# dluvizon/deephar

Measured on AMD Instinct MI355X. Metric: frames/sec whole-node, 256x256 MPII pose fwd, higher is better.
Workload: dtype f32; 1 GPU; MPII single-person 256x256, ReceptionNet 8 blocks J=16 ctx=2 k=5, pose-only forward, batch=64 per GPU (BASELINE.json configs[1]); global_batch=64, parallelism=frame-shard x1 (replicas, no collective), hipgraph=True, streams=1, input=f32, gemm=f32, outputs_finite_in_range=True

## Files before the change

### deephar_amd/_lib.py

```python
import ctypes as C
import os

_HERE = os.path.dirname(os.path.abspath(__file__))
LIB_PATH = os.path.join(_HERE, 'csrc', 'libdeephar_hip.so')

c_f = C.POINTER(C.c_float)
i32, i64, vp = C.c_int32, C.c_int64, C.c_void_p


class ConvArgs(C.Structure):
    _fields_ = [(n, vp) for n in ('x', 'w', 'y', 'pre_scale', 'pre_shift', 'post_scale', 'post_shift',
                                   'res1', 'res2', 'in_lut')] + \
               [(n, i32) for n in ('N', 'H', 'W', 'Cin', 'ldx', 'OH', 'OW', 'Cout', 'ldy', 'KH', 'KW', 'SH',
                                   'SW', 'PT', 'PL', 'K', 'Kp', 'Np', 'ldr1', 'ldr2', 'pre_relu', 'post_relu',
                                   'up2', 'x_u8', 'w_split', 'res2_down', 'ldyp', 'x_resample')] + [('y_pool', vp)]


class ConvSeg(C.Structure):
    _fields_ = [('x2', vp)] + [(n, i32) for n in ('ldx2', 'c_split', 'pool_sh', 'reserved')]


class DwArgs(C.Structure):
    _fields_ = [(n, vp) for n in ('x', 'w', 'y', 'pre_scale', 'pre_shift')] + \
               [(n, i32) for n in ('N', 'H', 'W', 'C', 'ldx', 'ldy', 'KH', 'KW', 'PT', 'PL', 'pre_relu', 'up_in')]


class DwsArgs(C.Structure):
    _fields_ = [(n, vp) for n in ('x', 'w', 'y', 'pre_scale', 'pre_shift')] + \
               [(n, i32) for n in ('N', 'H', 'W', 'C', 'ldx', 'ldy', 'OH', 'OW', 'KH', 'KW', 'SH', 'SW', 'PT', 'PL',
                                   'pre_relu', 'reserved')]


class ConvtArgs(C.Structure):
    _fields_ = [(n, vp) for n in ('x', 'w', 'y', 'pre_scale', 'pre_shift', 'res')] + \
               [(n, i32) for n in ('N', 'H', 'W', 'Cin', 'ldx', 'Cout', 'ldy', 'ldr', 'Kp', 'Np', 'pre_relu', 'post_relu')]


class PoolArgs(C.Structure):
    _fields_ = [(n, vp) for n in ('x', 'y')] + \
               [(n, i32) for n in ('N', 'H', 'W', 'C', 'ldx', 'OH', 'OW', 'ldy', 'KH', 'KW', 'SH', 'SW', 'PT',
                                   'PL', 'mode')]


class EltArgs(C.Structure):
    _fields_ = [(n, vp) for n in ('a', 'b', 'c', 'y', 'scale', 'shift')] + \
               [(n, i32) for n in ('lda', 'ldb', 'ldc', 'ldy')] + [('npix', i64)] + \
               [(n, i32) for n in ('C', 'relu', 'op', 'bcast_b')]


class SamArgs(C.Structure):
    _fields_ = [(n, vp) for n in ('h', 'gx', 'gy', 'xy', 'conf_raw', 'conf_prob', 'prob', 'gmax')] + \
               [(n, i32) for n in ('F', 'H', 'W', 'C', 'ldh', 'ldxy', 'ldcr', 'ldcp', 'ldp')] + \
               [('alpha', C.c_float), ('conf_scale', C.c_float), ('xy_times_conf', i32)]


SIGNATURES = {
    'dh_version': (C.c_int, []),
    'dh_error_string': (C.c_char_p, [C.c_int]),
    'dh_device_info': (C.c_int, [C.c_int, C.c_char_p, C.c_int, C.POINTER(C.c_int)]),
    'dh_conv2d_packed_dims': (C.c_int, [C.c_int] * 4 + [C.POINTER(C.c_int)] * 2),
    'dh_conv2d_pack_weights_host': (C.c_int, [vp, vp] + [C.c_int] * 4),
    'dh_conv2d_pack_weights_split_host': (C.c_int, [vp, vp] + [C.c_int] * 4),
    'dh_conv2d_pack_weights_parts_host': (C.c_int, [vp, vp] + [C.c_int] * 5),
    'dh_conv2d_num_tile_cfgs': (C.c_int, []),
    'dh_conv2d_num_split_tile_cfgs': (C.c_int, []),
    'dh_conv2d_pick_tile_cfg': (C.c_int, [C.c_int, C.c_int]),
    'dh_conv2d_uses_split_k': (C.c_int, [C.POINTER(ConvArgs)]),
    'dh_conv2d_uses_first_layer_kernel': (C.c_int, [C.POINTER(ConvArgs)]),
    'dh_conv2d_split_eligible': (C.c_int, [C.POINTER(ConvArgs)]),
    'dh_conv2d_split_wide_eligible': (C.c_int, [C.POINTER(ConvArgs)]),
    'dh_conv2d_halo_eligible': (C.c_int, [C.POINTER(ConvArgs)]),
    'dh_conv2d_num_halo_tile_cfgs': (C.c_int, []),
    'dh_conv2d_f32': (C.c_int, [C.POINTER(ConvArgs), C.c_int, vp]),
    'dh_normalize_u8_f32': (C.c_int, [vp, vp, vp, C.c_int64, C.c_int, vp]),
    'dh_dwconv2d_f32': (C.c_int, [C.POINTER(DwArgs), vp]),
    'dh_dwconv2d_strided_f32': (C.c_int, [C.POINTER(DwsArgs), vp]),
    'dh_conv2d_transpose2x2_num_tile_cfgs': (C.c_int, []),
    'dh_conv2d_transpose2x2_f32': (C.c_int, [C.POINTER(ConvtArgs), C.c_int, vp]),
    'dh_conv2d_transpose2x2_num_split_tile_cfgs': (C.c_int, []),
    'dh_conv2d_transpose2x2_split_eligible': (C.c_int, [C.POINTER(ConvtArgs)]),
    'dh_conv2d_transpose2x2_split_f32': (C.c_int, [C.POINTER(ConvtArgs), C.c_int, C.c_int, vp]),
    'dh_conv2d_dw_group_f32': (C.c_int, [C.POINTER(ConvArgs), C.POINTER(DwArgs), vp]),
    'dh_conv2d_pair_f32': (C.c_int, [C.POINTER(ConvArgs), C.POINTER(ConvArgs), vp]),
    'dh_conv2d_seg_f32': (C.c_int, [C.POINTER(ConvArgs), C.POINTER(ConvSeg), vp]),
    'dh_pool2d_f32': (C.c_int, [C.POINTER(PoolArgs), vp]),
    'dh_upsample2x_add_f32': (C.c_int, [vp, C.c_int, vp, C.c_int, vp, C.c_int] + [C.c_int] * 4 + [vp]),
    'dh_eltwise_f32': (C.c_int, [C.POINTER(EltArgs), vp]),
    'dh_softargmax2d_f32': (C.c_int, [C.POINTER(SamArgs), vp]),
    'dh_softargmax2d_context_f32': (C.c_int, [C.POINTER(SamArgs), C.c_int, C.c_int, C.c_float, vp, C.c_int, vp]),
    'dh_context_aggregation_f32': (C.c_int, [vp, vp, vp, vp, C.c_int, C.c_int, C.c_int, C.c_float, C.c_int, vp]),
    'dh_depth_means_f32': (C.c_int, [vp, C.c_int, vp, vp] + [C.c_int] * 4 + [vp]),
    'dh_softargmax1d_f32': (C.c_int, [vp, vp, vp, C.c_int, vp] + [C.c_int] * 3 + [vp]),
    'dh_kronecker_f32': (C.c_int, [vp, C.c_int, vp, C.c_int, vp, C.c_int] + [C.c_int] * 4 + [vp]),
    'dh_global_maxmin_softmax_f32': (C.c_int, [vp, C.c_int, vp] + [C.c_int] * 4 + [vp]),
    'dh_copy_channels_f32': (C.c_int, [vp, C.c_int, vp, C.c_int, i64, C.c_int, vp]),
    'dh_zeropad2d_f32': (C.c_int, [vp, vp] + [C.c_int] * 8 + [vp]),
    'dh_depth_from_maps_f32': (C.c_int, [vp, C.c_int, vp, C.c_int, vp, C.c_int] + [C.c_int] * 3 + [vp]),
    'dh_plan_create': (C.c_int, [vp, C.c_size_t, C.POINTER(vp)]),
    'dh_plan_destroy': (C.c_int, [vp]),
    'dh_plan_batch': (C.c_int, [vp]),
    'dh_plan_num_inputs': (C.c_int, [vp]),
    'dh_plan_num_outputs': (C.c_int, [vp]),
    'dh_plan_input_items': (C.c_int64, [vp, C.c_int]),
    'dh_plan_input_is_u8': (C.c_int, [vp, C.c_int]),
    'dh_plan_output_items': (C.c_int64, [vp, C.c_int]),
    'dh_forward': (C.c_int, [vp, C.POINTER(vp), C.c_int, C.POINTER(vp), vp]),
    'dh_forward_host': (C.c_int, [vp, C.POINTER(vp), C.c_int, C.POINTER(vp)]),
    'dh_graph_begin_capture': (C.c_int, [vp]),
    'dh_graph_end_capture': (C.c_int, [vp, C.POINTER(vp)]),
    'dh_graph_launch': (C.c_int, [vp, vp]),
    'dh_graph_destroy': (C.c_int, [vp]),
    'dh_event_create': (C.c_int, [C.POINTER(vp)]),
    'dh_event_record': (C.c_int, [vp, vp]),
    'dh_event_synchronize': (C.c_int, [vp]),
    'dh_event_elapsed_ms': (C.c_int, [vp, vp, C.POINTER(C.c_float)]),
    'dh_event_destroy': (C.c_int, [vp]),
    'dh_stream_synchronize': (C.c_int, [vp]),
    'dh_stream_create': (C.c_int, [C.POINTER(vp)]),
    'dh_stream_destroy': (C.c_int, [vp]),
    'dh_event_create_sync': (C.c_int, [C.POINTER(vp)]),
    'dh_stream_wait_event': (C.c_int, [vp, vp]),
    'dh_stream_spin_us': (C.c_int, [vp, C.c_int]),
}

_lib = None


class DeepharHipError(RuntimeError):
    pass


def load():
    global _lib
    if _lib is not None:
        return _lib
    try:
        import torch
    except ImportError:
        pass
    path = os.environ.get('DEEPHAR_HIP_LIB', LIB_PATH)
    if not os.path.exists(path):
        raise DeepharHipError(
            'libdeephar_hip.so not found at %s -- the HIP back-end is mandatory (no CPU fallback). '
            'Build it with `python -m deephar_amd.csrc.build`.' % path)
    lib = C.CDLL(path)
    for name, (res, args) in SIGNATURES.items():
        fn = getattr(lib, name)
        fn.restype = res
        fn.argtypes = args
    _lib = lib
    return lib


def check(rc, what=''):
    if rc != 0:
        msg = load().dh_error_string(rc).decode()
        raise DeepharHipError('%s failed: %s (rc=%d)' % (what or 'deephar_hip call', msg, rc))
```

### deephar_amd/csrc/build.py

```python
import os
import subprocess
import sys
from concurrent.futures import ThreadPoolExecutor

HERE = os.path.dirname(os.path.abspath(__file__))
ROOT = os.path.dirname(os.path.dirname(HERE))
INCLUDE = os.path.join(ROOT, "include")
SOURCES = ["conv_igemm.hip", "gemm1x1.hip", "convt2x2.hip", "convt2x2s.hip", "gemm1x1s.hip", "gemm1x1s_p2.hip", "gemm1x1s_p1.hip",
           "gemm1x1s_ext.hip", "gemm1x1s_ext_p2.hip", "gemm1x1s_ext_p1.hip", "conv_splitk.hip", "conv_halo.hip", "conv_stem.hip", "spatial.hip", "decoder.hip",
           "capi.hip", "plan.hip"]
HEADERS = sorted(os.path.join(HERE, f) for f in os.listdir(HERE) if f.endswith(".h")) + [os.path.join(INCLUDE, "deephar_hip.h")]
LIB = os.path.join(HERE, "libdeephar_hip.so")
OBJDIR = os.path.join(HERE, "build")
ARCH = "gfx950"
HIPCC = os.environ.get("HIPCC", "/opt/rocm/bin/hipcc")
FLAGS = ["--offload-arch=" + ARCH, "-O3", "-std=c++17", "-fPIC", "-I" + INCLUDE, "-I" + HERE,
         "-Wno-unused-result"]


def _stale(target, deps):
    if not os.path.exists(target):
        return True
    t = os.path.getmtime(target)
    return any(os.path.getmtime(d) > t for d in deps)


def _compile(src):
    obj = os.path.join(OBJDIR, src.replace(".hip", ".o"))
    path = os.path.join(HERE, src)
    deps = [path] + HEADERS
    if _stale(obj, deps):
        cmd = [HIPCC] + FLAGS + ["-c", path, "-o", obj]
        r = subprocess.run(cmd, capture_output=True, text=True)
        if r.returncode != 0:
            raise RuntimeError("hipcc failed for %s:\n%s\n%s" % (src, r.stdout, r.stderr))
    return obj


def build(force=False, verbose=True):
    os.makedirs(OBJDIR, exist_ok=True)
    if force:
        for f in os.listdir(OBJDIR):
            os.remove(os.path.join(OBJDIR, f))
        if os.path.exists(LIB):
            os.remove(LIB)
    with ThreadPoolExecutor(max_workers=len(SOURCES)) as ex:
        objs = list(ex.map(_compile, SOURCES))
    if _stale(LIB, objs):
        cmd = [HIPCC, "--offload-arch=" + ARCH, "-shared", "-fPIC", "-o", LIB] + objs
        r = subprocess.run(cmd, capture_output=True, text=True)
        if r.returncode != 0:
            raise RuntimeError("link failed:\n%s\n%s" % (r.stdout, r.stderr))
        if verbose:
            print("built", LIB)
    elif verbose:
        print("up to date:", LIB)
    return LIB


if __name__ == "__main__":
    build(force="--force" in sys.argv)
```

### deephar_amd/csrc/capi.hip

```cpp
#include <stddef.h>
#include <string.h>
#include <vector>
#include "dh_kernels.h"

using namespace dh;

static inline hipStream_t S(void* s) { return reinterpret_cast<hipStream_t>(s); }
static_assert(sizeof(dh_conv_seg) == 24, "dh_conv_seg layout");
static_assert(sizeof(dh_conv_args) == 200 && offsetof(dh_conv_args, y_pool) == 192 && offsetof(dh_conv_args, x_resample) == 188,
              "dh_conv_args layout");
static_assert(sizeof(dh_dw_args) == 88 && offsetof(dh_dw_args, up_in) == 84, "dh_dw_args layout");
static_assert(sizeof(dh_dw_strided) == 104 && sizeof(dh_conv_transpose) == 96, "dh_dw_strided / dh_conv_transpose layout");
static_assert(sizeof(dh_sam_args) == 112 && offsetof(dh_sam_args, xy_times_conf) == 108, "dh_sam_args layout");
static inline int rc_of(hipError_t e) { return e == hipSuccess ? DH_OK : DH_ELAUNCH; }

extern "C" {

int dh_version(void) { return 100; }

const char* dh_error_string(int rc) {
  switch (rc) {
    case DH_OK: return "ok";
    case DH_EINVAL: return "invalid argument or shape";
    case DH_EUNSUPPORTED: return "configuration not supported by the gfx950 kernels";
    case DH_ELAUNCH: return "HIP launch/runtime error";
    default: return "unknown error";
  }
}

int dh_device_info(int dev, char* arch_name, int arch_name_len, int* cu_count) {
  int n = 0;
  if (hipGetDeviceCount(&n) != hipSuccess || dev < 0 || dev >= n) return DH_ELAUNCH;
  hipDeviceProp_t p;
  if (hipGetDeviceProperties(&p, dev) != hipSuccess) return DH_ELAUNCH;
  if (arch_name != nullptr && arch_name_len > 0) {
    strncpy(arch_name, p.gcnArchName, (size_t)arch_name_len - 1);
    arch_name[arch_name_len - 1] = 0;
  }
  if (cu_count != nullptr) *cu_count = p.multiProcessorCount;
  return DH_OK;
}

int dh_conv2d_packed_dims(int KH, int KW, int Cin, int Cout, int* Kp, int* Np) {
  if (KH <= 0 || KW <= 0 || Cin <= 0 || Cout <= 0) return DH_EINVAL;
  const int K = KH * KW * Cin;
  if (Kp != nullptr) *Kp = (K + 31) / 32 * 32;
  if (Np != nullptr) *Np = (Cout + 31) / 32 * 32;
  return DH_OK;
}

int dh_conv2d_pack_weights_host(const float* w, float* packed, int KH, int KW, int Cin, int Cout) {
  int Kp, Np;
  if (w == nullptr || packed == nullptr || dh_conv2d_packed_dims(KH, KW, Cin, Cout, &Kp, &Np) != DH_OK)
    return DH_EINVAL;
  const int K = KH * KW * Cin;
  memset(packed, 0, sizeof(float) * (size_t)Kp * Np);
  for (int k = 0; k < K; ++k)
    for (int n = 0; n < Cout; ++n)
      packed[((size_t)(k >> 2) * Np + n) * 4 + (k & 3)] = w[(size_t)k * Cout + n];
  return DH_OK;
}

static inline uint16_t bf16_rne(float f) {
  uint32_t u;
  memcpy(&u, &f, 4);
  u += 0x7fffu + ((u >> 16) & 1u);
  return (uint16_t)(u >> 16);
}
static inline float bf16_to_f(uint16_t h) {
  const uint32_t u = (uint32_t)h << 16;
  float f;
  memcpy(&f, &u, 4);
  return f;
}

int dh_conv2d_pack_weights_parts_host(const float* w, uint16_t* packed, int KH, int KW, int Cin, int Cout, int parts) {
  int Kp, Np;
  if (w == nullptr || packed == nullptr || parts < 1 || parts > 3 || dh_conv2d_packed_dims(KH, KW, Cin, Cout, &Kp, &Np) != DH_OK)
    return DH_EINVAL;
  const int K = KH * KW * Cin;
  memset(packed, 0, sizeof(uint16_t) * (size_t)parts * Kp * Np);
  for (int k = 0; k < K; ++k)
    for (int n = 0; n < Cout; ++n) {
      float r = w[(size_t)k * Cout + n];
      const size_t base = ((size_t)(k >> 3) * parts * Np + n) * 8 + (k & 7);
      for (int q = 0; q < parts; ++q) {
        const uint16_t h = bf16_rne(r);
        packed[base + (size_t)q * Np * 8] = h;
        r -= bf16_to_f(h);
      }
    }
  return DH_OK;
}

int dh_conv2d_pack_weights_split_host(const float* w, uint16_t* packed, int KH, int KW, int Cin, int Cout) {
  return dh_conv2d_pack_weights_parts_host(w, packed, KH, KW, Cin, Cout, 3);
}

int dh_conv2d_num_tile_cfgs(void) { return conv_igemm_num_cfgs(); }
int dh_conv2d_num_split_tile_cfgs(void) { return gemm1x1_split_num_cfgs(); }
int dh_conv2d_uses_split_k(const dh_conv_args* a) { return a != nullptr && conv_is_skinny(*a) ? 1 : 0; }
int dh_conv2d_uses_first_layer_kernel(const dh_conv_args* a) {
  return a != nullptr && !conv_is_skinny(*a) && conv_stem_eligible(*a) ? 1 : 0;
}
int dh_conv2d_pick_tile_cfg(int M, int Cout) { return conv_igemm_pick_cfg(M, Cout); }
int dh_conv2d_split_eligible(const dh_conv_args* a) { return a != nullptr && gemm1x1_split_eligible(*a) ? 1 : 0; }
int dh_conv2d_split_wide_eligible(const dh_conv_args* a) { return a != nullptr && gemm1x1_split_wide_eligible(*a) ? 1 : 0; }
int dh_conv2d_halo_eligible(const dh_conv_args* a) { return a != nullptr && conv_halo_eligible(*a) ? 1 : 0; }
int dh_conv2d_num_halo_tile_cfgs(void) { return conv_halo_num_cfgs(); }

int dh_conv2d_f32(const dh_conv_args* a, int tile_cfg, void* stream) {
  if (a == nullptr || a->x == nullptr || a->w == nullptr || a->y == nullptr) return DH_EINVAL;
  if ((a->pre_scale == nullptr) != (a->pre_shift == nullptr)) return DH_EINVAL;
  if ((a->post_scale == nullptr) != (a->post_shift == nullptr)) return DH_EINVAL;
  if (a->SH <= 0 || a->SW <= 0 || a->KH <= 0 || a->KW <= 0) return DH_EINVAL;
  if (a->res2_down && (a->res2 == nullptr || a->up2 || (a->OH & 1) || (a->OW & 1))) return DH_EINVAL;
  return launch_conv_igemm(*a, tile_cfg, S(stream));
}

int dh_conv2d_dw_group_f32(const dh_conv_args* a, const dh_dw_args* d, void* stream) {
  if (a == nullptr || d == nullptr || a->x == nullptr || a->w == nullptr || a->y == nullptr || d->x == nullptr ||
      d->w == nullptr || d->y == nullptr)
    return DH_EINVAL;
  if ((a->pre_scale == nullptr) != (a->pre_shift == nullptr) || (a->post_scale == nullptr) != (a->post_shift == nullptr) ||
      (d->pre_scale == nullptr) != (d->pre_shift == nullptr))
    return DH_EINVAL;
  return launch_conv_dw_group(*a, *d, S(stream));
}

static int check_skinny_args(const dh_conv_args* c) {
  if (c == nullptr || c->x == nullptr || c->w == nullptr || c->y == nullptr) return DH_EINVAL;
  if ((c->pre_scale == nullptr) != (c->pre_shift == nullptr) || (c->post_scale == nullptr) != (c->post_shift == nullptr)) return DH_EINVAL;
  if (c->SH <= 0 || c->SW <= 0 || c->KH <= 0 || c->KW <= 0 || c->N <= 0 || c->Cin <= 0 || c->Cout <= 0 || c->OH <= 0 || c->OW <= 0)
    return DH_EINVAL;
  if (c->Kp % 32 != 0 || c->Np % 32 != 0 || c->Kp < c->K || c->Np < c->Cout || c->K != c->KH * c->KW * c->Cin) return DH_EINVAL;
  if ((long long)c->N * c->H * c->W > 0x7fffffffLL || (long long)c->N * c->OH * c->OW * (c->up2 ? 4 : 1) > 0x7fffffffLL) return DH_EINVAL;
  return DH_OK;
}

int dh_conv2d_pair_f32(const dh_conv_args* a, const dh_conv_args* b, void* stream) {
  if (check_skinny_args(a) != DH_OK || check_skinny_args(b) != DH_OK) return DH_EINVAL;
  return launch_conv_skinny_pair(*a, *b, S(stream));
}

int dh_conv2d_seg_f32(const dh_conv_args* a, const dh_conv_seg* seg, void* stream) {
  if (seg == nullptr || check_skinny_args(a) != DH_OK) return DH_EINVAL;
  return launch_conv_splitk_seg(*a, *seg, S(stream));
}

int dh_normalize_u8_f32(const uint8_t* x, const float* lut, float* y, int64_t n_pixels, int C, void* stream) {
  if (x == nullptr || lut == nullptr || y == nullptr) return DH_EINVAL;
  return launch_normalize_u8(x, lut, y, n_pixels, C, S(stream));
}

int dh_dwconv2d_f32(const dh_dw_args* a, void* stream) {
  if (a == nullptr || a->x == nullptr || a->w == nullptr || a->y == nullptr) return DH_EINVAL;
  if ((a->pre_scale == nullptr) != (a->pre_shift == nullptr)) return DH_EINVAL;
  return launch_dwconv(*a, S(stream));
}

int dh_dwconv2d_strided_f32(const dh_dw_strided* a, void* stream) {
  if (a == nullptr || a->x == nullptr || a->w == nullptr || a->y == nullptr) return DH_EINVAL;
  if ((a->pre_scale == nullptr) != (a->pre_shift == nullptr)) return DH_EINVAL;
  if (a->SH <= 0 || a->SW <= 0 || a->KH <= 0 || a->KW <= 0) return DH_EINVAL;
  return launch_dwconv_strided(*a, S(stream));
}

int dh_conv2d_transpose2x2_num_tile_cfgs(void) { return convt2x2_num_cfgs(); }

static dh_conv_args convt_gemm(const dh_conv_transpose* a) {
  dh_conv_args g;
  memset(&g, 0, sizeof(g));
  g.x = a->x; g.w = a->w; g.y = a->y;
  g.pre_scale = a->pre_scale; g.pre_shift = a->pre_shift;
  g.res1 = a->res; g.ldr1 = a->ldr;
  g.N = a->N; g.H = g.OH = a->H; g.W = g.OW = a->W; g.Cin = g.K = a->Cin; g.ldx = a->ldx;
  g.Cout = 4 * a->Cout; g.ldy = a->ldy;
  g.KH = g.KW = g.SH = g.SW = 1;
  g.Kp = a->Kp; g.Np = a->Np;
  g.pre_relu = a->pre_relu; g.post_relu = a->post_relu;
  return g;
}

int dh_conv2d_transpose2x2_f32(const dh_conv_transpose* a, int tile_cfg, void* stream) {
  if (a == nullptr || a->x == nullptr || a->w == nullptr || a->y == nullptr) return DH_EINVAL;
  if ((a->pre_scale == nullptr) != (a->pre_shift == nullptr)) return DH_EINVAL;
  if (a->N <= 0 || a->H <= 0 || a->W <= 0 || a->Cin <= 0 || a->Cout <= 0 || a->Cout > 0x7fffffff / 4) return DH_EINVAL;
  if (tile_cfg >= convt2x2_num_cfgs()) return DH_EINVAL;
  return launch_convt2x2(convt_gemm(a), a->Cout, tile_cfg, S(stream));
}

int dh_conv2d_transpose2x2_num_split_tile_cfgs(void) { return convt2x2_split_num_cfgs(); }

int dh_conv2d_transpose2x2_split_eligible(const dh_conv_transpose* a) {
  if (a == nullptr || (a->pre_scale == nullptr) != (a->pre_shift == nullptr)) return 0;
  if (a->N <= 0 || a->H <= 0 || a->W <= 0 || a->Cin <= 0 || a->Cout <= 0 || a->Cout > 0x7fffffff / 4) return 0;
  return convt2x2_split_eligible(convt_gemm(a), a->Cout) ? 1 : 0;
}

int dh_conv2d_transpose2x2_split_f32(const dh_conv_transpose* a, int parts, int tile_cfg, void* stream) {
  if (parts < 1 || parts > 3) return DH_EINVAL;
  if (a == nullptr || a->x == nullptr || a->w == nullptr || a->y == nullptr) return DH_EINVAL;
  if ((a->pre_scale == nullptr) != (a->pre_shift == nullptr)) return DH_EINVAL;
  if (a->N <= 0 || a->H <= 0 || a->W <= 0 || a->Cin <= 0 || a->Cout <= 0 || a->Cout > 0x7fffffff / 4) return DH_EINVAL;
  if (tile_cfg >= convt2x2_split_num_cfgs()) return DH_EINVAL;
  return launch_convt2x2_split(convt_gemm(a), a->Cout, parts, tile_cfg, S(stream));
}

int dh_pool2d_f32(const dh_pool_args* a, void* stream) {
  if (a == nullptr || a->x == nullptr || a->y == nullptr || a->SH <= 0 || a->SW <= 0) return DH_EINVAL;
  return launch_pool(*a, S(stream));
}

int dh_upsample2x_add_f32(const float* a, int lda, const float* b, int ldb, float* y, int ldy, int N, int H,
                          int W, int C, void* stream) {
  if (b == nullptr || y == nullptr) return DH_EINVAL;
  return launch_upsample2x_add(a, lda, b, ldb, y, ldy, N, H, W, C, S(stream));
}

int dh_eltwise_f32(const dh_elt_args* a, void* stream) {
  if (a == nullptr) return DH_EINVAL;
  if ((a->scale == nullptr) != (a->shift == nullptr)) return DH_EINVAL;
  return launch_eltwise(*a, S(stream));
}

int dh_softargmax2d_f32(const dh_sam_args* a, void* stream) {
  if (a == nullptr) return DH_EINVAL;
  return launch_softargmax2d(*a, S(stream));
}

int dh_softargmax2d_context_f32(const dh_sam_args* a, int J, int nctx, float agg_alpha, float* y, int ldy,
                                void* stream) {
  if (a == nullptr) return DH_EINVAL;
  return launch_softargmax2d_context(*a, J, nctx, agg_alpha, y, ldy, S(stream));
}

int dh_context_aggregation_f32(const float* ys, const float* yc, const float* pc, float* y, int F, int J,
                               int nctx, float alpha, int ldy, void* stream) {
  if (ys == nullptr || yc == nullptr || pc == nullptr || y == nullptr || ldy < 2) return DH_EINVAL;
  return launch_context_agg(ys, yc, pc, y, F, J, nctx, alpha, ldy, S(stream));
}

int dh_depth_means_f32(const float* h, int ldh, float* hxy, float* hz, int F, int HW, int D, int J,
                       void* stream) {
  if (h == nullptr || (hxy == nullptr && hz == nullptr)) return DH_EINVAL;
  return launch_depth_means(h, ldh, hxy, hz, F, HW, D, J, S(stream));
}

int dh_softargmax1d_f32(const float* hz, const float* grid, float* z, int ldz, float* vz, int F, int D, int J,
                        void* stream) {
  if (hz == nullptr || grid == nullptr) return DH_EINVAL;
  return launch_softargmax1d(hz, grid, z, ldz, vz, F, D, J, S(stream));
}

int dh_kronecker_f32(const float* hm, int ldh, const float* x, int ldx, float* f, int ldf, int B, int P, int J,
                     int C, void* stream) {
  if (hm == nullptr || x == nullptr || f == nullptr) return DH_EINVAL;
  return launch_kronecker(hm, ldh, x, ldx, f, ldf, B, P, J, C, S(stream));
}

int dh_global_maxmin_softmax_f32(const float* x, int ldx, float* y, int B, int P, int C, int softmax,
                                 void* stream) {
  if (x == nullptr || y == nullptr) return DH_EINVAL;
  return launch_global_maxmin_softmax(x, ldx, y, B, P, C, softmax, S(stream));
}

int dh_copy_channels_f32(const float* x, int ldx, float* y, int ldy, int64_t npix, int C, void* stream) {
  if (x == nullptr || y == nullptr) return DH_EINVAL;
  return launch_copy_channels(x, ldx, y, ldy, (long long)npix, C, S(stream));
}

int dh_zeropad2d_f32(const float* x, float* y, int B, int H, int W, int C, int OH, int OW, int PT, int PL,
                     void* stream) {
  if (x == nullptr || y == nullptr) return DH_EINVAL;
  return launch_zeropad(x, y, B, H, W, C, OH, OW, PT, PL, S(stream));
}

int dh_depth_from_maps_f32(const float* d, int ldd, const float* h, int ldh, float* z, int ldz, int F, int HW,
                           int J, void* stream) {
  if (d == nullptr || h == nullptr || z == nullptr) return DH_EINVAL;
  return launch_depth_from_maps(d, ldd, h, ldh, z, ldz, F, HW, J, S(stream));
}

int dh_graph_begin_capture(void* stream) {
  return rc_of(hipStreamBeginCapture(S(stream), hipStreamCaptureModeThreadLocal));
}

int dh_graph_end_capture(void* stream, void** graph_exec_out) {
  if (graph_exec_out == nullptr) return DH_EINVAL;
  hipGraph_t g = nullptr;
  if (hipStreamEndCapture(S(stream), &g) != hipSuccess || g == nullptr) return DH_ELAUNCH;
  hipGraphExec_t ge = nullptr;
  hipError_t e = hipGraphInstantiate(&ge, g, nullptr, nullptr, 0);
  hipGraphDestroy(g);
  if (e != hipSuccess) return DH_ELAUNCH;
  *graph_exec_out = ge;
  return DH_OK;
}

int dh_graph_launch(void* graph_exec, void* stream) {
  if (graph_exec == nullptr) return DH_EINVAL;
  return rc_of(hipGraphLaunch(reinterpret_cast<hipGraphExec_t>(graph_exec), S(stream)));
}

int dh_graph_destroy(void* graph_exec) {
  if (graph_exec == nullptr) return DH_OK;
  return rc_of(hipGraphExecDestroy(reinterpret_cast<hipGraphExec_t>(graph_exec)));
}

int dh_event_create(void** event_out) {
  if (event_out == nullptr) return DH_EINVAL;
  hipEvent_t e;
  if (hipEventCreate(&e) != hipSuccess) return DH_ELAUNCH;
  *event_out = e;
  return DH_OK;
}
int dh_event_record(void* event, void* stream) {
  return rc_of(hipEventRecord(reinterpret_cast<hipEvent_t>(event), S(stream)));
}
int dh_event_synchronize(void* event) { return rc_of(hipEventSynchronize(reinterpret_cast<hipEvent_t>(event))); }
int dh_event_elapsed_ms(void* start, void* stop, float* ms_out) {
  if (ms_out == nullptr) return DH_EINVAL;
  return rc_of(hipEventElapsedTime(ms_out, reinterpret_cast<hipEvent_t>(start), reinterpret_cast<hipEvent_t>(stop)));
}
int dh_event_destroy(void* event) { return rc_of(hipEventDestroy(reinterpret_cast<hipEvent_t>(event))); }
int dh_stream_synchronize(void* stream) { return rc_of(hipStreamSynchronize(S(stream))); }

int dh_stream_create(void** stream_out) {
  if (stream_out == nullptr) return DH_EINVAL;
  hipStream_t st;
  if (hipStreamCreateWithFlags(&st, hipStreamNonBlocking) != hipSuccess) return DH_ELAUNCH;
  *stream_out = st;
  return DH_OK;
}
int dh_stream_destroy(void* stream) { return rc_of(hipStreamDestroy(S(stream))); }
int dh_event_create_sync(void** event_out) {
  if (event_out == nullptr) return DH_EINVAL;
  hipEvent_t e;
  if (hipEventCreateWithFlags(&e, hipEventDisableTiming) != hipSuccess) return DH_ELAUNCH;
  *event_out = e;
  return DH_OK;
}
int dh_stream_wait_event(void* stream, void* event) {
  return rc_of(hipStreamWaitEvent(S(stream), reinterpret_cast<hipEvent_t>(event), 0));
}

__global__ void spin_kernel(long long ticks) {
  const long long t0 = wall_clock64();
  for (int i = 0; i < (1 << 22) && wall_clock64() - t0 < ticks; ++i) __builtin_amdgcn_s_sleep(8);
}
int dh_stream_spin_us(void* stream, int us) {
  if (us < 0 || us > 20000) return DH_EINVAL;
  hipLaunchKernelGGL(spin_kernel, dim3(1), dim3(64), 0, S(stream), (long long)us * 100);
  return check_launch();
}

}
```

### deephar_amd/csrc/dh_kernels.h

```cpp
#pragma once
#include <hip/hip_runtime.h>
#include <stdint.h>
#include "deephar_hip.h"

namespace dh {

using ConvArgs = dh_conv_args;
using ConvSeg = dh_conv_seg;
using DwArgs = dh_dw_args;
using DwsArgs = dh_dw_strided;
using PoolArgs = dh_pool_args;
using EltArgs = dh_elt_args;
using SamArgs = dh_sam_args;

__device__ __forceinline__ int xcd_order(int b, int nwg) {
  const int xcd = b & 7, q = nwg >> 3, r = nwg & 7;
  return (xcd < r ? xcd * (q + 1) : r * (q + 1) + (xcd - r) * q) + (b >> 3);
}

int launch_conv_igemm(const ConvArgs& a, int cfg, hipStream_t s);
int launch_normalize_u8(const unsigned char* x, const float* lut, float* y, long long n_pixels, int C, hipStream_t s);
int conv_igemm_pick_cfg(int M, int Cout);
int conv_igemm_num_cfgs();
bool conv_is_skinny(const ConvArgs& a);
bool conv_stem_eligible(const ConvArgs& a);
int gemm1x1_split_num_cfgs();
bool gemm1x1_split_eligible(const ConvArgs& a);
int conv_split_parts(int w_split);
bool gemm1x1_split_wide_eligible(const ConvArgs& a);
int conv_split_wide_base(int w_split);
bool conv_halo_eligible(const ConvArgs& a);
int conv_halo_num_cfgs();
int launch_dwconv(const DwArgs& a, hipStream_t s);
int launch_dwconv_strided(const DwsArgs& a, hipStream_t s);
int launch_convt2x2(const ConvArgs& gemm, int cb, int cfg, hipStream_t s);
int convt2x2_num_cfgs();
int launch_convt2x2_split(const ConvArgs& gemm, int cb, int parts, int cfg, hipStream_t s);
bool convt2x2_split_eligible(const ConvArgs& gemm, int cb);
int convt2x2_split_num_cfgs();
int launch_conv_dw_group(const ConvArgs& a, const DwArgs& d, hipStream_t s);
int launch_conv_skinny_pair(const ConvArgs& a, const ConvArgs& b, hipStream_t s);
int launch_conv_splitk_seg(const ConvArgs& a, const ConvSeg& seg, hipStream_t s);
int launch_pool(const PoolArgs& a, hipStream_t s);
int launch_upsample2x_add(const float* a, int lda, const float* b, int ldb, float* y, int ldy, int N, int H,
                          int W, int C, hipStream_t s);
int launch_eltwise(const EltArgs& a, hipStream_t s);
int launch_softargmax2d(const SamArgs& a, hipStream_t s);
int launch_softargmax2d_context(const SamArgs& a, int J, int nctx, float agg_alpha, float* y, int ldy, hipStream_t s);
int launch_context_agg(const float* ys, const float* yc, const float* pc, float* y, int F, int J, int nctx,
                       float alpha, int ldy, hipStream_t s);
int launch_depth_means(const float* h, int ldh, float* hxy, float* hz, int F, int HW, int D, int J,
                       hipStream_t s);
int launch_softargmax1d(const float* hz, const float* grid, float* z, int ldz, float* vz, int F, int D, int J,
                        hipStream_t s);
int launch_kronecker(const float* hm, int ldh, const float* x, int ldx, float* f, int ldf, int B, int P, int J,
                     int C, hipStream_t s);
int launch_global_maxmin_softmax(const float* x, int ldx, float* y, int B, int P, int C, int softmax,
                                 hipStream_t s);
int launch_copy_channels(const float* x, int ldx, float* y, int ldy, long long npix, int C, hipStream_t s);
int launch_zeropad(const float* x, float* y, int B, int H, int W, int C, int OH, int OW, int PT, int PL,
                   hipStream_t s);
int launch_depth_from_maps(const float* d, int ldd, const float* h, int ldh, float* z, int ldz, int F, int HW,
                           int J, hipStream_t s);

struct LdsLimit {
  unsigned long long done = 0;
  void raise(const void* kern, int bytes) {
    int dev = 0;
    if (hipGetDevice(&dev) != hipSuccess) return;
    const unsigned long long bit = 1ull << (dev & 63);
    if (done & bit) return;
    hipFuncSetAttribute(kern, hipFuncAttributeMaxDynamicSharedMemorySize, bytes);
    done |= bit;
  }
};

inline bool al16(const void* q) { return (reinterpret_cast<uintptr_t>(q) & 15) == 0; }
constexpr long long kMaxBufferBytes = 0xf0000000LL;
inline bool conv_is_1x1(const ConvArgs& a) { return a.KH == 1 && a.KW == 1 && a.SH == 1 && a.SW == 1 && a.PT == 0 && a.PL == 0; }
inline bool conv_is_pointwise(const ConvArgs& a) { return conv_is_1x1(a) && a.H == a.OH && a.W == a.OW && a.Cin % 4 == 0; }

inline int check_launch() {
  hipError_t e = hipGetLastError();
  return e == hipSuccess ? DH_OK : DH_ELAUNCH;
}

}
```

### deephar_amd/csrc/dw_lds.h

```cpp
#pragma once
#include "dh_kernels.h"
#include "lds_dma.h"

namespace dh {
namespace dwl {

__device__ __forceinline__ float4 ld4(const float* p) { return *reinterpret_cast<const float4*>(p); }
__device__ __forceinline__ void st4(float* p, float4 v) { *reinterpret_cast<float4*>(p) = v; }
__device__ __forceinline__ float4 fma4(float4 a, float4 b, float4 c) {
  return make_float4(fmaf(a.x, b.x, c.x), fmaf(a.y, b.y, c.y), fmaf(a.z, b.z, c.z), fmaf(a.w, b.w, c.w));
}
__device__ __forceinline__ float4 max4(float4 a, float4 b) {
  return make_float4(fmaxf(a.x, b.x), fmaxf(a.y, b.y), fmaxf(a.z, b.z), fmaxf(a.w, b.w));
}
__device__ __forceinline__ float4 min4(float4 a, float4 b) {
  return make_float4(fminf(a.x, b.x), fminf(a.y, b.y), fminf(a.z, b.z), fminf(a.w, b.w));
}


constexpr int DW_CQ = 8;
#ifndef DW_LDS_MIN_W
#define DW_LDS_MIN_W 8
#endif
constexpr int DW_PITCH = 9;
constexpr int DW_OOB = (int)0x80000000u;

typedef unsigned int dw_u4 __attribute__((ext_vector_type(4)));
template <typename RSRC>
__device__ __forceinline__ float4 buf_ld4(RSRC rs, int voff) {
  float4 r = make_float4(0.f, 0.f, 0.f, 0.f);
#if defined(__HIP_DEVICE_COMPILE__)
  const dw_u4 v = __builtin_amdgcn_raw_buffer_load_b128(rs, voff, 0, 0);
  r = make_float4(__uint_as_float(v.x), __uint_as_float(v.y), __uint_as_float(v.z), __uint_as_float(v.w));
#endif
  return r;
}
template <typename RSRC>
__device__ __forceinline__ void buf_st4(RSRC rs, int voff, int soff, float4 r) {
#if defined(__HIP_DEVICE_COMPILE__)
  dw_u4 v;
  v.x = __float_as_uint(r.x); v.y = __float_as_uint(r.y); v.z = __float_as_uint(r.z); v.w = __float_as_uint(r.w);
  __builtin_amdgcn_raw_buffer_store_b128(v, rs, voff, soff, 0);
#endif
}

template <int KS, int NT, int MAXT, int MAXN, bool AFF, bool RELU>
__device__ __forceinline__ void dwconv_lds_body(const DwArgs& p, const int tw, const int rows, const int twh_magic,
                                                const int block, float4* dsm) {
  constexpr int SP = NT / DW_CQ;
  const int tid = threadIdx.x;
  const int chunks = p.C / 32;
  const int bands = (p.H + rows - 1) / rows;
  const int ctiles = (p.W + tw - 1) / tw;
  int b = block;
  const int cchunk = b % chunks; b /= chunks;
  const int ct = b % ctiles;
  const int n = b / ctiles;
  const int c0 = cchunk * 32, w0 = ct * tw;
  const int th = rows + KS - 1, twh = tw + KS - 1;
  float4* wts = dsm;
  float4* tile = dsm + KS * KS * DW_CQ;
  const float4 zero = make_float4(0.f, 0.f, 0.f, 0.f);

  constexpr int WPT = (KS * KS * DW_CQ + NT - 1) / NT;
  float4 wreg[WPT];
#pragma unroll
  for (int k = 0; k < WPT; ++k) {
    const int i = tid + k * NT;
    const int ic = i < KS * KS * DW_CQ ? i : 0;
    wreg[k] = ld4(p.w + (size_t)(ic / DW_CQ) * p.C + c0 + (ic % DW_CQ) * 4);
  }
  const int q = tid & (DW_CQ - 1);
  float4 sc = make_float4(1.f, 1.f, 1.f, 1.f), sh = zero;
  if constexpr (AFF) { sc = ld4(p.pre_scale + c0 + q * 4); sh = ld4(p.pre_shift + c0 + q * 4); }

  const int ush = p.up_in ? 1 : 0;
  const int hw_in = (p.H >> ush) * (p.W >> ush), w_in = p.W >> ush;
  const auto rs_x = __builtin_amdgcn_make_buffer_rsrc(
      const_cast<float*>(p.x) + (size_t)n * hw_in * p.ldx, 0,
      (int)(((unsigned)(hw_in - 1) * p.ldx + (unsigned)p.C) * 4u), 0x00020000);
  const auto rs_y = __builtin_amdgcn_make_buffer_rsrc(
      p.y + (size_t)n * p.H * p.W * p.ldy, 0, (int)(((unsigned)(p.H * p.W - 1) * p.ldy + (unsigned)p.C) * 4u), 0x00020000);
  const int row_bytes = twh * DW_PITCH * 16, ring_bytes = th * row_bytes;
  const int dump = ring_bytes;
  auto row_of = [&](int px) { return (px * twh_magic) >> 16; };
  auto px_offset = [&](int px, int first_row) {
    const int tr = row_of(px), tc = px - tr * twh;
    const int iw = w0 - p.PL + tc;
    return (unsigned)iw < (unsigned)p.W ? ((((first_row + tr) >> ush) * w_in + (iw >> ush)) * p.ldx + c0 + q * 4) * 4 : DW_OOB;
  };

  float4 top[MAXT];
#pragma unroll
  for (int j = 0; j < MAXT; ++j) {
    const int px = (tid >> 3) + j * SP;
    top[j] = buf_ld4(rs_x, px < (KS - 1) * twh ? px_offset(px, -p.PT) : DW_OOB);
  }
  int voff[MAXN], loff[MAXN];
  int trow[AFF ? MAXN : 1];
#pragma unroll
  for (int j = 0; j < MAXN; ++j) {
    const int px = (tid >> 3) + j * SP;
    const bool in = px < rows * twh;
    voff[j] = in ? px_offset(px, KS - 1 - p.PT) : DW_OOB;
    loff[j] = in ? (KS - 1) * row_bytes + (px * DW_PITCH + q) * 16 : -1;
    if constexpr (AFF) trow[j] = (in && voff[j] != DW_OOB) ? row_of(px) : -1;
  }
  float4 stage[MAXN];
  auto fetch = [&](int band) {
    const int boff = band * (rows >> ush) * w_in * p.ldx * 4;
#pragma unroll
    for (int j = 0; j < MAXN; ++j) stage[j] = buf_ld4(rs_x, voff[j] + boff);
  };
  fetch(0);
#pragma unroll
  for (int k = 0; k < WPT; ++k) {
    const int i = tid + k * NT;
    if (i < KS * KS * DW_CQ) wts[i] = wreg[k];
  }
#pragma unroll
  for (int j = 0; j < MAXT; ++j) {
    const int px = (tid >> 3) + j * SP;
    float4 v = top[j];
    if constexpr (AFF) {
      const int tr = row_of(px), iw = w0 - p.PL + px - tr * twh;
      v = fma4(v, sc, sh);
      if (!((unsigned)(tr - p.PT) < (unsigned)p.H && (unsigned)iw < (unsigned)p.W)) v = zero;
    }
    if constexpr (RELU) v = relu4(v);
    if (px < (KS - 1) * twh) tile[px * DW_PITCH + q] = v;
  }
  const int strips = tw >> 3;
  const int strip = (tid >> 3) % strips;
  const int row = (tid >> 3) / strips;
  const int y_off = ((row * p.W + w0 + strip * 8) * p.ldy + c0 + q * 4) * 4;
  const int y_col = p.ldy * 4;
  char* const tile_b = reinterpret_cast<char*>(tile);

  int ring0 = 0;
  for (int band = 0; band < bands; ++band) {
    const int r0 = band * rows;
    const int shift = ring0 * row_bytes;
    if (band > 0) fetch(band);
#pragma unroll
    for (int j = 0; j < MAXN; ++j) {
      float4 v = stage[j];
      if constexpr (AFF) {
        v = fma4(v, sc, sh);
        if (!(trow[j] >= 0 && (unsigned)(r0 + KS - 1 - p.PT + trow[j]) < (unsigned)p.H)) v = zero;
      }
      if constexpr (RELU) v = relu4(v);
      int o = loff[j] + shift;
      o = o >= ring_bytes ? o - ring_bytes : o;
      o = loff[j] < 0 ? dump : o;
      *reinterpret_cast<float4*>(tile_b + o) = v;
    }
    __syncthreads();

    if (row < rows && r0 + row < p.H && w0 + strip * 8 < p.W) {
      float4 acc[8];
#pragma unroll
      for (int i = 0; i < 8; ++i) acc[i] = zero;
      int rr = ring0 + row;
      rr = rr >= th ? rr - th : rr;
#pragma unroll 1
      for (int kh = 0; kh < KS; ++kh) {
        float4 wv[KS];
#pragma unroll
        for (int kw = 0; kw < KS; ++kw) wv[kw] = wts[(kh * KS + kw) * DW_CQ + q];
        const float4* src = tile + (rr * twh + strip * 8) * DW_PITCH + q;
#pragma unroll
        for (int j = 0; j < 8 + KS - 1; ++j) {
          const float4 v = src[j * DW_PITCH];
#pragma unroll
          for (int kw = 0; kw < KS; ++kw) {
            const int o = j - kw;
            if (o >= 0 && o < 8) acc[o] = fma4(v, wv[kw], acc[o]);
          }
        }
        rr = rr + 1 == th ? 0 : rr + 1;
      }
      const int yo = y_off + r0 * p.W * p.ldy * 4;
#pragma unroll
      for (int i = 0; i < 8; ++i) buf_st4(rs_y, yo, i * y_col, acc[i]);
    }
    __syncthreads();
    ring0 += rows;
    ring0 = ring0 >= th ? ring0 - th : ring0;
  }
}

struct DwLdsGeom {
  int tw, rows, nt;
  unsigned blocks;
  size_t lds;
};
inline bool dw_lds_geometry(const DwArgs& a, DwLdsGeom& g) {
  const bool vec = (a.C % 4 == 0) && (a.ldx % 4 == 0) && (a.ldy % 4 == 0) && al16(a.x) && al16(a.y) && al16(a.w) &&
                   (a.pre_scale == nullptr || (al16(a.pre_scale) && al16(a.pre_shift)));
  if (!(vec && a.KH == a.KW && (a.KW == 5 || a.KW == 3) && a.C % 32 == 0 && a.W >= DW_LDS_MIN_W && a.W % 8 == 0)) return false;
  g.tw = a.W >= 32 ? 32 : a.W;
  g.nt = g.tw == 8 ? 64 : 256;
  g.rows = g.nt / (8 * (g.tw / 8));
  if (g.rows > a.H) g.rows = a.H;
  const long long blocks = (long long)a.N * ((a.W + g.tw - 1) / g.tw) * (a.C / 32);
  g.lds = ((size_t)(g.rows + a.KW - 1) * (g.tw + a.KW - 1) * DW_PITCH + (size_t)a.KW * a.KW * DW_CQ + 1) * 16;
  const bool fits31 = (long long)a.H * a.W * a.ldx * 4 < 0x7fffffffLL && (long long)a.H * a.W * a.ldy * 4 < 0x7fffffffLL;
  if (blocks > 0x7fffffffLL || !fits31) return false;
  g.blocks = (unsigned)blocks;
  const int twh = g.tw + a.KW - 1, maxt = a.KW == 5 ? (g.nt == 256 ? 5 : 6) : 3, maxn = a.KW == 5 ? (g.nt == 256 ? 10 : 12) : 10;
  return (a.KW - 1) * twh <= maxt * (g.nt / DW_CQ) && g.rows * twh <= maxn * (g.nt / DW_CQ);
}

}
}
```

### deephar_amd/csrc/gemm1x1_body.h

```cpp
#pragma once
#include "conv_common.h"
#include "gemm_family.h"
#include "lds_dma.h"

namespace dh {

template <bool PRE, int S>
__device__ __forceinline__ void fetch_affine(unsigned t_sc, unsigned t_sh, float4& sc, float4& sh) {
  if constexpr (PRE) {
    sc = lds_rd<S * 32>(t_sc);
    sh = lds_rd<S * 32>(t_sh);
  }
}

template <int TM, int TN, int BN, int BOFF, int S>
__device__ __forceinline__ void fetch_frags(const unsigned (&a_addr)[TM][4], unsigned b_addr, float4 (&fa)[TM],
                                            float4 (&fb)[TN]) {
  fa[0] = lds_rd<0>(a_addr[0][S]);
  if constexpr (TM > 1) fa[1] = lds_rd<0>(a_addr[1][S]);
  constexpr int BO = BOFF + S * 2 * BN * 16;
  fb[0] = lds_rd<BO>(b_addr);
  if constexpr (TN > 1) fb[1] = lds_rd<BO + 512>(b_addr);
  if constexpr (TN > 2) fb[2] = lds_rd<BO + 1024>(b_addr);
}

template <int WM, int WN, int TM, int TN, bool UP2, bool RELU, bool KXK = false, bool PRE = false, bool D2S = false>
__device__ __forceinline__ void gemm1x1_body(const ConvArgs& p, const int epi_vec, const int block, const int nblocks,
                                             float* const smem, const int cb = 0) {
  static_assert(!(PRE && (KXK || UP2)), "the BN prologue is built for the plain pointwise form");
  static_assert(!(D2S && (KXK || UP2)), "the depth-to-space epilogue follows the plain pointwise main loop");
  constexpr int NT = WM * WN * 64;
  constexpr int BM = WM * TM * 32;
  constexpr int BN = WN * TN * 32;
  constexpr int APASS = BM * 8 / NT;
  constexpr int BPASS = 8 * BN / NT;
  constexpr int STAGE = BM * BK + BK * BN;
  static_assert(BM * 8 % NT == 0 && (8 * BN) % NT == 0, "tile/thread mismatch");

  const int tid = threadIdx.x;
  const int lane = tid & 63;
  const int wave = tid >> 6;
  const int wm = wave / WN, wn = wave % WN;
  const int li = lane & 31, lh = lane >> 5;

  const int M = p.N * p.OH * p.OW;
  const int tiles_n = (p.Cout + BN - 1) / BN;
  const int tile = xcd_tile(block, nblocks);
  const int m0 = (tile / tiles_n) * BM;
  const int n0 = (tile % tiles_n) * BN;

  const int wave_u = __builtin_amdgcn_readfirstlane(wave);
  const auto rs_x = __builtin_amdgcn_make_buffer_rsrc(
      const_cast<float*>(p.x), 0, (int)(((unsigned)(p.N * p.H * p.W - 1) * p.ldx + (unsigned)p.Cin) * 4u), 0x00020000);
  const auto rs_w = __builtin_amdgcn_make_buffer_rsrc(const_cast<float*>(p.w), 0, (int)((unsigned)p.Kp * p.Np * 4u),
                                                      0x00020000);
  unsigned a_off[APASS];
  int a_slot[APASS];
  int a_pix[KXK ? APASS : 1], a_ih0[KXK ? APASS : 1], a_iw0[KXK ? APASS : 1];
#pragma unroll
  for (int ps = 0; ps < APASS; ++ps) {
    const int r = (tid >> 3) + ps * (NT / 8);
    int m = m0 + r;
    m = m < M ? m : M - 1;
    a_slot[ps] = ((tid & 7) ^ (r & 7)) * 4;
    if constexpr (KXK) {
      const int n = m / (p.OH * p.OW);
      const int rem = m - n * (p.OH * p.OW);
      const int oh = rem / p.OW, ow = rem - oh * p.OW;
      a_pix[ps] = n * p.H * p.W;
      a_ih0[ps] = oh * p.SH - p.PT;
      a_iw0[ps] = ow * p.SW - p.PL;
      a_off[ps] = 0;
    } else {
      a_off[ps] = ((unsigned)m * p.ldx + a_slot[ps]) * 4u;
    }
  }
  const int chunks_per_tap = KXK ? p.Cin / BK : 1;
  unsigned b_off[BPASS];
#pragma unroll
  for (int q = 0; q < BPASS; ++q) {
    const int idx = tid + q * NT;
    const int kq = idx / BN, j = idx - kq * BN;
    const int col = n0 + j < p.Np ? n0 + j : 0;
    b_off[q] = ((unsigned)kq * p.Np + col) * 16u;
  }
  const int b_step = 8 * p.Np * 16;

  auto issue = [&](int kt, int stage) {
    float* sA = smem + stage * STAGE;
    float* sB = sA + BM * BK;
    int kh = 0, kw = 0, c0 = 0;
    if constexpr (KXK) {
      const int tap = kt / chunks_per_tap;
      c0 = (kt - tap * chunks_per_tap) * BK;
      kh = tap / p.KW;
      kw = tap - kh * p.KW;
    }
#pragma unroll
    for (int ps = 0; ps < APASS; ++ps) {
      if constexpr (KXK) {
        const int ih = a_ih0[ps] + kh, iw = a_iw0[ps] + kw;
        const bool ok = (unsigned)ih < (unsigned)p.H && (unsigned)iw < (unsigned)p.W && kt * BK < p.K;
        const unsigned off = ok ? ((unsigned)(a_pix[ps] + ih * p.W + iw) * p.ldx + c0 + a_slot[ps]) * 4u : OOB;
        dma16(rs_x, sA + (ps * NT + wave_u * 64) * 4, off, 0);
      } else {
        dma16(rs_x, sA + (ps * NT + wave_u * 64) * 4, a_off[ps], kt * BK * 4);
      }
    }
#pragma unroll
    for (int q = 0; q < BPASS; ++q) dma16(rs_w, sB + (q * NT + wave_u * 64) * 4, b_off[q], kt * b_step);
  };

  f32x16 acc[TM][TN];
#pragma unroll
  for (int i = 0; i < TM; ++i)
#pragma unroll
    for (int j = 0; j < TN; ++j)
#pragma unroll
      for (int r = 0; r < 16; ++r) acc[i][j][r] = 0.f;

  const int nk = p.Kp / BK;
  issue(0, 0);
  if constexpr (PRE) {
    float* tab = smem + 2 * STAGE;
    for (int i = tid; i < p.Kp; i += NT) {
      tab[i] = i < p.K ? p.pre_scale[i] : 0.f;
      tab[p.Kp + i] = i < p.K ? p.pre_shift[i] : 0.f;
    }
  }
  asm volatile("s_waitcnt vmcnt(0)" ::: "memory");
  __syncthreads();

  const unsigned lds0 = (unsigned)(uintptr_t)(lptr_t)smem;
  unsigned a_base[TM][4];
#pragma unroll
  for (int i = 0; i < TM; ++i)
#pragma unroll
    for (int q = 0; q < 4; ++q)
      a_base[i][q] = lds0 + (unsigned)(((wm * TM + i) * 32 + li) * BK * 4 + (((q * 2 + lh) ^ (li & 7)) << 4));
  const unsigned b_base = lds0 + (unsigned)((lh * BN + wn * TN * 32 + li) * 16);
  constexpr int BOFF = BM * BK * 4;

  auto mfma_block = [&](const float4 (&a)[TM], const float4 (&b)[TN]) {
#pragma unroll
    for (int i = 0; i < TM; ++i)
#pragma unroll
      for (int j = 0; j < TN; ++j) {
        acc[i][j] = __builtin_amdgcn_mfma_f32_32x32x2f32(a[i].x, b[j].x, acc[i][j], 0, 0, 0);
        acc[i][j] = __builtin_amdgcn_mfma_f32_32x32x2f32(a[i].y, b[j].y, acc[i][j], 0, 0, 0);
        acc[i][j] = __builtin_amdgcn_mfma_f32_32x32x2f32(a[i].z, b[j].z, acc[i][j], 0, 0, 0);
        acc[i][j] = __builtin_amdgcn_mfma_f32_32x32x2f32(a[i].w, b[j].w, acc[i][j], 0, 0, 0);
      }
  };
  auto relu_frags = [&](float4 (&a)[TM], const float4& sc, const float4& sh) {
    if constexpr (PRE) {
#pragma unroll
      for (int i = 0; i < TM; ++i)
        a[i] = make_float4(fmaf(a[i].x, sc.x, sh.x), fmaf(a[i].y, sc.y, sh.y), fmaf(a[i].z, sc.z, sh.z), fmaf(a[i].w, sc.w, sh.w));
    }
    if constexpr (RELU) {
#pragma unroll
      for (int i = 0; i < TM; ++i) a[i] = relu4(a[i]);
    }
  };
  const unsigned t_sc0 = lds0 + (unsigned)(2 * STAGE * 4 + lh * 16);

  EpiPrefetch<TM, TN> pre;
  for (int kt = 0; kt < nk; ++kt) {
    const int cur = kt & 1;
    if constexpr (!D2S) {
      if (kt == nk - 1) pre.template issue<WM, WN>(p, m0, n0, M, epi_vec);
    }
    const unsigned so = (unsigned)(cur * STAGE * 4);
    unsigned a_addr[TM][4];
#pragma unroll
    for (int i = 0; i < TM; ++i)
#pragma unroll
      for (int q = 0; q < 4; ++q) a_addr[i][q] = a_base[i][q] + so;
    const unsigned b_addr = b_base + so;

    float4 fa0[TM], fb0[TN], fa1[TM], fb1[TN];
    float4 sc0, sh0, sc1, sh1;
    const unsigned t_sc = t_sc0 + (unsigned)(kt * BK * 4), t_sh = t_sc + (unsigned)(p.Kp * 4);
    fetch_frags<TM, TN, BN, BOFF, 0>(a_addr, b_addr, fa0, fb0);
    fetch_affine<PRE, 0>(t_sc, t_sh, sc0, sh0);
    __builtin_amdgcn_sched_barrier(0);
    if (kt + 1 < nk) issue(kt + 1, cur ^ 1);
    lgkm_wait();
    fetch_frags<TM, TN, BN, BOFF, 1>(a_addr, b_addr, fa1, fb1);
    fetch_affine<PRE, 1>(t_sc, t_sh, sc1, sh1);
    __builtin_amdgcn_sched_barrier(0);
    relu_frags(fa0, sc0, sh0);
    mfma_block(fa0, fb0);
    lgkm_wait();
    fetch_frags<TM, TN, BN, BOFF, 2>(a_addr, b_addr, fa0, fb0);
    fetch_affine<PRE, 2>(t_sc, t_sh, sc0, sh0);
    __builtin_amdgcn_sched_barrier(0);
    relu_frags(fa1, sc1, sh1);
    mfma_block(fa1, fb1);
    lgkm_wait();
    fetch_frags<TM, TN, BN, BOFF, 3>(a_addr, b_addr, fa1, fb1);
    fetch_affine<PRE, 3>(t_sc, t_sh, sc1, sh1);
    __builtin_amdgcn_sched_barrier(0);
    relu_frags(fa0, sc0, sh0);
    mfma_block(fa0, fb0);
    lgkm_wait();
    relu_frags(fa1, sc1, sh1);
    mfma_block(fa1, fb1);

    asm volatile("s_waitcnt vmcnt(0)" ::: "memory");
    __syncthreads();
  }

  if constexpr (D2S) d2s_epilogue<WM, WN, TM, TN>(p, acc, smem, m0, n0, M, epi_vec, cb);
  else conv_epilogue<WM, WN, TM, TN, UP2, true>(p, acc, smem, m0, n0, M, epi_vec, pre);
}

}
```

### deephar_amd/csrc/plan.hip

```cpp
#include <cstring>
#include <vector>
#include "dh_kernels.h"

namespace {

using dh::check_launch;

enum Fn { F_CONV, F_DW, F_POOL, F_UPADD, F_ELT, F_SAM, F_CTX, F_DMEANS, F_SAM1D, F_KRON, F_GMM, F_COPY, F_ZPAD, F_DFM, F_SAMCTX, F_NORM, F_GROUP, F_PAIR, F_SEG, F_DWS, F_CONVT, F_CONVTS, F_COUNT };

struct Step { int fn; std::vector<unsigned char> payload; };
struct In { uint64_t tag; size_t items; int u8; char* dst; };
struct Out { size_t off, npix; int C, ld; };

}

struct dh_plan {
  int n = 0;
  size_t arena_bytes = 0, weight_bytes = 0, byte_bytes = 0;
  char* arena = nullptr;
  char* weights = nullptr;
  char* bytes = nullptr;
  std::vector<In> ins;
  std::vector<Out> outs;
  std::vector<Step> steps;
  std::vector<float*> in_dev, out_dev;
  hipStream_t stream = nullptr;
};

namespace {

struct Reader {
  const unsigned char* p;
  const unsigned char* end;
  bool ok = true;
  template <typename T>
  T get() {
    T v{};
    if (p + sizeof(T) > end) { ok = false; return v; }
    std::memcpy(&v, p, sizeof(T));
    p += sizeof(T);
    return v;
  }
};

bool fix(const dh_plan& pl, uint64_t v, void** out) {
  const uint64_t region = v >> 60, off = v & ((1ull << 60) - 1);
  if (v == 0) { *out = nullptr; return true; }
  if (region == 1 && off < pl.arena_bytes) { *out = pl.arena + off; return true; }
  if (region == 2 && off < pl.weight_bytes) { *out = pl.weights + off; return true; }
  if (region == 3 && off < pl.byte_bytes) { *out = pl.bytes + off; return true; }
  return false;
}

int struct_pointers(int fn) {
  switch (fn) {
    case F_CONV: return 10;
    case F_DW: return 5;
    case F_POOL: return 2;
    case F_ELT: return 6;
    case F_SAM: return 8;
    case F_SAMCTX: return 8;
    case F_DWS: return 5;
    case F_CONVT: return 6;
    case F_CONVTS: return 6;
  }
  return -1;
}
void struct_extra(int fn, int* nargs, unsigned* ptr_mask) {
  *nargs = 0;
  *ptr_mask = 0;
  if (fn == F_CONV || fn == F_CONVT) *nargs = 1;
  if (fn == F_CONVTS) *nargs = 2;
  if (fn == F_SAMCTX) { *nargs = 5; *ptr_mask = 0x08; }
}
size_t struct_size(int fn) {
  switch (fn) {
    case F_CONV: return sizeof(dh_conv_args);
    case F_DW: return sizeof(dh_dw_args);
    case F_POOL: return sizeof(dh_pool_args);
    case F_ELT: return sizeof(dh_elt_args);
    case F_SAM: return sizeof(dh_sam_args);
    case F_SAMCTX: return sizeof(dh_sam_args);
    case F_DWS: return sizeof(dh_dw_strided);
    case F_CONVT: return sizeof(dh_conv_transpose);
    case F_CONVTS: return sizeof(dh_conv_transpose);
  }
  return 0;
}
bool scalar_sig(int fn, int* nargs, unsigned* ptr_mask) {
  switch (fn) {
    case F_UPADD: *nargs = 10; *ptr_mask = 0x15; return true;
    case F_CTX: *nargs = 9; *ptr_mask = 0x0f; return true;
    case F_DMEANS: *nargs = 8; *ptr_mask = 0x0d; return true;
    case F_SAM1D: *nargs = 8; *ptr_mask = 0x17; return true;
    case F_KRON: *nargs = 10; *ptr_mask = 0x15; return true;
    case F_GMM: *nargs = 7; *ptr_mask = 0x05; return true;
    case F_COPY: *nargs = 6; *ptr_mask = 0x05; return true;
    case F_ZPAD: *nargs = 10; *ptr_mask = 0x03; return true;
    case F_DFM: *nargs = 9; *ptr_mask = 0x15; return true;
    case F_NORM: *nargs = 5; *ptr_mask = 0x07; return true;
  }
  return false;
}

int run_step(const Step& st, void* stream) {
  const unsigned char* p = st.payload.data();
  auto u = [&](int i) { uint64_t v; std::memcpy(&v, p + 8 * i, 8); return v; };
  auto P = [&](int i) { return reinterpret_cast<float*>(static_cast<uintptr_t>(u(i))); };
  auto I = [&](int i) { return static_cast<int>(static_cast<int64_t>(u(i))); };
  auto Fl = [&](int i) { float f; std::memcpy(&f, p + 8 * i, 4); return f; };
  switch (st.fn) {
    case F_CONV: {
      int64_t cfg;
      std::memcpy(&cfg, p + sizeof(dh_conv_args), 8);
      return dh_conv2d_f32(reinterpret_cast<const dh_conv_args*>(p), (int)cfg, stream);
    }
    case F_SAMCTX: {
      const unsigned char* e = p + sizeof(dh_sam_args);
      int64_t J, nctx, ldy;
      float alpha;
      void* y;
      std::memcpy(&J, e, 8); std::memcpy(&nctx, e + 8, 8); std::memcpy(&alpha, e + 16, 4);
      std::memcpy(&y, e + 24, 8); std::memcpy(&ldy, e + 32, 8);
      return dh_softargmax2d_context_f32(reinterpret_cast<const dh_sam_args*>(p), (int)J, (int)nctx, alpha,
                                         static_cast<float*>(y), (int)ldy, stream);
    }
    case F_DW: return dh_dwconv2d_f32(reinterpret_cast<const dh_dw_args*>(p), stream);
    case F_DWS: return dh_dwconv2d_strided_f32(reinterpret_cast<const dh_dw_strided*>(p), stream);
    case F_CONVT: {
      int64_t cfg;
      std::memcpy(&cfg, p + sizeof(dh_conv_transpose), 8);
      return dh_conv2d_transpose2x2_f32(reinterpret_cast<const dh_conv_transpose*>(p), (int)cfg, stream);
    }
    case F_CONVTS: {
      int64_t parts, cfg;
      std::memcpy(&parts, p + sizeof(dh_conv_transpose), 8);
      std::memcpy(&cfg, p + sizeof(dh_conv_transpose) + 8, 8);
      return dh_conv2d_transpose2x2_split_f32(reinterpret_cast<const dh_conv_transpose*>(p), (int)parts, (int)cfg, stream);
    }
    case F_GROUP:
      return dh_conv2d_dw_group_f32(reinterpret_cast<const dh_conv_args*>(p),
                                    reinterpret_cast<const dh_dw_args*>(p + sizeof(dh_conv_args)), stream);
    case F_PAIR:
      return dh_conv2d_pair_f32(reinterpret_cast<const dh_conv_args*>(p), reinterpret_cast<const dh_conv_args*>(p + sizeof(dh_conv_args)),
                                stream);
    case F_SEG:
      return dh_conv2d_seg_f32(reinterpret_cast<const dh_conv_args*>(p), reinterpret_cast<const dh_conv_seg*>(p + sizeof(dh_conv_args)),
                               stream);
    case F_POOL: return dh_pool2d_f32(reinterpret_cast<const dh_pool_args*>(p), stream);
    case F_ELT: return dh_eltwise_f32(reinterpret_cast<const dh_elt_args*>(p), stream);
    case F_SAM: return dh_softargmax2d_f32(reinterpret_cast<const dh_sam_args*>(p), stream);
    case F_UPADD: return dh_upsample2x_add_f32(P(0), I(1), P(2), I(3), P(4), I(5), I(6), I(7), I(8), I(9), stream);
    case F_CTX: return dh_context_aggregation_f32(P(0), P(1), P(2), P(3), I(4), I(5), I(6), Fl(7), I(8), stream);
    case F_DMEANS: return dh_depth_means_f32(P(0), I(1), P(2), P(3), I(4), I(5), I(6), I(7), stream);
    case F_SAM1D: return dh_softargmax1d_f32(P(0), P(1), P(2), I(3), P(4), I(5), I(6), I(7), stream);
    case F_KRON: return dh_kronecker_f32(P(0), I(1), P(2), I(3), P(4), I(5), I(6), I(7), I(8), I(9), stream);
    case F_GMM: return dh_global_maxmin_softmax_f32(P(0), I(1), P(2), I(3), I(4), I(5), I(6), stream);
    case F_COPY: return dh_copy_channels_f32(P(0), I(1), P(2), I(3), static_cast<int64_t>(u(4)), I(5), stream);
    case F_ZPAD: return dh_zeropad2d_f32(P(0), P(1), I(2), I(3), I(4), I(5), I(6), I(7), I(8), I(9), stream);
    case F_DFM: return dh_depth_from_maps_f32(P(0), I(1), P(2), I(3), P(4), I(5), I(6), I(7), I(8), stream);
    case F_NORM: return dh_normalize_u8_f32(reinterpret_cast<const uint8_t*>(P(0)), P(1), P(2), static_cast<int64_t>(u(3)),
                                            I(4), stream);
  }
  return DH_EINVAL;
}

}

extern "C" {

int dh_plan_create(const void* blob, size_t blob_bytes, dh_plan** out) {
  if (blob == nullptr || out == nullptr || blob_bytes < 44) return DH_EINVAL;
  Reader r{static_cast<const unsigned char*>(blob), static_cast<const unsigned char*>(blob) + blob_bytes};
  if (std::memcmp(r.p, "DHPL", 4) != 0) return DH_EINVAL;
  r.p += 4;
  const uint32_t version = r.get<uint32_t>();
  if (version < 1 || version > 4) return DH_EINVAL;
  dh_plan* pl = new dh_plan();
  pl->n = r.get<int32_t>();
  pl->arena_bytes = r.get<uint64_t>();
  pl->weight_bytes = r.get<uint64_t>();
  const uint32_t nin = r.get<uint32_t>(), nout = r.get<uint32_t>(), nsteps = r.get<uint32_t>();
  if (version >= 2) pl->byte_bytes = r.get<uint64_t>();
  auto fail = [&](int rc) { dh_plan_destroy(pl); return rc; };
  if (!r.ok || pl->n <= 0 || nin == 0 || nout == 0 || nin > 64 || nout > 4096 || nsteps > (1u << 20) ||
      pl->byte_bytes > (1ull << 40))
    return fail(DH_EINVAL);
  for (uint32_t i = 0; i < nin; ++i) {
    In in{};
    in.tag = r.get<uint64_t>();
    in.items = (size_t)r.get<uint64_t>();
    if (version >= 2) {
      in.u8 = (int)r.get<uint32_t>();
      (void)r.get<uint32_t>();
    } else {
      in.tag |= 1ull << 60;
    }
    pl->ins.push_back(in);
  }
  for (uint32_t i = 0; i < nout; ++i) {
    Out o;
    o.off = r.get<uint64_t>(); o.npix = r.get<uint64_t>(); o.C = (int)r.get<uint32_t>(); o.ld = (int)r.get<uint32_t>();
    pl->outs.push_back(o);
  }
  for (uint32_t i = 0; i < nsteps && r.ok; ++i) {
    Step st;
    st.fn = (int)r.get<uint32_t>();
    const uint32_t nb = r.get<uint32_t>();
    if (!r.ok || st.fn < 0 || st.fn >= (version >= 4 ? (int)F_COUNT : (version == 3 ? (int)F_CONVTS : (int)F_DWS)) || r.p + nb > r.end) return fail(DH_EINVAL);
    st.payload.assign(r.p, r.p + nb);
    r.p += nb;
    pl->steps.push_back(std::move(st));
  }
  if (!r.ok || (size_t)(r.end - r.p) != pl->weight_bytes) return fail(DH_EINVAL);
  if (hipMalloc(&pl->arena, pl->arena_bytes ? pl->arena_bytes : 16) != hipSuccess) return fail(DH_ELAUNCH);
  if (hipMalloc(&pl->weights, pl->weight_bytes ? pl->weight_bytes : 16) != hipSuccess) return fail(DH_ELAUNCH);
  if (pl->weight_bytes && hipMemcpy(pl->weights, r.p, pl->weight_bytes, hipMemcpyHostToDevice) != hipSuccess)
    return fail(DH_ELAUNCH);
  if (pl->byte_bytes && hipMalloc(&pl->bytes, pl->byte_bytes) != hipSuccess) return fail(DH_ELAUNCH);
  const uint64_t arena_f = pl->arena_bytes / 4, nn = (uint64_t)pl->n;
  auto fits = [&](uint64_t off_bytes, uint64_t rows, uint64_t pitch, uint64_t last) {
    if (off_bytes % 4 || off_bytes / 4 > arena_f || rows == 0 || pitch > arena_f || last > arena_f || rows > arena_f) return false;
    const uint64_t room = arena_f - off_bytes / 4;
    if (pitch != 0 && rows - 1 > room / pitch) return false;
    return (rows - 1) * pitch + last <= room;
  };
  for (In& in : pl->ins) {
    const uint64_t region = in.tag >> 60, off = in.tag & ((1ull << 60) - 1);
    if (in.u8 == 0) {
      if (region != 1 || in.items == 0 || in.items > arena_f || !fits(off, nn, in.items, in.items)) return fail(DH_EINVAL);
      in.dst = pl->arena + off;
    } else {
      if (in.u8 != 1 || region != 3 || in.items == 0 || in.items > pl->byte_bytes || nn > pl->byte_bytes / in.items ||
          off > pl->byte_bytes - in.items * nn)
        return fail(DH_EINVAL);
      in.dst = pl->bytes + off;
    }
  }
  for (const Out& o : pl->outs)
    if (o.C <= 0 || o.ld < o.C || o.npix == 0 || o.npix > arena_f || !fits(o.off, o.npix * nn, (uint64_t)o.ld, (uint64_t)o.C))
      return fail(DH_EINVAL);
  for (Step& st : pl->steps) {
    const int np = struct_pointers(st.fn);
    if (st.fn == F_GROUP || st.fn == F_PAIR || st.fn == F_SEG) {
      const size_t second = st.fn == F_GROUP ? sizeof(dh_dw_args) : (st.fn == F_PAIR ? sizeof(dh_conv_args) : sizeof(dh_conv_seg));
      if (st.payload.size() != sizeof(dh_conv_args) + second) return fail(DH_EINVAL);
      size_t at_off[10 + 1 + 10 + 1];
      int k = 0;
      for (int i = 0; i < 10; ++i) at_off[k++] = (size_t)8 * i;
      at_off[k++] = offsetof(dh_conv_args, y_pool);
      for (int i = 0; i < (st.fn == F_GROUP ? 5 : (st.fn == F_PAIR ? 10 : 1)); ++i) at_off[k++] = sizeof(dh_conv_args) + (size_t)8 * i;
      if (st.fn == F_PAIR) at_off[k++] = sizeof(dh_conv_args) + offsetof(dh_conv_args, y_pool);
      for (int i = 0; i < k; ++i) {
        unsigned char* at = st.payload.data() + at_off[i];
        uint64_t v;
        void* ptr;
        std::memcpy(&v, at, 8);
        if (!fix(*pl, v, &ptr)) return fail(DH_EINVAL);
        std::memcpy(at, &ptr, 8);
      }
    } else if (np >= 0) {
      int nextra;
      unsigned emask;
      struct_extra(st.fn, &nextra, &emask);
      if (st.payload.size() != struct_size(st.fn) + (size_t)nextra * 8) return fail(DH_EINVAL);
      if (st.fn == F_CONV) {
        unsigned char* at = st.payload.data() + offsetof(dh_conv_args, y_pool);
        uint64_t v;
        void* ptr;
        std::memcpy(&v, at, 8);
        if (!fix(*pl, v, &ptr)) return fail(DH_EINVAL);
        std::memcpy(at, &ptr, 8);
      }
      for (int i = 0; i < np + nextra; ++i) {
        if (i >= np && !(emask & (1u << (i - np)))) continue;
        unsigned char* at = st.payload.data() + (i < np ? (size_t)8 * i : struct_size(st.fn) + (size_t)8 * (i - np));
        uint64_t v;
        void* ptr;
        std::memcpy(&v, at, 8);
        if (!fix(*pl, v, &ptr)) return fail(DH_EINVAL);
        std::memcpy(at, &ptr, 8);
      }
    } else {
      int nargs;
      unsigned mask;
      if (!scalar_sig(st.fn, &nargs, &mask) || st.payload.size() != (size_t)nargs * 8) return fail(DH_EINVAL);
      for (int i = 0; i < nargs; ++i)
        if (mask & (1u << i)) {
          uint64_t v;
          void* ptr;
          std::memcpy(&v, st.payload.data() + 8 * i, 8);
          if (!fix(*pl, v, &ptr)) return fail(DH_EINVAL);
          std::memcpy(st.payload.data() + 8 * i, &ptr, 8);
        }
    }
  }
  *out = pl;
  return DH_OK;
}

int dh_plan_destroy(dh_plan* pl) {
  if (pl == nullptr) return DH_OK;
  if (pl->stream) hipStreamSynchronize(pl->stream);
  for (float* q : pl->in_dev) hipFree(q);
  for (float* q : pl->out_dev) hipFree(q);
  if (pl->stream) hipStreamDestroy(pl->stream);
  if (pl->arena) hipFree(pl->arena);
  if (pl->weights) hipFree(pl->weights);
  if (pl->bytes) hipFree(pl->bytes);
  delete pl;
  return DH_OK;
}

int dh_plan_batch(const dh_plan* pl) { return pl ? pl->n : 0; }
int dh_plan_num_inputs(const dh_plan* pl) { return pl ? (int)pl->ins.size() : 0; }
int dh_plan_num_outputs(const dh_plan* pl) { return pl ? (int)pl->outs.size() : 0; }
int64_t dh_plan_input_items(const dh_plan* pl, int i) {
  return (pl && i >= 0 && i < (int)pl->ins.size()) ? (int64_t)pl->ins[i].items : -1;
}
int dh_plan_input_is_u8(const dh_plan* pl, int i) {
  return (pl && i >= 0 && i < (int)pl->ins.size()) ? pl->ins[i].u8 : -1;
}
int64_t dh_plan_output_items(const dh_plan* pl, int i) {
  return (pl && i >= 0 && i < (int)pl->outs.size()) ? (int64_t)(pl->outs[i].npix * pl->outs[i].C) : -1;
}

int dh_forward(dh_plan* pl, const float* const* inputs, int m, float* const* outputs, void* stream) {
  if (pl == nullptr || inputs == nullptr || outputs == nullptr || m <= 0 || m > pl->n) return DH_EINVAL;
  hipStream_t s = reinterpret_cast<hipStream_t>(stream);
  for (size_t i = 0; i < pl->ins.size(); ++i) {
    if (inputs[i] == nullptr) return DH_EINVAL;
    const In& in = pl->ins[i];
    if (hipMemcpyAsync(in.dst, inputs[i], in.items * (in.u8 ? 1 : 4) * (size_t)m, hipMemcpyDeviceToDevice, s) != hipSuccess)
      return DH_ELAUNCH;
  }
  for (const Step& st : pl->steps) {
    const int rc = run_step(st, stream);
    if (rc != DH_OK) return rc;
  }
  for (size_t i = 0; i < pl->outs.size(); ++i) {
    const Out& o = pl->outs[i];
    if (outputs[i] == nullptr) continue;
    const int rc = dh_copy_channels_f32(reinterpret_cast<const float*>(pl->arena + o.off), o.ld, outputs[i], o.C,
                                        (int64_t)o.npix * m, o.C, stream);
    if (rc != DH_OK) return rc;
  }
  return DH_OK;
}

int dh_forward_host(dh_plan* pl, const float* const* inputs_host, int m, float* const* outputs_host) {
  if (pl == nullptr || inputs_host == nullptr || outputs_host == nullptr || m <= 0 || m > pl->n) return DH_EINVAL;
  if (pl->stream == nullptr) {
    hipStream_t st = nullptr;
    std::vector<float*> in_dev, out_dev;
    bool ok = hipStreamCreateWithFlags(&st, hipStreamNonBlocking) == hipSuccess;
    for (size_t i = 0; ok && i < pl->ins.size(); ++i) {
      float* q = nullptr;
      ok = hipMalloc(&q, pl->ins[i].items * (pl->ins[i].u8 ? 1 : 4) * (size_t)pl->n) == hipSuccess;
      if (ok) in_dev.push_back(q);
    }
    for (size_t i = 0; ok && i < pl->outs.size(); ++i) {
      float* q = nullptr;
      ok = hipMalloc(&q, pl->outs[i].npix * pl->outs[i].C * 4 * (size_t)pl->n) == hipSuccess;
      if (ok) out_dev.push_back(q);
    }
    if (!ok) {
      for (float* q : in_dev) hipFree(q);
      for (float* q : out_dev) hipFree(q);
      if (st) hipStreamDestroy(st);
      return DH_ELAUNCH;
    }
    pl->in_dev.swap(in_dev);
    pl->out_dev.swap(out_dev);
    pl->stream = st;
  }
  for (size_t i = 0; i < pl->ins.size(); ++i)
    if (hipMemcpyAsync(pl->in_dev[i], inputs_host[i], pl->ins[i].items * (pl->ins[i].u8 ? 1 : 4) * (size_t)m,
                       hipMemcpyHostToDevice, pl->stream) != hipSuccess)
      return DH_ELAUNCH;
  const int rc = dh_forward(pl, pl->in_dev.data(), m, pl->out_dev.data(), pl->stream);
  if (rc != DH_OK) return rc;
  for (size_t i = 0; i < pl->outs.size(); ++i)
    if (outputs_host[i] != nullptr &&
        hipMemcpyAsync(outputs_host[i], pl->out_dev[i], pl->outs[i].npix * pl->outs[i].C * 4 * (size_t)m,
                       hipMemcpyDeviceToHost, pl->stream) != hipSuccess)
      return DH_ELAUNCH;
  return hipStreamSynchronize(pl->stream) == hipSuccess ? DH_OK : DH_ELAUNCH;
}

}
```

### deephar_amd/engine/executor.py

```python
import ctypes as C
import functools
import os

import numpy as np

from .. import _lib
from . import packing

SPLIT_CODES = {'bf16x3': 1, 'bf16x2': 3, 'bf16': 4}
WIDE_SPLIT_CODES = {'bf16x3': 5, 'bf16x2': 6, 'bf16': 7}

BN_EPS = 1e-3


def _torch():
    import torch
    return torch


class WeightStore:

    def __init__(self, device):
        self.device = device
        self.conv = {}
        self.dw = {}
        self.bn = {}
        self.const = {}

    def _dev(self, arr):
        torch = _torch()
        return torch.from_numpy(np.ascontiguousarray(arr, dtype=np.float32)).to(self.device)

    @staticmethod
    def _require(p):
        if p.value is None:
            raise RuntimeError('weight %s is not set: call model.load_weights(...) or '
                               'deephar_amd.weights.init_synthetic(model) before predict' % p.key)
        return p.value

    def conv_weight(self, p, split=0):
        split = packing.WIDE_SPLIT_BASE.get(int(split), int(split))
        key = (id(p), int(split))
        ent = self.conv.get(key)
        if ent is None or ent[3] != p.version:
            packer = {0: packing.pack_conv, 2: packing.pack_conv_halo}.get(int(split)) or \
                functools.partial(packing.pack_conv_split, parts=packing.SPLIT_PARTS[int(split)])
            packed, kp, np_ = packer(self._require(p))
            if ent is None:
                ent = (self._dev(packed), kp, np_, p.version)
            else:
                ent[0].copy_(self._dev(packed))
                ent = (ent[0], kp, np_, p.version)
            self.conv[key] = ent
        return ent[0], ent[1], ent[2]

    CONVT = 'convt'

    def convt_weight(self, p, split=0):
        key = (id(p), self.CONVT if not split else (self.CONVT, int(split)))
        ent = self.conv.get(key)
        if ent is None or ent[3] != p.version:
            packed, kp, np_ = packing.pack_convt(self._require(p), parts=packing.SPLIT_PARTS[int(split)] if split else None)
            if ent is None:
                ent = (self._dev(packed), kp, np_, p.version)
            else:
                ent[0].copy_(self._dev(packed))
                ent = (ent[0], kp, np_, p.version)
            self.conv[key] = ent
        return ent[0], ent[1], ent[2]

    def dw_weight(self, p):
        ent = self.dw.get(id(p))
        if ent is None or ent[1] != p.version:
            w = self._require(p)
            flat = np.ascontiguousarray(w.reshape(w.shape[0] * w.shape[1], w.shape[2]))
            if ent is None:
                ent = (self._dev(flat), p.version)
            else:
                ent[0].copy_(self._dev(flat))
                ent = (ent[0], p.version)
            self.dw[id(p)] = ent
        return ent[0]

    def _bn_host(self, layer):
        byrole = {p.role: self._require(p) for p in layer.params}
        inv = (np.float32(1.0) / np.sqrt(byrole['var'].astype(np.float32) + np.float32(BN_EPS))).astype(np.float32)
        if 'gamma' in byrole:
            inv = (inv * byrole['gamma']).astype(np.float32)
        return inv, (byrole['beta'] - byrole['mean'] * inv).astype(np.float32)

    def bn_affine(self, layer):
        vers = tuple(p.version for p in layer.params)
        ent = self.bn.get(id(layer))
        if ent is None or ent[2] != vers:
            if hasattr(layer, 'parts'):
                pieces = [self._bn_host(l) if l is not None else (np.ones(c, np.float32), np.zeros(c, np.float32))
                          for c, l in layer.parts]
                inv = np.concatenate([a for a, _ in pieces]).astype(np.float32)
                shift = np.concatenate([b for _, b in pieces]).astype(np.float32)
            else:
                inv, shift = self._bn_host(layer)
            if ent is None:
                ent = (self._dev(inv), self._dev(shift), vers)
            else:
                ent[0].copy_(self._dev(inv))
                ent[1].copy_(self._dev(shift))
                ent = (ent[0], ent[1], vers)
            self.bn[id(layer)] = ent
        return ent[0], ent[1]

    def constant(self, key, make):
        t = self.const.get(key)
        if t is None:
            t = self._dev(make())
            self.const[key] = t
        return t


def grid_x(w):
    return np.linspace(0.0, 1.0, num=w).astype(np.float32)


def normalization_lut(channels, channel_power=1):
    powers = [channel_power] * channels if isinstance(channel_power, int) else list(channel_power)
    if len(powers) != channels:
        raise ValueError('channel_power expected to be int or a list with one entry per channel')
    lut = np.empty((channels, 256), np.float32)
    for c, pw in enumerate(powers):
        v = np.arange(256, dtype=np.float32)
        v /= 255.
        if pw != 1:
            v = np.power(v, pw)
        v -= .5
        v *= 2.
        lut[c] = v
    return lut


def grid_depth(d):
    s = 1 / (2 * d)
    return np.linspace(s, 1 - s, num=d).astype(np.float32)


class _InputStep:
    kind, name, stream, wait, record, deps, params = 'normalize_u8', 'input', 0, (), False, (), {}

    def __init__(self, v):
        self.outs = {'y': v}
        self.ins = {}
        self.attrs = {}

    def flops(self, n):
        return 0

    def bytes(self, n):
        v = self.outs['y']
        return 5 * n * int(np.prod(v.shape))


from .planner import split_k_rule


class BoundPlan:

    def __init__(self, plan, n, store, device, u8_norm=None):
        torch = _torch()
        self.plan, self.n, self.store, self.device = plan, n, store, device
        self.lib = _lib.load()
        self.arena = torch.empty(max(plan.arena_items * n, 4), dtype=torch.float32, device=device)
        self.base = self.arena.data_ptr()
        self.calls = []
        self._keep = []
        self.graph = None
        self.perturb = None
        self.u8 = None
        self.npre = 0
        if u8_norm is not None:
            self.u8 = {}
            for v in plan.inputs:
                lut = store.constant(('u8lut', v.C, repr(u8_norm)), lambda v=v: normalization_lut(v.C, u8_norm))
                buf = torch.zeros((n,) + v.shape, dtype=torch.uint8, device=device)
                users = [s for s in plan.steps for w in s.ins.values() if w is not None and w.buf is v.buf]
                fused = all(s.kind == 'conv' and s.ins['x'].buf is v.buf and s.ins['x'].C == v.C and
                            s.ins['x'].coff == v.coff and v.C % 4 != 0 and 'pre_bn' not in s.params and
                            s.ins.get('res1') is None and s.ins.get('res2') is None for s in users)
                self.u8[id(v.buf)] = (buf, lut, fused)
                if not fused:
                    self.calls.append((self.lib.dh_normalize_u8_f32,
                                       (buf.data_ptr(), lut.data_ptr(), self.ptr(v), n * int(np.prod(v.shape[:-1])),
                                        v.C), _InputStep(v)))
                    self.npre += 1
        for step in plan.steps:
            self._bind(step)
        self.grouped = 0
        self.noop_calls = set()
        self.paired = []
        self.absorbed = {}

    def weight_layout(self, args):
        mode = getattr(self.plan, 'gemm_precision', 'f32')
        if getattr(self.plan, 'gemm_scope', 'standard') == 'extended':
            code = WIDE_SPLIT_CODES.get(mode)
            if code and self.lib.dh_conv2d_split_wide_eligible(C.byref(args)):
                return code
        else:
            code = SPLIT_CODES.get(mode)
            if code and self.lib.dh_conv2d_split_eligible(C.byref(args)):
                return code
        if self.plan.rules.halo_conv and self.lib.dh_conv2d_halo_eligible(C.byref(args)):
            return 2
        return 0

    def ptr(self, v):
        return self.base + 4 * (v.buf.offset * self.n + v.coff)

    def tensor(self, v):
        torch = _torch()
        shape = (self.n,) + v.shape
        strides = [1] * len(shape)
        strides[-1] = 1
        if len(shape) >= 2:
            strides[-2] = v.ld
            for i in range(len(shape) - 3, -1, -1):
                strides[i] = strides[i + 1] * shape[i + 1]
        return torch.as_strided(self.arena, shape, strides, v.buf.offset * self.n + v.coff)

    def _bind(self, s):
        lib, n, k = self.lib, self.n, s.kind
        a = s.attrs
        P = self.ptr

        def opt(role, d=s.ins):
            v = d.get(role)
            return P(v) if v is not None else None

        if k == 'conv':
            x, y = s.ins['x'], s.outs['y']
            args = _lib.ConvArgs()
            args.x, args.y = P(x), P(y)
            if 'pre_bn' in s.params:
                sc, sh = self.store.bn_affine(s.params['pre_bn'])
                args.pre_scale, args.pre_shift = sc.data_ptr(), sh.data_ptr()
            if 'post_bn' in s.params or 'post_affine' in s.params:
                sc, sh = self.store.bn_affine(s.params.get('post_bn') or s.params['post_affine'])
                args.post_scale, args.post_shift = sc.data_ptr(), sh.data_ptr()
            up = 2 if a['up2'] else 1
            args.N = n * x.lead(3)
            args.H, args.W, args.Cin, args.ldx = x.shape[-3], x.shape[-2], x.C, x.ld
            sg = a.get('seg')
            if sg is not None:
                args.H, args.W, args.Cin = x.shape[-3] // sg['pool_sh'], x.shape[-2] // 2, a['Cin']
            rs = a.get('x_resample', 0)
            if rs:
                args.x_resample = rs
                args.H, args.W = (2 * x.shape[-3], 2 * x.shape[-2]) if rs == 1 else (x.shape[-3] // 2, x.shape[-2] // 2)
            args.OH, args.OW, args.Cout, args.ldy = y.shape[-3] // up, y.shape[-2] // up, a['Cout'], y.ld
            args.KH, args.KW, args.SH, args.SW, args.PT, args.PL = a['kh'], a['kw'], a['sh'], a['sw'], a['pt'], a['pl']
            kp_np = (C.c_int(), C.c_int())
            _lib.check(lib.dh_conv2d_packed_dims(a['kh'], a['kw'], args.Cin, a['Cout'], C.byref(kp_np[0]), C.byref(kp_np[1])))
            args.K, args.Kp, args.Np = a['K'], kp_np[0].value, kp_np[1].value
            r1, r2 = s.ins.get('res1'), s.ins.get('res2')
            if r1 is not None:
                args.res1, args.ldr1 = P(r1), r1.ld
            if r2 is not None:
                args.res2, args.ldr2 = P(r2), r2.ld
            args.pre_relu, args.post_relu, args.up2 = a['pre_relu'], a['post_relu'], a['up2']
            args.res2_down = a.get('res2_down', 0)
            yp = s.outs.get('ypool')
            if yp is not None:
                args.y_pool, args.ldyp = P(yp), yp.ld
            if self.u8 is not None and id(x.buf) in self.u8 and self.u8[id(x.buf)][2]:
                buf, lut, _ = self.u8[id(x.buf)]
                args.x, args.in_lut, args.x_u8 = buf.data_ptr(), lut.data_ptr(), 1
            a['x_u8'] = int(args.x_u8)
            split = self.weight_layout(args)
            wt, kp, np_ = self.store.conv_weight(s.params['w'], split=split)
            assert (kp, np_) == (args.Kp, args.Np)
            args.w, args.w_split = wt.data_ptr(), int(split)
            a['w_split'] = int(split)
            self._keep.append(args)
            if sg is not None:
                seg = _lib.ConvSeg()
                x2 = s.ins.get('x2')
                if x2 is not None:
                    seg.x2, seg.ldx2 = P(x2), x2.ld
                seg.c_split, seg.pool_sh = sg['c_split'], sg['pool_sh']
                self._keep.append(seg)
                self.calls.append((lib.dh_conv2d_seg_f32, (C.byref(args), C.byref(seg)), s))
                return
            self.calls.append((lib.dh_conv2d_f32, (C.byref(args), a.get('tile_cfg', -1)), s))
        elif k == 'dwconv' and (a.get('sh', 1), a.get('sw', 1)) != (1, 1):
            x, y = s.ins['x'], s.outs['y']
            args = _lib.DwsArgs()
            args.x, args.w, args.y = P(x), self.store.dw_weight(s.params['w']).data_ptr(), P(y)
            if 'pre_bn' in s.params:
                sc, sh = self.store.bn_affine(s.params['pre_bn'])
                args.pre_scale, args.pre_shift = sc.data_ptr(), sh.data_ptr()
            args.N, args.H, args.W, args.C = n * x.lead(3), x.shape[-3], x.shape[-2], x.C
            args.OH, args.OW, args.ldx, args.ldy = y.shape[-3], y.shape[-2], x.ld, y.ld
            args.KH, args.KW, args.SH, args.SW, args.PT, args.PL = a['kh'], a['kw'], a['sh'], a['sw'], a['pt'], a['pl']
            args.pre_relu = a['pre_relu']
            self._keep.append(args)
            self.calls.append((lib.dh_dwconv2d_strided_f32, (C.byref(args),), s))
        elif k == 'convtranspose':
            x, y = s.ins['x'], s.outs['y']
            args = _lib.ConvtArgs()
            args.x, args.y = P(x), P(y)
            if 'pre_bn' in s.params:
                sc, sh = self.store.bn_affine(s.params['pre_bn'])
                args.pre_scale, args.pre_shift = sc.data_ptr(), sh.data_ptr()
            r1 = s.ins.get('res1')
            if r1 is not None:
                args.res, args.ldr = P(r1), r1.ld
            args.N, args.H, args.W, args.Cin, args.ldx = n * x.lead(3), x.shape[-3], x.shape[-2], x.C, x.ld
            kp_np = (C.c_int(), C.c_int())
            _lib.check(lib.dh_conv2d_packed_dims(1, 1, x.C, 4 * a['Cout'], C.byref(kp_np[0]), C.byref(kp_np[1])))
            args.Cout, args.ldy, args.Kp, args.Np = a['Cout'], y.ld, kp_np[0].value, kp_np[1].value
            args.pre_relu, args.post_relu = a['pre_relu'], a['post_relu']
            split = SPLIT_CODES.get(getattr(self.plan, 'gemm_precision', 'f32'), 0)
            if split and not lib.dh_conv2d_transpose2x2_split_eligible(C.byref(args)):
                split = 0
            wt, kp, np_ = self.store.convt_weight(s.params['w'], split=split)
            assert (kp, np_) == (args.Kp, args.Np)
            args.w = wt.data_ptr()
            a['w_split'] = int(split)
            self._keep.append(args)
            if split:
                self.calls.append((lib.dh_conv2d_transpose2x2_split_f32,
                                   (C.byref(args), packing.SPLIT_PARTS[split], a.get('tile_cfg', -1)), s))
            else:
                self.calls.append((lib.dh_conv2d_transpose2x2_f32, (C.byref(args), a.get('tile_cfg', -1)), s))
        elif k == 'dwconv':
            x, y = s.ins['x'], s.outs['y']
            args = _lib.DwArgs()
            args.x, args.w, args.y = P(x), self.store.dw_weight(s.params['w']).data_ptr(), P(y)
            if 'pre_bn' in s.params:
                sc, sh = self.store.bn_affine(s.params['pre_bn'])
                args.pre_scale, args.pre_shift = sc.data_ptr(), sh.data_ptr()
            args.N, args.H, args.W, args.C = n * y.lead(3), y.shape[-3], y.shape[-2], x.C
            args.ldx, args.ldy = x.ld, y.ld
            args.KH, args.KW, args.PT, args.PL, args.pre_relu = a['kh'], a['kw'], a['pt'], a['pl'], a['pre_relu']
            args.up_in = a.get('up_in', 0)
            self._keep.append(args)
            self.calls.append((lib.dh_dwconv2d_f32, (C.byref(args),), s))
        elif k == 'pool':
            x, y = s.ins['x'], s.outs['y']
            args = _lib.PoolArgs()
            args.x, args.y = P(x), P(y)
            args.N, args.H, args.W, args.C, args.ldx = n * x.lead(3), x.shape[-3], x.shape[-2], x.C, x.ld
            args.OH, args.OW, args.ldy = y.shape[-3], y.shape[-2], y.ld
            args.KH, args.KW, args.SH, args.SW, args.PT, args.PL = a['kh'], a['kw'], a['sh'], a['sw'], a['pt'], a['pl']
            args.mode = a.get('mode', 0)
            self._keep.append(args)
            self.calls.append((lib.dh_pool2d_f32, (C.byref(args),), s))
        elif k == 'upsample_add':
            b, y = s.ins['b'], s.outs['y']
            av = s.ins.get('a')
            self.calls.append((lib.dh_upsample2x_add_f32,
                               (P(av) if av is not None else None, av.ld if av is not None else 0, P(b), b.ld,
                                P(y), y.ld, n * y.lead(3), y.shape[-3], y.shape[-2], y.C), s))
        elif k == 'eltwise':
            av, y = s.ins['a'], s.outs['y']
            args = _lib.EltArgs()
            args.a, args.y, args.lda, args.ldy = P(av), P(y), av.ld, y.ld
            bv, cv = s.ins.get('b'), s.ins.get('c')
            if bv is not None:
                args.b, args.ldb = P(bv), bv.ld
            if cv is not None:
                args.c, args.ldc = P(cv), cv.ld
            if 'bn' in s.params:
                sc, sh = self.store.bn_affine(s.params['bn'])
                args.scale, args.shift = sc.data_ptr(), sh.data_ptr()
            elif 'scale_const' in a:
                kc, cc = a['scale_const'], av.C
                args.scale = self.store.constant(('const', kc, cc), lambda: np.full(cc, kc, np.float32)).data_ptr()
                args.shift = self.store.constant(('const', 0.0, cc), lambda: np.zeros(cc, np.float32)).data_ptr()
            args.npix, args.C = n * av.npix, av.C
            args.relu, args.op, args.bcast_b = a.get('relu', 0), a.get('op', 0), a.get('bcast_b', 0)
            self._keep.append(args)
            self.calls.append((lib.dh_eltwise_f32, (C.byref(args),), s))
        elif k == 'sam':
            h = s.ins['h']
            H, W = h.shape[-3], h.shape[-2]
            args = _lib.SamArgs()
            args.h = P(h)
            args.gx = self.store.constant(('gx', W), lambda: grid_x(W)).data_ptr()
            args.gy = self.store.constant(('gx', H), lambda: grid_x(H)).data_ptr()
            o = s.outs
            if o.get('xy') is not None:
                args.xy, args.ldxy = P(o['xy']), o['xy'].ld
            if o.get('conf_raw') is not None:
                args.conf_raw, args.ldcr = P(o['conf_raw']), o['conf_raw'].ld
            if o.get('conf_prob') is not None:
                args.conf_prob, args.ldcp = P(o['conf_prob']), o['conf_prob'].ld
            if o.get('prob') is not None:
                args.prob, args.ldp = P(o['prob']), o['prob'].ld
            if o.get('gmax') is not None:
                assert o['gmax'].dense
                args.gmax = P(o['gmax'])
            args.F, args.H, args.W, args.C, args.ldh = n * h.lead(3), H, W, h.C, h.ld
            args.alpha, args.conf_scale = a['alpha'], a['conf_scale']
            args.xy_times_conf = a.get('xy_times_conf', 0)
            self._keep.append(args)
            self.calls.append((lib.dh_softargmax2d_f32, (C.byref(args),), s))
        elif k == 'sam_ctx':
            h, y = s.ins['h'], s.outs['y']
            H, W = h.shape[-3], h.shape[-2]
            args = _lib.SamArgs()
            args.h = P(h)
            args.gx = self.store.constant(('gx', W), lambda: grid_x(W)).data_ptr()
            args.gy = self.store.constant(('gx', H), lambda: grid_x(H)).data_ptr()
            cr = s.outs.get('conf_raw')
            if cr is not None:
                args.conf_raw, args.ldcr = P(cr), cr.ld
            args.F, args.H, args.W, args.C, args.ldh = n * h.lead(3), H, W, h.C, h.ld
            args.alpha, args.conf_scale = a['sam_alpha'], a['conf_scale']
            self._keep.append(args)
            self.calls.append((lib.dh_softargmax2d_context_f32,
                               (C.byref(args), a['J'], a['nctx'], a['alpha'], P(y), y.ld), s))
        elif k == 'context_agg':
            ys, y = s.ins['ys'], s.outs['y']
            self.calls.append((lib.dh_context_aggregation_f32,
                               (P(ys), P(s.ins['yc']), P(s.ins['pc']), P(y), n * ys.lead(2), ys.shape[-2],
                                a['nctx'], a['alpha'], y.ld), s))
        elif k == 'depth_means':
            h = s.ins['h']
            self.calls.append((lib.dh_depth_means_f32,
                               (P(h), h.ld, opt('hxy', s.outs), opt('hz', s.outs), n * h.lead(3),
                                h.shape[-3] * h.shape[-2], a['D'], a['J']), s))
        elif k == 'softargmax1d':
            hz = s.ins['hz']
            D, J = hz.shape[-2], hz.shape[-1]
            grid = self.store.constant(('gd', D), lambda: grid_depth(D))
            z = s.outs.get('z')
            self.calls.append((lib.dh_softargmax1d_f32,
                               (P(hz), grid.data_ptr(), P(z) if z is not None else None,
                                z.ld if z is not None else 1, opt('vz', s.outs), n * hz.lead(2), D, J), s))
        elif k == 'kronecker':
            hm, x, y = s.ins['hm'], s.ins['x'], s.outs['y']
            self.calls.append((lib.dh_kronecker_f32,
                               (P(hm), hm.ld, P(x), x.ld, P(y), y.ld, n * hm.lead(3),
                                hm.shape[-3] * hm.shape[-2], hm.C, x.C), s))
        elif k == 'globalmaxmin':
            x, y = s.ins['x'], s.outs['y']
            self.calls.append((lib.dh_global_maxmin_softmax_f32,
                               (P(x), x.ld, P(y), n * x.lead(3), x.shape[-3] * x.shape[-2], x.C, a['softmax']), s))
        elif k == 'copy':
            x, y = s.ins['x'], s.outs['y']
            self.calls.append((lib.dh_copy_channels_f32, (P(x), x.ld, P(y), y.ld, n * x.npix, x.C), s))
        elif k == 'zeropad':
            x, y = s.ins['x'], s.outs['y']
            self.calls.append((lib.dh_zeropad2d_f32,
                               (P(x), P(y), n * x.lead(3), x.shape[-3], x.shape[-2], x.C, y.shape[-3],
                                y.shape[-2], a.get('pt', 0), a.get('pl', 0)), s))
        elif k == 'depthsum':
            d, h, z = s.ins['d'], s.ins['h'], s.outs['z']
            self.calls.append((lib.dh_depth_from_maps_f32,
                               (P(d), d.ld, P(h), h.ld, P(z), z.ld, n * d.lead(3), d.shape[-3] * d.shape[-2], d.C), s))
        else:
            raise NotImplementedError('no binding for step kind %r' % k)

    def _side_streams(self, main_ptr=None):
        if getattr(self, '_streams', None) is None:
            lib = self.lib
            self._streams, self._events, self._join, self._fork, self._relay = [], {}, [], C.c_void_p(), {}
            roles = [shared_stream(self.device, r) for r in ('head', 'comm', 'copy')]
            spare = [st for st in roles if main_ptr is None or st.cuda_stream != main_ptr]
            for k in range(self.plan.nstreams - 1):
                st, ev = C.c_void_p(), C.c_void_p()
                if k < len(spare):
                    st = C.c_void_p(spare[k].cuda_stream)
                else:
                    _lib.check(lib.dh_stream_create(C.byref(st)), 'stream create')
                _lib.check(lib.dh_event_create_sync(C.byref(ev)), 'event create')
                self._streams.append(st)
                self._join.append(ev)
            _lib.check(lib.dh_event_create_sync(C.byref(self._fork)), 'event create')
            for i, (_, _, step) in enumerate(self.calls):
                if step.record:
                    ev = C.c_void_p()
                    _lib.check(lib.dh_event_create_sync(C.byref(ev)), 'event create')
                    self._events[i] = ev
        return self._streams

    def launch_all(self, stream_ptr):
        lib = self.lib
        if self.plan.nstreams <= 1:
            for i, (fn, args, step) in enumerate(self.calls):
                if self.perturb is not None:
                    self.perturb(i, step, stream_ptr, [stream_ptr])
                rc = fn(*args, stream_ptr)
                if rc != 0:
                    _lib.check(rc, 'step %s (%s)' % (step.kind, step.name))
            return
        side = self._side_streams(stream_ptr)
        ptrs = [stream_ptr] + [st for st in side]
        for fn, args, step in self.calls[:self.npre]:
            _lib.check(fn(*args, stream_ptr), step.kind)
        _lib.check(lib.dh_event_record(self._fork, stream_ptr), 'fork')
        for st in side:
            _lib.check(lib.dh_stream_wait_event(st, self._fork), 'fork wait')
        for i, (fn, args, step) in enumerate(self.calls):
            if i < self.npre:
                continue
            sp = ptrs[step.stream]
            for w in step.wait:
                ev = self._events[w + self.npre]
                src = self.calls[w + self.npre][2].stream
                if step.stream != 0 and src > step.stream:
                    key = (i, w)
                    if key not in self._relay:
                        r = C.c_void_p()
                        _lib.check(lib.dh_event_create_sync(C.byref(r)), 'event create')
                        self._relay[key] = r
                    _lib.check(lib.dh_stream_wait_event(stream_ptr, ev), 'relay wait')
                    _lib.check(lib.dh_event_record(self._relay[key], stream_ptr), 'relay record')
                    ev = self._relay[key]
                _lib.check(lib.dh_stream_wait_event(sp, ev), 'dependency wait')
            if self.perturb is not None:
                self.perturb(i, step, sp, ptrs)
            rc = fn(*args, sp)
            if rc != 0:
                _lib.check(rc, 'step %s (%s)' % (step.kind, step.name))
            if step.record:
                _lib.check(lib.dh_event_record(self._events[i], sp), 'event record')
        for st, ev in zip(side, self._join):
            _lib.check(lib.dh_event_record(ev, st), 'join record')
            _lib.check(lib.dh_stream_wait_event(stream_ptr, ev), 'join wait')

    GROUP_MAX_ROWS = 8192
    GROUP_MAX_DW_ELEMS = 1 << 23

    def group_launches(self, stream_ptr):
        if not self.plan.rules.group_launches or self.grouped or self.paired:
            return self.grouped
        lib = self.lib
        for i in range(self.npre, len(self.calls) - 1):
            fc, ac, sc = self.calls[i]
            j = next((k for k in range(i + 1, len(self.calls)) if self.calls[k][2].stream == sc.stream), None)
            if j is None:
                continue
            fd, ad, sd = self.calls[j]
            if sc.kind != 'conv' or sd.kind != 'dwconv' or sd.wait or i in self.noop_calls or fc is lib.dh_conv2d_dw_group_f32:
                continue
            if fd is not lib.dh_dwconv2d_f32:
                continue
            if sc.ins['x'].buf is not sd.ins['x'].buf or not self._independent(sc, sd):
                continue
            ca, da = ac[0]._obj, ad[0]._obj
            if ca.N * ca.OH * ca.OW > self.GROUP_MAX_ROWS or da.N * da.H * da.W * da.C > self.GROUP_MAX_DW_ELEMS:
                continue
            if lib.dh_conv2d_dw_group_f32(ac[0], ad[0], stream_ptr) != 0:
                continue
            sc.attrs['grouped'] = True
            self._absorb(i, j, lib.dh_conv2d_dw_group_f32)
            self.grouped += 1
        self._pair_skinny_convs(stream_ptr)
        if self.grouped or self.paired:
            self._drop_graph()
        return self.grouped

    def _absorb(self, i, k, fn):
        (_, ai, si), (_, ak, sk) = self.calls[i], self.calls[k]
        self.calls[i] = (fn, (ai[0], ak[0]), si)
        self.calls[k] = (_noop_launch, (), sk)
        self.noop_calls.add(k)
        self.absorbed[i] = sk

    PAIR_LOOKAHEAD = 3

    @staticmethod
    def _values_overlap(v, w):
        if v is None or w is None:
            return False
        if v.buf is w.buf:
            return not (v.ld == w.ld and (v.coff + v.C <= w.coff or w.coff + w.C <= v.coff))
        a, b = v.buf, w.buf
        return not (a.offset + a.items <= b.offset or b.offset + b.items <= a.offset)

    @classmethod
    def _independent(cls, s, t):
        for o in s.outs.values():
            if any(cls._values_overlap(o, v) for v in list(t.ins.values()) + list(t.outs.values())):
                return False
        for o in t.outs.values():
            if any(cls._values_overlap(o, v) for v in s.ins.values()):
                return False
        return True

    def _pair_skinny_convs(self, stream_ptr):
        if not self.plan.rules.pair_convs:
            return
        lib = self.lib

        def skinny(k):
            fn, args, st = self.calls[k]
            if fn is not lib.dh_conv2d_f32 or k in self.noop_calls or st.kind != 'conv':
                return False
            ca = args[0]._obj
            return not ca.x_resample and ca.N * ca.OH * ca.OW <= self.GROUP_MAX_ROWS and lib.dh_conv2d_uses_split_k(args[0]) == 1

        i = self.npre
        while i < len(self.calls) - 1:
            if not skinny(i):
                i += 1
                continue
            fa, aa, sa = self.calls[i]
            passed, npassed = [], 0
            for k in range(i + 1, len(self.calls)):
                fk, ak, sk = self.calls[k]
                if sk.stream != sa.stream or k in self.noop_calls:
                    continue
                if sk.wait or npassed > self.PAIR_LOOKAHEAD:
                    break
                if skinny(k) and self._independent(sa, sk) and all(self._independent(q, sk) for q in passed) and \
                        lib.dh_conv2d_pair_f32(aa[0], ak[0], stream_ptr) == 0:
                    self._absorb(i, k, lib.dh_conv2d_pair_f32)
                    self.paired.append((i, k))
                    break
                passed.append(sk)
                npassed += 1
                if k in self.absorbed:
                    passed.append(self.absorbed[k])
            i += 1

    def capture(self, stream_ptr):
        global _MULTISTREAM_GRAPHS
        lib = self.lib
        if self.plan.nstreams > 1:
            if _MULTISTREAM_GRAPHS >= MAX_MULTISTREAM_GRAPHS:
                return False
        _lib.check(lib.dh_graph_begin_capture(stream_ptr), 'graph capture begin')
        try:
            self.launch_all(stream_ptr)
        finally:
            g = C.c_void_p()
            rc = lib.dh_graph_end_capture(stream_ptr, C.byref(g))
        _lib.check(rc, 'graph capture end')
        self.graph = g
        if self.plan.nstreams > 1:
            _MULTISTREAM_GRAPHS += 1
        return True

    def replay(self, stream_ptr):
        _lib.check(self.lib.dh_graph_launch(self.graph, stream_ptr), 'graph launch')

    @staticmethod
    def _conv_signature(step):
        a, x, y = step.attrs, step.ins['x'], step.outs['y']
        r1, r2 = step.ins.get('res1'), step.ins.get('res2')
        align = (x.coff % 4, y.coff % 4, r1.coff % 4 if r1 is not None else 0, r2.coff % 4 if r2 is not None else 0,
                 r1.ld % 4 if r1 is not None else 0, r2.ld % 4 if r2 is not None else 0)
        return (x.lead(3), x.shape[-3], x.shape[-2], x.C, x.ld, y.ld, a['Cout'], a['kh'], a['kw'], a['sh'],
                a['sw'], a['pre_relu'], a['post_relu'], a['up2'], 'res1' in step.ins, 'res2' in step.ins,
                'pre_bn' in step.params, 'post_bn' in step.params or 'post_affine' in step.params, a['pt'], a['pl'], y.shape[-3], y.shape[-2], a.get('res2_down', 0), 'ypool' in step.outs) + align

    def autotune(self, stream_ptr, table=None, reps=3):
        lib = self.lib
        table = {} if table is None else table
        ncfgs = {'conv': lib.dh_conv2d_num_tile_cfgs()}
        e0, e1 = C.c_void_p(), C.c_void_p()
        _lib.check(lib.dh_event_create(C.byref(e0)))
        _lib.check(lib.dh_event_create(C.byref(e1)))
        for i, (fn, args, step) in enumerate(self.calls):
            if step.kind not in ncfgs:
                continue
            if fn is lib.dh_conv2d_seg_f32:
                step.attrs['tile_cfg'] = -1
                step.attrs['split_k'] = True
                continue
            ncfg = ncfgs[step.kind]
            cargs = args[0]._obj
            sig = (self.n, step.kind) + self._conv_signature(step) + ((('u8',) if cargs.x_u8 else ())) + \
                ((({1: 'bf16x3', 2: 'halo', 3: 'bf16x2', 4: 'bf16', 5: 'bf16x3', 6: 'bf16x2', 7: 'bf16'}[cargs.w_split],) if cargs.w_split else ()))
            if cargs.w_split:
                ncfg = lib.dh_conv2d_num_halo_tile_cfgs() if cargs.w_split == 2 else lib.dh_conv2d_num_split_tile_cfgs()
            if step.kind == 'conv' and lib.dh_conv2d_uses_split_k(args[0]):
                step.attrs['tile_cfg'] = -1
                step.attrs['split_k'] = True
                self.calls[i] = (fn, (args[0], -1), step)
                continue
            if step.kind == 'conv' and lib.dh_conv2d_uses_first_layer_kernel(args[0]):
                step.attrs['tile_cfg'] = -1
                step.attrs['first_layer'] = True
                self.calls[i] = (fn, (args[0], -1), step)
                continue
            shape_key = ('shape', int(cargs.w_split), self.n, cargs.N * cargs.OH * cargs.OW, cargs.K, cargs.Cout, cargs.KH,
                         cargs.KW, cargs.up2)
            if sig not in table:
                def time_cfg(cfg, nrep, trials):
                    t_cfg = float('inf')
                    for _trial in range(trials):
                        _lib.check(lib.dh_event_record(e0, stream_ptr))
                        for _ in range(nrep):
                            fn(args[0], cfg, stream_ptr)
                        _lib.check(lib.dh_event_record(e1, stream_ptr))
                        _lib.check(lib.dh_event_synchronize(e1))
                        ms = C.c_float()
                        _lib.check(lib.dh_event_elapsed_ms(e0, e1, C.byref(ms)))
                        t_cfg = min(t_cfg, ms.value / nrep)
                    return t_cfg
                timed = {}
                for cfg in range(ncfg):
                    if fn(args[0], cfg, stream_ptr) != 0:
                        continue
                    timed[cfg] = time_cfg(cfg, reps, 2)
                best = -1
                if timed:
                    lo = min(timed.values())
                    close = [c for c, t in timed.items() if t <= 1.08 * lo]
                    if len(close) > 1:
                        for c in close:
                            timed[c] = time_cfg(c, 4 * reps, 3)
                        best = min(close, key=lambda c: timed[c])
                        pref = table.get(shape_key)
                        if pref in close and timed[pref] <= 1.01 * timed[best]:
                            best = pref
                    else:
                        best = close[0]
                table[sig] = best
                table.setdefault(shape_key, best)
            step.attrs['tile_cfg'] = table[sig]
            self.calls[i] = (fn, (args[0], table[sig]), step)
        lib.dh_event_destroy(e0)
        lib.dh_event_destroy(e1)
        self._drop_graph()
        return table

    def profile(self, stream_ptr, reps=1):
        lib = self.lib
        evs = []
        for _ in range(len(self.calls) + 1):
            e = C.c_void_p()
            _lib.check(lib.dh_event_create(C.byref(e)))
            evs.append(e)
        times = np.zeros(len(self.calls))
        for _ in range(reps):
            _lib.check(lib.dh_event_record(evs[0], stream_ptr))
            for i, (fn, args, step) in enumerate(self.calls):
                _lib.check(fn(*args, stream_ptr), step.kind)
                _lib.check(lib.dh_event_record(evs[i + 1], stream_ptr))
            _lib.check(lib.dh_event_synchronize(evs[-1]))
            for i in range(len(self.calls)):
                ms = C.c_float()
                _lib.check(lib.dh_event_elapsed_ms(evs[i], evs[i + 1], C.byref(ms)))
                times[i] += ms.value
        for e in evs:
            lib.dh_event_destroy(e)
        return times / reps

    def _drop_graph(self):
        if self.graph is not None:
            if self.plan.nstreams > 1:
                _GRAPH_GRAVEYARD.append(self.graph)
            else:
                self.lib.dh_graph_destroy(self.graph)
            self.graph = None

    def __del__(self):
        try:
            self._drop_graph()
        except Exception:
            pass


def _noop_launch(*_args):
    return 0


_GRAPH_GRAVEYARD = []
_MULTISTREAM_GRAPHS = 0
MAX_MULTISTREAM_GRAPHS = max(0, int(os.environ.get('DEEPHAR_MAX_MULTISTREAM_GRAPHS', '64')))
_ROLE_STREAMS = {}
_ROLE_LOCKS = {}


def stream_lock(device, role):
    import threading
    torch = _torch()
    device = torch.device(device)
    key = (device.index if device.index is not None else torch.cuda.current_device(), role)
    lk = _ROLE_LOCKS.get(key)
    if lk is None:
        lk = _ROLE_LOCKS.setdefault(key, threading.RLock())
    return lk


def shared_stream(device, role):
    torch = _torch()
    device = torch.device(device)
    key = (device.index if device.index is not None else torch.cuda.current_device(), role)
    st = _ROLE_STREAMS.get(key)
    if st is None:
        with torch.cuda.device(device):
            for r in ('compute', 'copy', 'head', 'comm'):
                k = (key[0], r)
                if k not in _ROLE_STREAMS:
                    _ROLE_STREAMS[k] = torch.cuda.Stream(device=device)
        st = _ROLE_STREAMS.get(key)
        if st is None:
            with torch.cuda.device(device):
                st = _ROLE_STREAMS[key] = torch.cuda.Stream(device=device)
    return st


_STAGING_THREADS = max(1, min(8, (os.cpu_count() or 2) // 2, int(os.environ.get('DEEPHAR_STAGING_THREADS', '6'))))
_POOL = None


def _staging_pool():
    global _POOL
    if _POOL is None:
        from concurrent.futures import ThreadPoolExecutor
        _POOL = ThreadPoolExecutor(max_workers=_STAGING_THREADS, thread_name_prefix='deephar-staging')
    return _POOL


class Executor:
    def __init__(self, plan, device=None, use_graph=True, autotune=True, stream_role='compute'):
        torch = _torch()
        if not torch.cuda.is_available():
            raise _lib.DeepharHipError('no HIP device visible: deephar_amd runs only on an AMD GPU (gfx950); '
                                       'there is no CPU execution path')
        _lib.load()
        self.device = torch.device(device or 'cuda:%d' % torch.cuda.current_device())
        self.plan = plan
        self.use_graph = use_graph
        self.autotune = autotune
        self.tune_table = {}
        self.store = WeightStore(self.device)
        self.bound = {}
        self.max_bound = max(1, int(os.environ.get('DEEPHAR_MAX_BOUND_PLANS', '4')))
        self._wstamp = None
        self.stream = shared_stream(self.device, stream_role)
        self._lock = stream_lock(self.device, stream_role)

    @property
    def stream_ptr(self):
        return self.stream.cuda_stream

    def bind(self, n, u8_norm=None):
        with self._lock:
            return self._bind_locked(n, u8_norm)

    def _bind_locked(self, n, u8_norm=None):
        key = n if u8_norm is None else (n, repr(u8_norm))
        bp = self.bound.get(key)
        if bp is None:
            torch = _torch()
            with torch.cuda.device(self.device), torch.cuda.stream(self.stream):
                bp = BoundPlan(self.plan, n, self.store, self.device, u8_norm=u8_norm)
                if self.autotune:
                    bp.autotune(self.stream_ptr, self.tune_table)
                bp.group_launches(self.stream_ptr)
            self.bound[key] = bp
            while len(self.bound) > self.max_bound:
                old = next(iter(self.bound))
                if old == key:
                    break
                del self.bound[old]
        else:
            self.bound[key] = self.bound.pop(key)
        return bp

    def _weight_stamp(self):
        return sum(p.version for p in self.plan.params)

    def sync_weights(self):
        stamp = self._weight_stamp()
        if self._wstamp is None:
            self._wstamp = stamp
        elif stamp != self._wstamp:
            self.refresh_weights()

    def refresh_weights(self):
        torch = _torch()
        self._wstamp = self._weight_stamp()
        with torch.cuda.device(self.device), torch.cuda.stream(self.stream):
            for s in self.plan.steps:
                for role, p in s.params.items():
                    if role == 'w' and s.kind == 'convtranspose':
                        for (pid, key) in [k_ for k_ in self.store.conv if k_[0] == id(p)]:
                            self.store.convt_weight(p, split=key[1] if isinstance(key, tuple) else 0)
                    elif role == 'w' and s.kind != 'dwconv':
                        for (pid, split) in [k_ for k_ in self.store.conv if k_[0] == id(p)]:
                            self.store.conv_weight(p, split=split)
                    elif role == 'w':
                        self.store.dw_weight(p)
                    elif role == 'dw':
                        self.store.dw_weight(p)
                    else:
                        self.store.bn_affine(p)
        self.stream.synchronize()

    def set_inputs(self, bp, arrays):
        torch = _torch()
        for v, arr in zip(self.plan.inputs, arrays):
            if bp.u8 is not None:
                dst = bp.u8[id(v.buf)][0]
                src = torch.from_numpy(np.ascontiguousarray(arr)) if isinstance(arr, np.ndarray) else arr
                if src.dtype != torch.uint8 or tuple(src.shape[1:]) != tuple(dst.shape[1:]) or src.shape[0] > bp.n:
                    raise ValueError('uint8-bound plan expects uint8 input [<=%d, %s], got %s %s' %
                                     (bp.n, tuple(dst.shape[1:]), src.dtype, tuple(src.shape)))
                dst[:src.shape[0]].copy_(src.to(self.device, non_blocking=True))
                continue
            dst = bp.tensor(v)
            if isinstance(arr, np.ndarray):
                src = torch.from_numpy(np.ascontiguousarray(arr))
            else:
                src = arr
            m = src.shape[0]
            if tuple(src.shape[1:]) != tuple(dst.shape[1:]) or m > bp.n:
                raise ValueError('input has shape %s, model expects [<=%d, %s]' % (tuple(src.shape), bp.n,
                                                                                  tuple(dst.shape[1:])))
            dst[:m].copy_(src.to(self.device, non_blocking=True).to(torch.float32))

    def forward(self, bp):
        with self._lock:
            return self._forward_locked(bp)

    def _forward_locked(self, bp):
        if self.use_graph and (bp.graph is not None or bp.capture(self.stream_ptr)):
            bp.replay(self.stream_ptr)
        else:
            bp.launch_all(self.stream_ptr)

    def run(self, arrays, n=None, u8_norm=None):
        return self.run_pipelined(arrays, n or arrays[0].shape[0], u8_norm=u8_norm)

    def _io(self, bp, depth):
        io = getattr(bp, '_io', None)
        if io is None:
            io = bp._io = dict(host_in=[], dev_in=[], host_out=[], h2d=[], done=[], pending=[])
        torch = _torch()
        dt = torch.uint8 if bp.u8 is not None else torch.float32
        while len(io['host_in']) < depth:
            io['host_in'].append([torch.empty((bp.n,) + v.shape, dtype=dt, pin_memory=True) for v in self.plan.inputs])
            io['dev_in'].append([torch.empty((bp.n,) + v.shape, dtype=dt, device=self.device) for v in self.plan.inputs])
            io['host_out'].append(torch.empty(max(self.plan.out_items * bp.n, 4), dtype=torch.float32, pin_memory=True))
            io['h2d'].append(torch.cuda.Event())
            io['done'].append(torch.cuda.Event())
            io['pending'].append(None)
        return io

    def _host_outputs(self, bp, flat, m):
        torch = _torch()
        outs = []
        for v in self.plan.outputs:
            shape = (bp.n,) + v.shape
            strides = [1] * len(shape)
            if len(shape) >= 2:
                strides[-2] = v.ld
                for i in range(len(shape) - 3, -1, -1):
                    strides[i] = strides[i + 1] * shape[i + 1]
            view = torch.as_strided(flat, shape, strides, v.buf.offset * bp.n + v.coff)
            outs.append(np.array(view[:m].numpy(), dtype=np.float32, copy=True, order='C'))
        return outs

    def run_pipelined(self, arrays, bs, u8_norm=None, verbose=0):
        with self._lock:
            return self._run_pipelined_locked(arrays, bs, u8_norm, verbose)

    def _run_pipelined_locked(self, arrays, bs, u8_norm=None, verbose=0):
        torch = _torch()
        total = arrays[0].shape[0]
        bs = int(min(bs, total))
        nchunks = (total + bs - 1) // bs
        with torch.cuda.device(self.device):
            if self.bound:
                self.sync_weights()
            with torch.cuda.stream(self.stream):
                bp = self.bind(bs, u8_norm=u8_norm)
            if self._wstamp is None:
                self._wstamp = self._weight_stamp()
            if getattr(self, 'copy_stream', None) is None:
                self.copy_stream = shared_stream(self.device, 'copy')
            want = torch.uint8 if bp.u8 is not None else torch.float32
            slot_bytes = sum(bs * int(np.prod(v.shape)) for v in self.plan.inputs) * (1 if want == torch.uint8 else 4)
            depth = max(2, min(nchunks, int(os.environ.get('DEEPHAR_PREDICT_DEPTH', '8')),
                               max(2, (512 << 20) // max(slot_bytes, 1))))
            io = self._io(bp, depth)
            io['pending'] = [None] * len(io['pending'])
            results = []
            ahead = min(2, depth - 1)
            pool = _staging_pool()
            staged = {}

            def collect(slot):
                m = io['pending'][slot]
                if m is not None:
                    io['done'][slot].synchronize()
                    results.append(self._host_outputs(bp, io['host_out'][slot], m))
                    io['pending'][slot] = None

            def stage(ci):
                slot, start = ci % depth, ci * bs
                collect(slot)
                m = min(bs, total - start)
                on_dev, dev_src, futs = [], [], []
                for k, (v, arr) in enumerate(zip(self.plan.inputs, arrays)):
                    part = arr[start:start + m]
                    if tuple(part.shape[1:]) != tuple(v.shape):
                        raise ValueError('input has shape %s, model expects [N, %s]' % (tuple(arr.shape), tuple(v.shape)))
                    src = torch.from_numpy(np.ascontiguousarray(part)) if isinstance(part, np.ndarray) else part
                    if (src.dtype == torch.uint8) != (want == torch.uint8):
                        raise ValueError('plan bound for %s inputs, got %s' % (want, src.dtype))
                    on_dev.append(bool(src.is_cuda))
                    dev_src.append(src if src.is_cuda else None)
                    if not src.is_cuda:
                        dst = io['host_in'][slot][k]
                        nsl = max(1, min(_STAGING_THREADS, src.numel() * src.element_size() >> 22, m))
                        step = -(-m // nsl)
                        for a0 in range(0, m, step):
                            a1 = min(a0 + step, m)
                            futs.append(pool.submit(dst[a0:a1].copy_, src[a0:a1]))
                return m, on_dev, dev_src, futs

            try:
                for ci in range(min(ahead, nchunks)):
                    staged[ci] = stage(ci)
                for ci in range(nchunks):
                    if ci + ahead < nchunks:
                        staged[ci + ahead] = stage(ci + ahead)
                    slot = ci % depth
                    m, on_dev, dev_src, futs = staged.pop(ci)
                    for fu in futs:
                        fu.result()
                    with torch.cuda.stream(self.copy_stream):
                        if any(on_dev):
                            self.copy_stream.wait_stream(torch.cuda.current_stream())
                        for k in range(len(arrays)):
                            src = dev_src[k] if on_dev[k] else io['host_in'][slot][k][:m]
                            io['dev_in'][slot][k][:m].copy_(src, non_blocking=True)
                        io['h2d'][slot].record(self.copy_stream)
                    with torch.cuda.stream(self.stream):
                        self.stream.wait_event(io['h2d'][slot])
                        for k, v in enumerate(self.plan.inputs):
                            dst = bp.u8[id(v.buf)][0] if bp.u8 is not None else bp.tensor(v)
                            dst[:m].copy_(io['dev_in'][slot][k][:m], non_blocking=True)
                        self.forward(bp)
                        io['host_out'][slot].copy_(bp.arena[:io['host_out'][slot].numel()], non_blocking=True)
                        io['done'][slot].record(self.stream)
                    io['pending'][slot] = m
                    if verbose:
                        print('%d/%d' % (min((ci + 1) * bs, total), total))
                for k in range(depth):
                    collect((nchunks + k) % depth)
            finally:
                for _, _, _, futs in staged.values():
                    for fu in futs:
                        fu.cancel() or fu.exception()
                if any(p is not None for p in io['pending']):
                    self.stream.synchronize()
                    io['pending'] = [None] * len(io['pending'])
        nres = len(self.plan.outputs)
        return [np.concatenate([r[k] for r in results], axis=0) if len(results) > 1 else results[0][k]
                for k in range(nres)]

    def run_device(self, tensors, n=None, inputs_copied=None):
        with self._lock:
            return self._run_device_locked(tensors, n, inputs_copied)

    def _run_device_locked(self, tensors, n=None, inputs_copied=None):
        torch = _torch()
        m = tensors[0].shape[0]
        n = n or m
        with torch.cuda.device(self.device), torch.cuda.stream(self.stream):
            if self.bound:
                self.sync_weights()
            bp = self.bind(n)
            if self._wstamp is None:
                self._wstamp = self._weight_stamp()
            for v, t in zip(self.plan.inputs, tensors):
                dst = bp.tensor(v)[:m] if m <= bp.n else None
                if dst is None or t.shape[0] != m or t.numel() != dst.numel() or \
                        tuple(t.shape[-1:]) != tuple(v.shape[-1:]):
                    raise ValueError('input has shape %s, model expects [<=%d, %s]' % (tuple(t.shape), bp.n, v.shape))
                if tuple(t.shape) != tuple(dst.shape):
                    dst = dst.view(tuple(t.shape))
                dst.copy_(t, non_blocking=True)
            if inputs_copied is not None:
                inputs_copied.record(self.stream)
            self.forward(bp)
            return [bp.tensor(v)[:m] for v in self.plan.outputs]
```

### deephar_amd/engine/planner.py

```python
import os

import numpy as np

from .. import graph as G
from .rules import RuleSet


class Buf:
    def __init__(self, items, kind='act'):
        self.items = int(items)
        self.kind = kind
        self.start = None
        self.end = None
        self.offset = None
        self.pinned = False


class Value:

    def __init__(self, shape, buf, coff=0, ld=None):
        self.shape = tuple(shape)
        self.buf = buf
        self.coff = coff
        self.ld = self.shape[-1] if ld is None else ld
# ... 80 lines not shown
        self.params = params or {}
        self.name = name

    def flops(self, n=1):
        a = self.attrs
        if self.kind == 'conv':
            y = self.outs['y']
            m = y.npix // (4 if a.get('up2') else 1)
            return 2.0 * n * m * a['K'] * a['Cout']
        if self.kind == 'convtranspose':
            return 2.0 * n * self.outs['y'].npix * a['K'] * a['Cout']
        if self.kind == 'dwconv':
            y = self.outs['y']
            return 2.0 * n * y.npix * y.C * a['kh'] * a['kw']
        if self.kind == 'kronecker':
            return 2.0 * n * self.ins['x'].npix * self.ins['hm'].C * self.ins['x'].C
        return 0.0

    def bytes(self, n=1):
        tot = 0
        for v in list(self.ins.values()) + list(self.outs.values()):
            if v is not None:
                tot += v.npix * v.C
        return 4.0 * n * tot


class Plan:
    def __init__(self):
        self.steps = []
        self.inputs = []
        self.outputs = []
        self.bufs = []
        self.arena_items = 0
        self.out_items = 0
        self.params = []
        self.nstreams = 1
        self.gemm_precision = 'f32'
        self.gemm_scope = 'standard'
        self.rules = RuleSet()

    @property
    def split_adds(self):
        return self.rules.split_adds

    def total_flops(self, n=1):
        return sum(s.flops(n) for s in self.steps)



class _Lazy:

    def __init__(self, base, bn=None, relu=False):
        self.base = base
        self.bn = bn
        self.relu = relu


class _UpView:

    def __init__(self, low, shape):
        self.low, self.shape, self.full = low, tuple(shape), None


class _PoolView:

    def __init__(self, base, shape, attrs):
        self.base, self.shape, self.attrs, self.full = base, tuple(shape), dict(attrs), None


class Planner:
    def __init__(self, inputs, outputs, nstreams=1, stream_policy='list', rules=RuleSet()):
        self.rules = rules
        self.nstreams = nstreams
        self.stream_policy = stream_policy
        self.producer = {}
        self.g_inputs = inputs
        self.g_outputs = outputs
        self.nodes = G.topo_nodes(outputs)
        if self.rules.split_adds:
            self.nodes = self._split_wide_adds(self.nodes, outputs)
        self.plan = Plan()
        self.plan.rules = self.rules
        self.val = {}
        self.absorbed = set()
        self.consumers = {}
        for n in self.nodes:
            for i, t in enumerate(n.inputs):
                self.consumers.setdefault(t.uid, []).append((n, i))
        self.out_uids = {}
        for t in outputs:
            self.out_uids[t.uid] = self.out_uids.get(t.uid, 0) + 1
        self.concat_val = {}
        self.processed = set()
        self.deferred = {}

    @staticmethod
    def _split_wide_adds(nodes, outputs):
        index = {n.uid: i for i, n in enumerate(nodes)}
        readers = {}
        for n in nodes:
            for t in n.inputs:
                readers[t.uid] = readers.get(t.uid, 0) + 1
        for t in outputs:
            readers[t.uid] = readers.get(t.uid, 0) + 1
        insert_after, replace = {}, {}
        for n in nodes:
            if n.op != 'add' or len(n.inputs) < 4 or len({t.uid for t in n.inputs}) != len(n.inputs):
                continue
            prods = [t for t in n.inputs if t.node is not None and t.node.op in ('conv', 'sepconv') and
                     t.node.uid in index and readers.get(t.uid, 0) == 1]
            if not prods:
                continue
            prods.sort(key=lambda t: index[t.node.uid])
            others = [t for t in n.inputs if all(t.uid != q.uid for q in prods)]
            pos = lambda t: index[t.node.uid] if t.node is not None and t.node.uid in index else -1
            partial = None
            for k, p in enumerate(prods):
                last = k == len(prods) - 1
                take = [partial] if partial is not None else []
                ready = [t for t in others if pos(t) < index[p.node.uid]]
                while len(take) < 2 and ready:
                    take.append(ready.pop(0))
                others = [t for t in others if all(t.uid != q.uid for q in take)]
                ins = [p] + take + (others if last else [])
                if not last and len(ins) == 1:
                    others.append(p)
                    continue
                node = G.Node('add', ins, [n.outputs[0].shape], name=(n.name or 'add') + ('' if last else '/part%d' % k))
                if last:
                    node.outputs = [n.outputs[0]]
                    replace[n.uid] = node
                else:
                    insert_after.setdefault(p.node.uid, []).append(node)
                partial = node.outputs[0]
        if not replace:
            return nodes
        out = []
        for n in nodes:
            out.append(replace.get(n.uid, n))
            out.extend(insert_after.get(n.uid, []))
        return out

    def new_buf(self, shape, kind='act'):
        items = int(np.prod(shape))
        items = (items + 3) // 4 * 4
        b = Buf(items, kind)
        self.plan.bufs.append(b)
        return b

    def new_value(self, shape):
        return Value(shape, self.new_buf(shape))

    def n_consumers(self, t):
        return len(self.consumers.get(t.uid, [])) + self.out_uids.get(t.uid, 0)

    def sole_consumer(self, t, op=None):
        if self.out_uids.get(t.uid, 0):
            return None
        cs = self.consumers.get(t.uid, [])
        if len(cs) != 1:
            return None
        n = cs[0][0]
        if op is not None and n.op != op:
            return None
        return n

    def emit(self, kind, ins, outs, attrs=None, params=None, name=None):
        s = Step(kind, ins, outs, attrs, params, name)
        self.plan.steps.append(s)
        for v in outs.values():
            if v is not None:
                self.producer[id(v)] = s
        return s

    def available(self, t):
        return t.uid in self.val

    def materialize(self, t):
        v = self.val[t.uid]
        if isinstance(v, _UpView):
            v = self.val[t.uid] = self._realize_up(v)
        if isinstance(v, _PoolView):
            v = self.val[t.uid] = self._realize_pool(v)
        if isinstance(v, _Lazy) and isinstance(v.base, _UpView):
            v = _Lazy(self._realize_up(v.base), bn=v.bn, relu=v.relu)
        if isinstance(v, _Lazy) and isinstance(v.base, _PoolView):
            v = _Lazy(self._realize_pool(v.base), bn=v.bn, relu=v.relu)
        if isinstance(v, _Lazy):
            out = self.new_value(v.base.shape)
            self.emit('eltwise', dict(a=v.base), dict(y=out), dict(op=0, relu=int(v.relu)),
                      dict(bn=v.bn) if v.bn is not None else {}, name='materialize')
            self.val[t.uid] = out
            return out
        return v

    def lazy_or_value(self, t):
        return self.val[t.uid]

    def _realize_up(self, uv):
        if uv.full is None:
            uv.full = self.new_value(uv.shape)
            self.emit('upsample_add', dict(b=uv.low), dict(y=uv.full), name='upsample')
        return uv.full

    def _realize_pool(self, pv):
        if pv.full is None:
            pv.full = self.new_value(pv.shape)
            self.emit('pool', dict(x=pv.base), dict(y=pv.full), dict(pv.attrs), name='pool')
        return pv.full

    def _skinny_conv_node(self, n, cin):
        a, shape = n.attrs, n.outputs[0].shape
        return n.op == 'conv' and len(shape) >= 3 and (a.get('sh', 1), a.get('sw', 1)) == (1, 1) and \
            split_k_rule(shape[-3] * shape[-2], a['kh'] * a['kw'] * cin, a['filters'], cin, a['kh'], a['kw'])

    def _only_reader_through_bn_relu(self, t):
        while True:
            if self.out_uids.get(t.uid, 0):
                return None
            cs = self.consumers.get(t.uid, [])
            if len(cs) != 1:
                return None
            n = cs[0][0]
            if n.op not in ('bn', 'relu'):
                return n
            t = n.outputs[0]

    def _virtual_upsample_ok(self, node):
        t = node.outputs[0]
        if not self.rules.up_commute or len(t.shape) < 3 or node.attrs.get('size', (2, 2)) != (2, 2):
            return False
        seen, stack, ends = set(), [t], 0
        while stack:
            x = stack.pop()
            if self.out_uids.get(x.uid, 0):
                return False
            for n, _ in self.consumers.get(x.uid, []):
                if n.op in ('bn', 'relu'):
                    if n.uid not in seen:
                        seen.add(n.uid)
                        stack.append(n.outputs[0])
                elif n.op == 'conv' and (n.attrs['kh'], n.attrs['kw'], n.attrs.get('sh', 1), n.attrs.get('sw', 1)) == (1, 1, 1, 1):
                    ends += 1
                elif self._skinny_conv_node(n, t.shape[-1]) and self.rules.resample_on_load:
                    ends += 1
                elif n.op == 'sepconv' and (n.attrs.get('sh', 1), n.attrs.get('sw', 1)) == (1, 1):
                    ends += 1
                else:
                    return False
        return ends > 0

    _VIEW_READERS = ('softmax2d', 'jointprob', 'globalmax2d')

    def _concat_home(self, t):
        cat = self.sole_consumer(t, 'concat')
        if cat is not None or self.out_uids.get(t.uid, 0) or not self.rules.concat_shared:
            return cat
        cs = [n for n, _ in self.consumers.get(t.uid, [])]
        cats = [n for n in cs if n.op == 'concat']
        if len(cats) != 1 or any(n.op not in self._VIEW_READERS for n in cs if n.op != 'concat'):
            return None
        return cats[0]

    def out_value_for(self, t, shape=None):
        shape = shape or t.shape
        cat = self._concat_home(t)
        if cat is not None and all(len(x.shape) == len(shape) for x in cat.inputs):
            cv = self.concat_val.get(cat.uid)
            if cv is None:
                target = self.out_value_for(cat.outputs[0])
                cv = target
                self.concat_val[cat.uid] = cv
            off = 0
            for x in cat.inputs:
                if x.uid == t.uid:
                    break
                off += x.shape[-1]
            if sum(1 for x in cat.inputs if x.uid == t.uid) == 1:
                return Value(shape, cv.buf, cv.coff + off, cv.ld)
        return self.new_value(shape)

    def run(self):
        for t in self.g_inputs:
            v = Value(t.shape, self.new_buf(t.shape, 'input'))
            self.val[t.uid] = v
            self.plan.inputs.append(v)
        for node in self.nodes:
            if node.uid in self.absorbed:
                continue
            if node.op in ('conv', 'sepconv') and self._defer_for_upsampled_residual(node):
                continue
            getattr(self, 'op_' + node.op)(node)
            self.processed.add(node.uid)
            self._flush_deferred()
        assert not self.deferred, 'deferred convolutions never became ready'
        for t in self.g_outputs:
            v = self.materialize(t)
            v.buf.pinned = True
            self.plan.outputs.append(v)
        self._merge_sibling_pointwise()
        self._merge_siblings_into_joint_buffers()
        self._merge_sibling_pools()
        self._pool_into_segmented_conv()
        self._collect_params()
        from . import schedule
        schedule.finalize(self.plan, self.nstreams, self.stream_policy)
        return self.plan

    def _merge_sibling_pointwise(self):
        if not self.rules.merge_heads:
            return
        same = ('sh', 'sw', 'Cin', 'pre_relu', 'post_relu', 'up2', 'res2_down')

        def mergeable(a, b):
            if a.kind != 'conv' or b.kind != 'conv' or set(a.ins) != {'x'} or set(b.ins) != {'x'} or \
                    set(a.outs) != {'y'} or set(b.outs) != {'y'}:
                return False
            if any(a.attrs.get(k) != b.attrs.get(k) for k in same) or \
                    a.attrs['up2'] or a.attrs['res2_down'] or a.attrs.get('sh', 1) != 1 or a.attrs.get('sw', 1) != 1:
                return False
            pointwise = all(st.attrs['kh'] == 1 and st.attrs['kw'] == 1 for st in (a, b))
            if not pointwise:
                for st in (a, b):
                    if st.attrs['kh'] % 2 == 0 or st.attrs['kw'] % 2 == 0 or st.attrs['pt'] != st.attrs['kh'] // 2 or \
                            st.attrs['pl'] != st.attrs['kw'] // 2 or st.attrs['Cin'] % 16 == 0:
                        return False
                if not self.rules.merge_kxk:
                    return False
                cin = a.attrs['Cin']
                shapes = [q.shape[:2] for st in (a, b)
                          for q in (st.params['w'].parts if isinstance(st.params['w'], ConcatParam) else [st.params['w']])]
                KH, KW = max(h for h, _ in shapes), max(w_ for _, w_ in shapes)
                if cin not in (2, 3) and not all(kxk_window_keeps_k_order(h, w_, KH, KW, cin) for h, w_ in shapes):
                    return False
            if set(a.params) - {'w', 'pre_bn'} or set(b.params) - {'w', 'pre_bn'} or \
                    a.params.get('pre_bn') is not b.params.get('pre_bn'):
                return False
            xa, xb, ya, yb = a.ins['x'], b.ins['x'], a.outs['y'], b.outs['y']
            if xa.buf is not xb.buf or (xa.coff, xa.ld, xa.shape) != (xb.coff, xb.ld, xb.shape):
                return False
            if ya.buf is not yb.buf or ya.ld != yb.ld or ya.shape[:-1] != yb.shape[:-1] or ya.coff + ya.C != yb.coff:
                return False
            px = ya.shape[-3] * ya.shape[-2] if len(ya.shape) >= 3 else 1
            kh, kw = max(a.attrs['kh'], b.attrs['kh']), max(a.attrs['kw'], b.attrs['kw'])
            fam = lambda st, c, h, w_: split_k_rule(px, h * w_ * st.attrs['Cin'], c, st.attrs['Cin'], h, w_)
            whole = fam(a, ya.C + yb.C, kh, kw)
            if whole and not pointwise:
                return False
            return fam(a, ya.C, a.attrs['kh'], a.attrs['kw']) == fam(b, yb.C, b.attrs['kh'], b.attrs['kw']) == whole

        steps = self.plan.steps
        i = 0
        while i + 1 < len(steps):
            a = steps[i]
            j = next((j for j in range(i + 1, min(i + 8, len(steps))) if mergeable(a, steps[j]) or mergeable(steps[j], a)), None)
            if j is None:
                i += 1
                continue
            b = steps[j]
            first, second = (a, b) if mergeable(a, b) else (b, a)
            ya, yb = first.outs['y'], second.outs['y']
            y = Value(ya.shape[:-1] + (ya.C + yb.C,), ya.buf, ya.coff, ya.ld)
            parts = []
            for st in (first, second):
                w = st.params['w']
                parts += w.parts if isinstance(w, ConcatParam) else [w]
            wcat = ConcatParam(parts)
            params = dict(first.params, w=wcat)
            attrs = dict(first.attrs, Cout=ya.C + yb.C, kh=wcat.kh, kw=wcat.kw, pt=wcat.kh // 2, pl=wcat.kw // 2,
                         K=wcat.kh * wcat.kw * first.attrs['Cin'])
            if (wcat.kh, wcat.kw) == (1, 1):
                attrs.update(pt=first.attrs['pt'], pl=first.attrs['pl'])
            merged = Step('conv', dict(first.ins), dict(y=y), attrs, params, '%s+%s' % (first.name, second.name))
            del steps[j]
            steps[i] = merged
            for v in (ya, yb, y):
                self.producer[id(v)] = merged

    def _merge_siblings_into_joint_buffers(self):
        if not self.rules.merge_siblings:
            return
        steps = self.plan.steps

        def plain(st):
            return st.kind == 'conv' and set(st.ins) == {'x'} and set(st.outs) == {'y'} and \
                (st.attrs['kh'], st.attrs['kw'], st.attrs.get('sh', 1), st.attrs.get('sw', 1)) == (1, 1, 1, 1) and \
                not st.attrs['up2'] and not st.attrs['res2_down'] and not (set(st.params) - {'w', 'pre_bn', 'post_bn'})

        def readers(buf):
            return [(q, role, v) for q in steps for role, v in q.ins.items() if v is not None and v.buf is buf]

        def family(st, c):
            y = st.outs['y']
            px = y.shape[-3] * y.shape[-2] if len(y.shape) >= 3 else 1
            return split_k_rule(px, st.attrs['K'], c, st.attrs['Cin'])

        def compatible(a, b):
            if not plain(a) or not plain(b) or a.params.get('pre_bn') is not b.params.get('pre_bn') or \
                    a.attrs['pre_relu'] != b.attrs['pre_relu'] or a.attrs['Cin'] != b.attrs['Cin']:
                return False
            xa, xb, ya, yb = a.ins['x'], b.ins['x'], a.outs['y'], b.outs['y']
            if xa.buf is not xb.buf or (xa.coff, xa.ld, xa.shape) != (xb.coff, xb.ld, xb.shape):
                return False
            if ya.buf is yb.buf or ya.shape[:-1] != yb.shape[:-1] or ya.buf.pinned or yb.buf.pinned:
                return False
            for st in (a, b):
                y = st.outs['y']
                if y.coff != 0 or y.ld != y.C or y.buf.items != (int(np.prod(y.shape)) + 3) // 4 * 4:
                    return False
                if any(v is not None and v.buf is y.buf for q in steps if q is not st for v in q.outs.values()):
                    return False
            if not (family(a, ya.C) and family(b, yb.C) and family(a, ya.C + yb.C)):
                return False
            for st in (a, b):
                for q, role, v in readers(st.outs['y'].buf):
                    if q.kind not in ('conv', 'sam'):
                        return False
            if a.attrs['post_relu'] != b.attrs['post_relu']:
                st = a if a.attrs['post_relu'] else b
                for q, role, v in readers(st.outs['y'].buf):
                    if q.kind != 'conv' or role != 'x' or 'pre_bn' in q.params:
                        return False
            return True

        def key(st):
            x = st.ins['x']
            return (id(x.buf), x.coff, x.ld, x.shape, id(st.params.get('pre_bn')), st.attrs['pre_relu'])

        i = 0
        while i + 1 < len(steps):
            a = steps[i]
            j = None
            if plain(a):
                ka = key(a)
                j = next((j for j in range(i + 1, len(steps)) if plain(steps[j]) and key(steps[j]) == ka and
                          compatible(a, steps[j])), None)
            if j is None:
                i += 1
                continue
            b = steps[j]
            ya, yb = a.outs['y'], b.outs['y']
            ca, cb = ya.C, yb.C
            post_relu = int(a.attrs['post_relu'] and b.attrs['post_relu'])
            if a.attrs['post_relu'] != b.attrs['post_relu']:
                st = a if a.attrs['post_relu'] else b
                for q, role, v in readers(st.outs['y'].buf):
                    q.attrs['pre_relu'] = 1
            joint = self.new_buf(ya.shape[:-1] + (ca + cb,))
            for old, base in ((ya.buf, 0), (yb.buf, ca)):
                for q in steps:
                    for v in list(q.ins.values()) + list(q.outs.values()):
                        if v is not None and v.buf is old:
                            v.buf, v.coff, v.ld = joint, v.coff + base, ca + cb
                self.plan.bufs.remove(old)
            parts = []
            for st in (a, b):
                w = st.params['w']
                parts += w.parts if isinstance(w, ConcatParam) else [w]
            params = dict(w=ConcatParam(parts))
            if 'pre_bn' in a.params:
                params['pre_bn'] = a.params['pre_bn']
            if 'post_bn' in a.params or 'post_bn' in b.params:
                params['post_affine'] = ConcatAffine([(ca, a.params.get('post_bn')), (cb, b.params.get('post_bn'))])
            y = Value(ya.shape[:-1] + (ca + cb,), joint, 0, ca + cb)
            merged = Step('conv', dict(a.ins), dict(y=y), dict(a.attrs, Cout=ca + cb, post_relu=post_relu), params,
                          '%s+%s' % (a.name, b.name))
            del steps[j]
            steps[i] = merged
            for v in (ya, yb, y):
                self.producer[id(v)] = merged

    def _merge_sibling_pools(self):
        if not self.rules.merge_pools:
            return
        steps = self.plan.steps

        def sole_buffer(st):
            x = st.ins['x']
            if x.coff != 0 or x.ld != x.C or x.buf.pinned or x.buf.kind != 'act' or \
                    x.buf.items != (int(np.prod(x.shape)) + 3) // 4 * 4:
                return False
            writers = [q for q in steps for v in q.outs.values() if v is not None and v.buf is x.buf]
            readers = [q for q in steps for v in q.ins.values() if v is not None and v.buf is x.buf]
            return len(writers) == 1 and readers == [st] and writers[0].kind == 'conv' and \
                writers[0].outs.get('y') is not None and writers[0].outs['y'].buf is x.buf and \
                all(v.coff == 0 and v.ld == x.C for v in writers[0].outs.values() if v is not None and v.buf is x.buf)

        i = 0
        while i < len(steps):
            a = steps[i]
            j = None
            if a.kind == 'pool' and sole_buffer(a):
                xa, ya = a.ins['x'], a.outs['y']
                for jj in range(i + 1, len(steps)):
                    b = steps[jj]
                    if b.kind != 'pool' or b.attrs != a.attrs:
                        continue
                    xb, yb = b.ins['x'], b.outs['y']
                    if yb.buf is ya.buf and yb.ld == ya.ld and yb.coff == ya.coff + ya.C and yb.shape[:-1] == ya.shape[:-1] and \
                            xb.shape[:-1] == xa.shape[:-1] and xb.buf is not xa.buf and sole_buffer(b) and \
                            not any(v is not None and v.buf is ya.buf for q in steps[i + 1:jj] for v in q.ins.values()):
                        j = jj
                        break
            if j is None:
                i += 1
                continue
            b = steps[j]
            xb, yb = b.ins['x'], b.outs['y']
            ca, cb = xa.C, xb.C
            joint = self.new_buf(xa.shape[:-1] + (ca + cb,))
            for old, base in ((xa.buf, 0), (xb.buf, ca)):
                for q in steps:
                    for v in list(q.ins.values()) + list(q.outs.values()):
                        if v is not None and v.buf is old:
                            v.buf, v.coff, v.ld = joint, v.coff + base, ca + cb
                self.plan.bufs.remove(old)
            x = Value(xa.shape[:-1] + (ca + cb,), joint, 0, ca + cb)
            y = Value(ya.shape[:-1] + (ya.C + yb.C,), ya.buf, ya.coff, ya.ld)
            merged = Step('pool', dict(x=x), dict(y=y), dict(a.attrs), {}, '%s+%s' % (a.name, b.name))
            steps[j] = merged
            del steps[i]
            for v in (ya, yb, y):
                self.producer[id(v)] = merged

    def _pool_into_segmented_conv(self):
        if not self.rules.pool_segments:
            return
        steps = self.plan.steps
        i = 0
        while i < len(steps):
            p = steps[i]
            i += 1
            a = p.attrs
            if p.kind != 'pool' or a.get('mode', 0) != 0 or (a['kh'], a['kw'], a['sw'], a['pt'], a['pl']) != (2, 2, 2, 0, 0) or \
                    a['sh'] not in (1, 2):
                continue
            x, y = p.ins['x'], p.outs['y']
            if len(x.shape) < 3 or x.coff != 0 or x.ld != x.C or x.buf.pinned or y.coff != 0 or y.buf.pinned or x.C % 4 or \
                    x.shape[-2] != 2 * y.shape[-2] or x.shape[-3] != a['sh'] * y.shape[-3]:
                continue
            if any(v is not None and v.buf is x.buf for q in steps if q is not p for v in q.ins.values()):
                continue
            readers = [(q, r) for q in steps for r, v in q.ins.items() if v is not None and v.buf is y.buf]
            if len(readers) != 1 or readers[0][1] != 'x':
                continue
            q = readers[0][0]
            cx = q.ins['x']
            qa = q.attrs
            if q.kind != 'conv' or qa.get('x_resample') or qa.get('up2') or qa.get('res2_down') or 'ypool' in q.outs or \
                    cx.coff != 0 or cx.ld != y.ld or cx.C < y.C or cx.shape[:-1] != y.shape[:-1] or qa['Cin'] != cx.C:
                continue
            oy = q.outs['y']
            if not split_k_rule(oy.shape[-3] * oy.shape[-2] if len(oy.shape) >= 3 else 1, qa['K'], qa['Cout'], qa['Cin'], qa['kh'],
                                qa['kw']):
                continue
            others = [v for w in steps if w is not p for v in w.outs.values() if v is not None and v.buf is y.buf]
            if any(v.coff < y.C or v.ld != y.ld for v in others) or (cx.C > y.C) != bool(others) or (cx.C - y.C) % 4:
                continue
            q.ins['x'] = x
            if cx.C > y.C:
                q.ins['x2'] = Value(cx.shape[:-1] + (cx.C - y.C,), y.buf, y.C, y.ld)
            qa['seg'] = dict(c_split=y.C, pool_sh=a['sh'])
            steps.remove(p)
            i -= 1

    def _upsampled_residual(self, t):
        a2 = self.sole_consumer(t, 'add')
        if a2 is None or len(a2.inputs) != 2 or len(t.shape) < 3 or not self.rules.res2_down:
            return None
        other = [x for x in a2.inputs if x.uid != t.uid]
        if len(other) != 1:
            return None
        up = next((n for n in self.nodes if n.op == 'upsample' and n.outputs[0].uid == other[0].uid), None)
        if up is None or self.sole_consumer(up.outputs[0], 'add') is not a2:
            return None
        b = up.inputs[0]
        if tuple(b.shape[:-3]) != tuple(t.shape[:-3]) or b.shape[-1] != t.shape[-1] or t.shape[-3] % 2 or \
                t.shape[-2] % 2 or (b.shape[-3], b.shape[-2]) != (t.shape[-3] // 2, t.shape[-2] // 2):
            return None
        return a2, up, b

    def _epilogue_tail(self, out_t):
        t, chain = out_t, []
        n = self.sole_consumer(t, 'bn')
        if n is not None:
            t = n.outputs[0]
            chain.append(n)
        if self.sole_consumer(t, 'relu') is not None:
            return None, chain
        n = self.sole_consumer(t, 'add')
        if n is not None:
            others = [x for x in n.inputs if x.uid != t.uid]
            if len(others) == len(n.inputs) - 1 and len(others) == 1 and all(self.available(x) for x in others):
                return n.outputs[0], chain + [n]
            if self._upsampled_residual(t) is None:
                return None, chain
        return t, chain

    def _defer_for_upsampled_residual(self, node):
        if not all(self.available(x) for x in node.inputs):
            return False
        if self._node_is_skinny(node):
            return False
        t, chain = self._epilogue_tail(node.outputs[0])
        hit = self._upsampled_residual(t) if t is not None else None
        if hit is None or self.available(hit[2]):
            return False
        self.deferred.setdefault(hit[2].uid, []).append(node)
        self.absorbed.update(n.uid for n in chain + [hit[0], hit[1]])
        return True
# ... 597 lines not shown
```

### deephar_amd/engine/schedule.py

```python
from collections import defaultdict

import numpy as np


def _ranges_overlap(a, b):
    return a[0] < b[1] and b[0] < a[1]


def _step_cost_us(step):
    return max(step.flops(64) / 100e12, step.bytes(64) / 3e12) * 1e6 + 5.0


def compute_deps(plan):
    writers = defaultdict(list)
    readers = defaultdict(list)
    deps = []
    for j, s in enumerate(plan.steps):
        d = set()
        for v in s.ins.values():
            if v is None:
                continue
            r = (v.coff, v.coff + v.C)
            for (wr, i) in writers[id(v.buf)]:
                if _ranges_overlap(r, wr):
                    d.add(i)
        for v in s.outs.values():
            if v is None:
                continue
            r = (v.coff, v.coff + v.C)
            for (wr, i) in writers[id(v.buf)]:
                if _ranges_overlap(r, wr):
                    d.add(i)
            for (rr, i) in readers[id(v.buf)]:
                if _ranges_overlap(r, rr):
                    d.add(i)
        d.discard(j)
        deps.append(sorted(d))
        for v in s.ins.values():
            if v is not None:
                readers[id(v.buf)].append(((v.coff, v.coff + v.C), j))
        for v in s.outs.values():
            if v is not None:
                writers[id(v.buf)].append(((v.coff, v.coff + v.C), j))
    return deps


def assign_streams(plan, deps, nstreams):
    n = len(plan.steps)
    stream = [0] * n
    if nstreams <= 1 or n == 0:
        return stream
    consumers = defaultdict(list)
    for j, d in enumerate(deps):
        for i in d:
            consumers[i].append(j)
    cost = [_step_cost_us(s) for s in plan.steps]
    down = [0.0] * n
    for i in range(n - 1, -1, -1):
        down[i] = cost[i] + max((down[j] for j in consumers[i]), default=0.0)
    tail = [-1] * nstreams
    for j in range(n):
        cands = [s for s in range(nstreams) if tail[s] >= 0 and tail[s] in deps[j]]
        chosen = None
        for s in sorted(cands, key=lambda s: -tail[s]):
            t = tail[s]
            rival = max((down[k] for k in consumers[t] if k > j and stream_unassigned(k, j)), default=-1.0)
            if rival <= down[j]:
                chosen = s
                break
        if chosen is None:
            if j == 0:
                chosen = 0
            else:
                free = [s for s in range(nstreams) if s not in cands]
                pool = free if free else list(range(nstreams))
                chosen = min(pool, key=lambda s: tail[s])
        stream[j] = chosen
        tail[chosen] = j
    return stream


def stream_unassigned(k, j):
    return k > j


def assign_streams_tail(plan, deps, items=2, nstreams=2, floor_us=30.0, shift=0):
    import heapq
    n = len(plan.steps)
    stream, order = [0] * n, list(range(n))
    if n < 8:
        return stream, order
    cost = [floor_us + max(st.flops(items) / 90e12, st.bytes(items) / 3e12) * 1e6 for st in plan.steps]
    consumers = [[] for _ in range(n)]
    for j, d in enumerate(deps):
        for i in d:
            consumers[i].append(j)
    fin0 = [0.0] * n
    t = 0.0
    for i in range(n):
        t += cost[i]
        fin0[i] = t
    serial = t

    def simulate(s, chain=None, bound=float('inf')):
        indeg = [0] * n
        ready_at = [0.0] * n
        heaps = ([], [])
        which = (lambda j: 1 if chain is not None and j in chain else 0)
        for j in range(s, n):
            for i in deps[j]:
                if i >= s:
                    indeg[j] += 1
                else:
                    ready_at[j] = max(ready_at[j], fin0[i])
            if indeg[j] == 0:
                heapq.heappush(heaps[which(j)], (ready_at[j], j))
        clock, placed = [0.0, 0.0], {}
        while heaps[0] or heaps[1]:
            cand = [(max(clock[q], heaps[q][0][0]), q) for q in (0, 1) if heaps[q]]
            _, q = min(cand)
            r, j = heapq.heappop(heaps[q])
            start = max(clock[q], r)
            clock[q] = start + cost[j]
            if clock[q] >= bound:
                return bound, None
            placed[j] = (start, 1 + q)
            for k in consumers[j]:
                ready_at[k] = max(ready_at[k], clock[q])
                indeg[k] -= 1
                if indeg[k] == 0:
                    heapq.heappush(heaps[which(k)], (ready_at[k], k))
        return max(fin0[s - 1], clock[0], clock[1]), placed

    best_s, best, best_placed = 0, serial, None
    spans = {}
    for s in range(1, n):
        span, placed = simulate(s)
        spans[s] = span
        if span < best:
            best_s, best, best_placed = s, span, placed
    if best_s == 0 or best > 0.95 * serial:
        return stream, order
    if shift:
        best_s = min(max(best_s + shift, 1), n - 1)
        best, best_placed = simulate(best_s)
    if nstreams >= 3:
        descendants = {}

        def cone(x):
            if x not in descendants:
                chain, stack = {x}, [x]
                while stack:
                    for k in consumers[stack.pop()]:
                        if k not in chain:
                            chain.add(k)
                            stack.append(k)
                descendants[x] = chain
            return descendants[x]
        for s in sorted(spans, key=spans.get)[:24]:
            for x in range(s, n):
                chain = cone(x)
                if len(chain) < 8 or len(chain) > (n - s) - 8:
                    continue
                span, placed = simulate(s, chain, bound=best)
                if placed is not None and span < 0.97 * best:
                    best, best_placed = span, placed
    start = [fin0[i] - cost[i] for i in range(n)]
    for j, (st_, q) in best_placed.items():
        start[j] = st_
        stream[j] = q
    order = sorted(range(n), key=lambda j: (start[j], j))
    return [stream[j] for j in order], order


def happens_before(n, deps, stream):
    succ = [[] for _ in range(n)]
    for j, d in enumerate(deps):
        for i in d:
            succ[i].append(j)
    last = {}
    for j in range(n):
        s = stream[j]
        if s in last:
            succ[last[s]].append(j)
        last[s] = j
    reach = [0] * n
    for i in range(n - 1, -1, -1):
        m = 0
        for j in succ[i]:
            m |= (1 << j) | reach[j]
        reach[i] = m
    return reach


def allocate(plan, reach):
    n = len(plan.steps)
    acc = defaultdict(list)
    for j, s in enumerate(plan.steps):
        for v in list(s.ins.values()) + list(s.outs.values()):
            if v is not None and j not in acc[id(v.buf)]:
                acc[id(v.buf)].append(j)
    full = (1 << n) - 1
    info = {}
    for b in plan.bufs:
        steps = acc.get(id(b), [])
        mask = 0
        for j in steps:
            mask |= 1 << j
        after_all = full
        for j in steps:
            after_all &= reach[j]
        info[id(b)] = (steps, mask, after_all)
        b.start = min(steps) if steps else 0
        b.end = max(steps) if steps else n
        if b.kind == 'input':
            b.start = -1
        if b.pinned or not steps:
            b.end = n

    def ordered(x, y):
        if x.pinned or y.kind == 'input':
            return False
        sx, mx, after_x = info[id(x)]
        sy, my, _ = info[id(y)]
        if not sx or not sy:
            return False
        return (my & ~after_x) == 0

    placed = []
    off = 0
    for b in plan.bufs:
        if b.pinned:
            b.offset = off
            off += b.items
            placed.append(b)
    plan.out_items = off
    for b in sorted(plan.bufs, key=lambda b: -b.items):
        if b.pinned:
            continue
        spans = sorted((p.offset, p.offset + p.items) for p in placed if not (ordered(p, b) or ordered(b, p)))
        off = 0
        for lo, hi in spans:
            if off + b.items <= lo:
                break
            off = max(off, hi)
        b.offset = off
        placed.append(b)
    plan.arena_items = max((b.offset + b.items for b in plan.bufs), default=0)


def finalize(plan, nstreams=1, policy='list'):
    deps = compute_deps(plan)
    if policy == 'tail' and nstreams >= 2:
        stream, order = assign_streams_tail(plan, deps, nstreams=nstreams, floor_us=plan.rules.tail_floor_us,
                                            shift=plan.rules.tail_shift)
        if order != list(range(len(order))):
            plan.steps[:] = [plan.steps[j] for j in order]
            deps = compute_deps(plan)
    else:
        stream = assign_streams(plan, deps, nstreams)
    n = len(plan.steps)
    reach = happens_before(n, deps, stream)
    waited = {}
    for j, s in enumerate(plan.steps):
        s.stream = stream[j]
        s.deps = deps[j]
        newest = {}
        for i in deps[j]:
            if stream[i] != stream[j]:
                newest[stream[i]] = max(newest.get(stream[i], -1), i)
        s.wait = []
        for src, i in sorted(newest.items()):
            if waited.get((stream[j], src), -1) < i:
                s.wait.append(i)
                waited[(stream[j], src)] = i
    needs_event = set(i for s in plan.steps for i in s.wait)
    for j, s in enumerate(plan.steps):
        s.record = j in needs_event
    plan.nstreams = max(stream) + 1 if n else 1
    allocate(plan, reach)
    return plan
```

### deephar_amd/engine/serialize.py

```python
import ctypes as C
import struct

import numpy as np

from .. import _lib

MAGIC, VERSION = b'DHPL', 2
FUNCTIONS = ['dh_conv2d_f32', 'dh_dwconv2d_f32', 'dh_pool2d_f32', 'dh_upsample2x_add_f32', 'dh_eltwise_f32',
             'dh_softargmax2d_f32', 'dh_context_aggregation_f32', 'dh_depth_means_f32', 'dh_softargmax1d_f32',
             'dh_kronecker_f32', 'dh_global_maxmin_softmax_f32', 'dh_copy_channels_f32', 'dh_zeropad2d_f32',
             'dh_depth_from_maps_f32', 'dh_softargmax2d_context_f32', 'dh_normalize_u8_f32', 'dh_conv2d_dw_group_f32',
             'dh_conv2d_pair_f32', 'dh_conv2d_seg_f32', 'dh_dwconv2d_strided_f32', 'dh_conv2d_transpose2x2_f32']
V3_FUNCTIONS = FUNCTIONS.index('dh_dwconv2d_strided_f32')
V4_FUNCTIONS = ['dh_conv2d_transpose2x2_split_f32']
ALL_FUNCTIONS = FUNCTIONS + V4_FUNCTIONS
ARENA, WEIGHTS, BYTES = 1, 2, 3


class _Regions:
    def __init__(self, bp):
        self.base = bp.base
        self.end = bp.base + bp.arena.numel() * 4
        st = bp.store
        tensors = [e[0] for e in st.conv.values()] + [e[0] for e in st.dw.values()] + list(st.const.values())
        for e in st.bn.values():
            tensors += [e[0], e[1]]
        self.known = sorted(((t.data_ptr(), t.data_ptr() + t.numel() * t.element_size(), t) for t in tensors),
                            key=lambda r: r[0])
        self.offset = {}
        self.image = []
        self.size = 0
        self.u8 = []
        self.u8_size = 0
        for buf, _, _ in (bp.u8 or {}).values():
            self.u8.append((buf.data_ptr(), buf.data_ptr() + buf.numel(), self.u8_size))
            self.u8_size = (self.u8_size + buf.numel() + 255) & ~255

    def tag(self, ptr):
        ptr = int(ptr or 0)
        if ptr == 0:
            return 0
        if self.base <= ptr < self.end:
            return (ARENA << 60) | (ptr - self.base)
        for lo, hi, off in self.u8:
            if lo <= ptr < hi:
                return (BYTES << 60) | (off + ptr - lo)
        for lo, hi, t in self.known:
            if lo <= ptr < hi:
                if lo not in self.offset:
                    self.size = (self.size + 255) & ~255
                    self.offset[lo] = self.size
                    self.image.append((self.size, t))
                    self.size += hi - lo
                return (WEIGHTS << 60) | (self.offset[lo] + ptr - lo)
        raise ValueError('pointer 0x%x belongs neither to the arena nor to the weight store' % ptr)


def _is_ptr_type(t):
    return t is C.c_void_p


def _scalars(sig, args, reg):
    assert len(sig) == len(args), (len(sig), len(args))
    parts = []
    for t, a in zip(sig, args):
        if _is_ptr_type(t):
            parts.append(struct.pack('<Q', reg.tag(a)))
        elif t is C.c_float:
            parts.append(struct.pack('<fI', float(a), 0))
        else:
            parts.append(struct.pack('<q', int(a)))
    return b''.join(parts)


def blob_version(function_ids):
    top = max(function_ids, default=0)
    return 4 if top >= len(FUNCTIONS) else (3 if top >= V3_FUNCTIONS else VERSION)


def dump_plan(model, batch, u8_norm=None):
    ex = model.executor
    torch = __import__('torch')
    with torch.cuda.device(ex.device), torch.cuda.stream(ex.stream):
        if ex.bound:
            ex.sync_weights()
        bp = ex.bind(batch, u8_norm=u8_norm)
    ex.stream.synchronize()
    lib = _lib.load()
    names = {n: i for i, n in enumerate(ALL_FUNCTIONS)}
    by_addr = {C.cast(getattr(lib, n), C.c_void_p).value: n for n in ALL_FUNCTIONS}
    reg = _Regions(bp)
    steps = []
    for idx, (fn, args, step) in enumerate(bp.calls):
        if idx in bp.noop_calls:
            continue
        name = by_addr.get(C.cast(fn, C.c_void_p).value)
        if name is None:
            raise ValueError('step %s (%s) has no serialised form' % (step.kind, step.name))
        sig = _lib.SIGNATURES[name][1][:-1]
        if len(sig) and isinstance(getattr(sig[0], '_type_', None), type) and issubclass(sig[0]._type_, C.Structure):
            payload, nstruct = b'', 0
            while nstruct < len(sig) and isinstance(getattr(sig[nstruct], '_type_', None), type) and \
                    issubclass(sig[nstruct]._type_, C.Structure):
                obj = args[nstruct]._obj
                raw = bytearray(bytes(obj))
                for fname, ftype in obj._fields_:
                    if _is_ptr_type(ftype):
                        off = getattr(type(obj), fname).offset
                        raw[off:off + 8] = struct.pack('<Q', reg.tag(getattr(obj, fname)))
                payload += bytes(raw)
                nstruct += 1
            payload += _scalars(sig[nstruct:], args[nstruct:], reg)
        else:
            payload = _scalars(sig, args, reg)
        steps.append(struct.pack('<II', names[name], len(payload)) + payload)
    plan = bp.plan
    version = blob_version(struct.unpack_from('<I', st)[0] for st in steps)
    head = MAGIC + struct.pack('<IiQQIIIQ', version, bp.n, bp.arena.numel() * 4, (reg.size + 255) & ~255,
                               len(plan.inputs), len(plan.outputs), len(steps), reg.u8_size)
    ins = b''
    for v in plan.inputs:
        if bp.u8 is not None:
            ins += struct.pack('<QQII', reg.tag(bp.u8[id(v.buf)][0].data_ptr()), int(np.prod(v.shape)), 1, 0)
        else:
            ins += struct.pack('<QQII', reg.tag(bp.ptr(v)), int(np.prod(v.shape)), 0, 0)
    outs = b''
    for v in plan.outputs:
        if v.coff % 1 or v.ld < v.C:
            raise ValueError('output view not serialisable')
        outs += struct.pack('<QQII', bp.ptr(v) - bp.base, v.npix, v.C, v.ld)
    image = bytearray((reg.size + 255) & ~255)
    for off, t in reg.image:
        b = t.detach().cpu().contiguous().numpy().tobytes()
        image[off:off + len(b)] = b
    return head + ins + outs + b''.join(steps) + bytes(image)
```

### include/deephar_hip.h

```cpp
#ifndef DEEPHAR_HIP_H_
#define DEEPHAR_HIP_H_

#include <stddef.h>
#include <stdint.h>

#ifdef __cplusplus
extern "C" {
#endif

#define DH_OK 0
#define DH_EINVAL (-1)
#define DH_EUNSUPPORTED (-2)
#define DH_ELAUNCH (-3)

int dh_version(void);
const char* dh_error_string(int rc);
int dh_device_info(int dev, char* arch_name, int arch_name_len, int* cu_count);

typedef struct dh_conv_args {
  const float* x;
  const float* w;
  float* y;
  const float* pre_scale;
  const float* pre_shift;
  const float* post_scale;
  const float* post_shift;
  const float* res1;
  const float* res2;
  const float* in_lut;
  int32_t N, H, W, Cin, ldx;
  int32_t OH, OW, Cout, ldy;
  int32_t KH, KW, SH, SW, PT, PL;
  int32_t K;
  int32_t Kp, Np;
  int32_t ldr1, ldr2;
  int32_t pre_relu, post_relu;
  int32_t up2;
  int32_t x_u8;
  int32_t w_split;
  int32_t res2_down;
  int32_t ldyp;
  int32_t x_resample;
  float* y_pool;
} dh_conv_args;

int dh_conv2d_packed_dims(int KH, int KW, int Cin, int Cout, int* Kp, int* Np);
int dh_conv2d_pack_weights_host(const float* w_hwio_host, float* packed_host, int KH, int KW, int Cin,
                                int Cout);
int dh_conv2d_pack_weights_split_host(const float* w_hwio_host, uint16_t* packed_host, int KH, int KW, int Cin,
                                      int Cout);
int dh_conv2d_pack_weights_parts_host(const float* w_hwio_host, uint16_t* packed_host, int KH, int KW, int Cin,
                                      int Cout, int parts);
int dh_conv2d_num_tile_cfgs(void);
int dh_conv2d_num_split_tile_cfgs(void);
int dh_conv2d_pick_tile_cfg(int M, int Cout);
int dh_conv2d_uses_split_k(const dh_conv_args* a);
int dh_conv2d_uses_first_layer_kernel(const dh_conv_args* a);
int dh_conv2d_split_eligible(const dh_conv_args* a);
int dh_conv2d_split_wide_eligible(const dh_conv_args* a);
int dh_conv2d_halo_eligible(const dh_conv_args* a);
int dh_conv2d_num_halo_tile_cfgs(void);
int dh_conv2d_f32(const dh_conv_args* a, int tile_cfg, void* stream);

int dh_normalize_u8_f32(const uint8_t* x, const float* lut, float* y, int64_t n_pixels, int C, void* stream);

typedef struct dh_dw_args {
  const float* x;
  const float* w;
  float* y;
  const float* pre_scale;
  const float* pre_shift;
  int32_t N, H, W, C, ldx, ldy;
  int32_t KH, KW, PT, PL;
  int32_t pre_relu;
  int32_t up_in;
} dh_dw_args;
int dh_dwconv2d_f32(const dh_dw_args* a, void* stream);

typedef struct dh_dw_strided {
  const float* x;
  const float* w;
  float* y;
  const float* pre_scale;
  const float* pre_shift;
  int32_t N, H, W, C, ldx, ldy;
  int32_t OH, OW;
  int32_t KH, KW, SH, SW, PT, PL;
  int32_t pre_relu;
  int32_t reserved;
} dh_dw_strided;
int dh_dwconv2d_strided_f32(const dh_dw_strided* a, void* stream);

typedef struct dh_conv_transpose {
  const float* x;
  const float* w;
  float* y;
  const float* pre_scale;
  const float* pre_shift;
  const float* res;
  int32_t N, H, W, Cin, ldx;
  int32_t Cout, ldy, ldr;
  int32_t Kp, Np;
  int32_t pre_relu, post_relu;
} dh_conv_transpose;
int dh_conv2d_transpose2x2_num_tile_cfgs(void);
int dh_conv2d_transpose2x2_f32(const dh_conv_transpose* a, int tile_cfg, void* stream);
int dh_conv2d_transpose2x2_num_split_tile_cfgs(void);
int dh_conv2d_transpose2x2_split_eligible(const dh_conv_transpose* a);
int dh_conv2d_transpose2x2_split_f32(const dh_conv_transpose* a, int parts, int tile_cfg, void* stream);

int dh_conv2d_dw_group_f32(const dh_conv_args* conv, const dh_dw_args* dw, void* stream);

typedef struct dh_conv_seg {
  const float* x2;
  int32_t ldx2;
  int32_t c_split;
  int32_t pool_sh;
  int32_t reserved;
} dh_conv_seg;
int dh_conv2d_seg_f32(const dh_conv_args* a, const dh_conv_seg* seg, void* stream);

int dh_conv2d_pair_f32(const dh_conv_args* a, const dh_conv_args* b, void* stream);

typedef struct dh_pool_args {
  const float* x;
  float* y;
  int32_t N, H, W, C, ldx;
  int32_t OH, OW, ldy;
  int32_t KH, KW, SH, SW, PT, PL;
  int32_t mode;
} dh_pool_args;
int dh_pool2d_f32(const dh_pool_args* a, void* stream);

int dh_upsample2x_add_f32(const float* a, int lda, const float* b, int ldb, float* y, int ldy, int N, int H,
                          int W, int C, void* stream);

typedef struct dh_elt_args {
  const float* a;
  const float* b;
  const float* c;
  float* y;
  const float* scale;
  const float* shift;
  int32_t lda, ldb, ldc, ldy;
  int64_t npix;
  int32_t C;
  int32_t relu;
  int32_t op;
  int32_t bcast_b;
} dh_elt_args;
int dh_eltwise_f32(const dh_elt_args* a, void* stream);

typedef struct dh_sam_args {
  const float* h;
  const float* gx;
  const float* gy;
  float* xy;
  float* conf_raw;
  float* conf_prob;
  float* prob;
  float* gmax;
  int32_t F, H, W, C, ldh, ldxy, ldcr, ldcp, ldp;
  float alpha;
  float conf_scale;
  int32_t xy_times_conf;
} dh_sam_args;
int dh_softargmax2d_f32(const dh_sam_args* a, void* stream);

int dh_softargmax2d_context_f32(const dh_sam_args* a, int J, int nctx, float agg_alpha, float* y, int ldy,
                                void* stream);

int dh_context_aggregation_f32(const float* ys, const float* yc, const float* pc, float* y, int F, int J,
                               int nctx, float alpha, int ldy, void* stream);

int dh_depth_means_f32(const float* h, int ldh, float* hxy, float* hz, int F, int HW, int D, int J,
                       void* stream);
int dh_softargmax1d_f32(const float* hz, const float* grid, float* z, int ldz, float* vz, int F, int D, int J,
                        void* stream);

int dh_kronecker_f32(const float* hm, int ldh, const float* x, int ldx, float* f, int ldf, int B, int P, int J,
                     int C, void* stream);

int dh_global_maxmin_softmax_f32(const float* x, int ldx, float* y, int B, int P, int C, int softmax,
                                 void* stream);

int dh_copy_channels_f32(const float* x, int ldx, float* y, int ldy, int64_t npix, int C, void* stream);
int dh_zeropad2d_f32(const float* x, float* y, int B, int H, int W, int C, int OH, int OW, int PT, int PL,
                     void* stream);

int dh_depth_from_maps_f32(const float* d, int ldd, const float* h, int ldh, float* z, int ldz, int F, int HW,
                           int J, void* stream);

typedef struct dh_plan dh_plan;
int dh_plan_create(const void* blob, size_t blob_bytes, dh_plan** plan_out);
int dh_plan_destroy(dh_plan* plan);
int dh_plan_batch(const dh_plan* plan);
int dh_plan_num_inputs(const dh_plan* plan);
int dh_plan_num_outputs(const dh_plan* plan);
int64_t dh_plan_input_items(const dh_plan* plan, int i);
int dh_plan_input_is_u8(const dh_plan* plan, int i);
int64_t dh_plan_output_items(const dh_plan* plan, int i);
int dh_forward(dh_plan* plan, const float* const* inputs_dev, int m, float* const* outputs_dev, void* stream);
int dh_forward_host(dh_plan* plan, const float* const* inputs_host, int m, float* const* outputs_host);

int dh_graph_begin_capture(void* stream);
int dh_graph_end_capture(void* stream, void** graph_exec_out);
int dh_graph_launch(void* graph_exec, void* stream);
int dh_graph_destroy(void* graph_exec);

int dh_event_create(void** event_out);
int dh_event_record(void* event, void* stream);
int dh_event_synchronize(void* event);
int dh_event_elapsed_ms(void* start, void* stop, float* ms_out);
int dh_event_destroy(void* event);
int dh_stream_synchronize(void* stream);
int dh_stream_create(void** stream_out);
int dh_stream_destroy(void* stream);
int dh_event_create_sync(void** event_out);
int dh_stream_wait_event(void* stream, void* event);
int dh_stream_spin_us(void* stream, int us);

#ifdef __cplusplus
}
#endif
#endif
```

Baseline: 5130 frames/s.

## Fuse pointwise conv with following depthwise conv in a chained kernel

Adds a kernel that runs a 1x1 GEMM tile and then, in the same block, runs the depthwise convolution on the just-produced output tile from LDS-staged data. This removes a separate launch and the extra round trip of the intermediate through memory for 8x8 and 16x16 feature maps. The planner hoists depthwise steps to sit right after their producing conv, and the executor times fused against unfused at bind and keeps the fused form only when it is clearly faster. The cost is larger LDS use, the barrier-count matching needed for idle wave groups, and a new plan blob version.

```diff
diff --git a/deephar_amd/_lib.py b/deephar_amd/_lib.py
--- a/deephar_amd/_lib.py
+++ b/deephar_amd/_lib.py
@@ -81,6 +81,10 @@
     'dh_conv2d_transpose2x2_split_eligible': (C.c_int, [C.POINTER(ConvtArgs)]),
     'dh_conv2d_transpose2x2_split_f32': (C.c_int, [C.POINTER(ConvtArgs), C.c_int, C.c_int, vp]),
     'dh_conv2d_dw_group_f32': (C.c_int, [C.POINTER(ConvArgs), C.POINTER(DwArgs), vp]),
+    'dh_conv2d_dw_chain_f32': (C.c_int, [C.POINTER(ConvArgs), C.POINTER(DwArgs), vp]),
+    'dh_conv2d_dw_chain_cfg_f32': (C.c_int, [C.POINTER(ConvArgs), C.POINTER(DwArgs), C.c_int, vp]),
+    'dh_conv2d_dw_chain_eligible': (C.c_int, [C.POINTER(ConvArgs), C.POINTER(DwArgs)]),
+    'dh_conv2d_dw_chain_num_tile_cfgs': (C.c_int, []),
     'dh_conv2d_pair_f32': (C.c_int, [C.POINTER(ConvArgs), C.POINTER(ConvArgs), vp]),
     'dh_conv2d_seg_f32': (C.c_int, [C.POINTER(ConvArgs), C.POINTER(ConvSeg), vp]),
     'dh_pool2d_f32': (C.c_int, [C.POINTER(PoolArgs), vp]),
diff --git a/deephar_amd/csrc/build.py b/deephar_amd/csrc/build.py
--- a/deephar_amd/csrc/build.py
+++ b/deephar_amd/csrc/build.py
@@ -6,7 +6,7 @@
 HERE = os.path.dirname(os.path.abspath(__file__))
 ROOT = os.path.dirname(os.path.dirname(HERE))
 INCLUDE = os.path.join(ROOT, "include")
-SOURCES = ["conv_igemm.hip", "gemm1x1.hip", "convt2x2.hip", "convt2x2s.hip", "gemm1x1s.hip", "gemm1x1s_p2.hip", "gemm1x1s_p1.hip",
+SOURCES = ["conv_igemm.hip", "gemm1x1.hip", "gemm1x1_dw.hip", "gemm1x1_dw8.hip", "convt2x2.hip", "convt2x2s.hip", "gemm1x1s.hip", "gemm1x1s_p2.hip", "gemm1x1s_p1.hip",
            "gemm1x1s_ext.hip", "gemm1x1s_ext_p2.hip", "gemm1x1s_ext_p1.hip", "conv_splitk.hip", "conv_halo.hip", "conv_stem.hip", "spatial.hip", "decoder.hip",
            "capi.hip", "plan.hip"]
 HEADERS = sorted(os.path.join(HERE, f) for f in os.listdir(HERE) if f.endswith(".h")) + [os.path.join(INCLUDE, "deephar_hip.h")]
diff --git a/deephar_amd/csrc/capi.hip b/deephar_amd/csrc/capi.hip
--- a/deephar_amd/csrc/capi.hip
+++ b/deephar_amd/csrc/capi.hip
@@ -128,6 +128,18 @@
   return launch_conv_dw_group(*a, *d, S(stream));
 }
 
+int dh_conv2d_dw_chain_eligible(const dh_conv_args* a, const dh_dw_args* d) {
+  return a != nullptr && d != nullptr && conv_dw_chain_eligible(*a, *d) ? 1 : 0;
+}
+int dh_conv2d_dw_chain_num_tile_cfgs(void) { return conv_dw_chain_num_cfgs(); }
+int dh_conv2d_dw_chain_cfg_f32(const dh_conv_args* a, const dh_dw_args* d, int chain_cfg, void* stream) {
+  if (a == nullptr || d == nullptr) return DH_EINVAL;
+  return launch_conv_dw_chain(*a, *d, chain_cfg, S(stream));
+}
+int dh_conv2d_dw_chain_f32(const dh_conv_args* a, const dh_dw_args* d, void* stream) {
+  return dh_conv2d_dw_chain_cfg_f32(a, d, -1, stream);
+}
+
 static int check_skinny_args(const dh_conv_args* c) {
   if (c == nullptr || c->x == nullptr || c->w == nullptr || c->y == nullptr) return DH_EINVAL;
   if ((c->pre_scale == nullptr) != (c->pre_shift == nullptr) || (c->post_scale == nullptr) != (c->post_shift == nullptr)) return DH_EINVAL;
diff --git a/deephar_amd/csrc/dh_kernels.h b/deephar_amd/csrc/dh_kernels.h
--- a/deephar_amd/csrc/dh_kernels.h
+++ b/deephar_amd/csrc/dh_kernels.h
@@ -39,6 +39,9 @@
 bool convt2x2_split_eligible(const ConvArgs& gemm, int cb);
 int convt2x2_split_num_cfgs();
 int launch_conv_dw_group(const ConvArgs& a, const DwArgs& d, hipStream_t s);
+int launch_conv_dw_chain(const ConvArgs& a, const DwArgs& d, int cfg, hipStream_t s);
+int conv_dw_chain_num_cfgs();
+bool conv_dw_chain_eligible(const ConvArgs& a, const DwArgs& d);
 int launch_conv_skinny_pair(const ConvArgs& a, const ConvArgs& b, hipStream_t s);
 int launch_conv_splitk_seg(const ConvArgs& a, const ConvSeg& seg, hipStream_t s);
 int launch_pool(const PoolArgs& a, hipStream_t s);
diff --git a/deephar_amd/csrc/dw_lds.h b/deephar_amd/csrc/dw_lds.h
--- a/deephar_amd/csrc/dw_lds.h
+++ b/deephar_amd/csrc/dw_lds.h
@@ -46,9 +46,9 @@
 
 template <int KS, int NT, int MAXT, int MAXN, bool AFF, bool RELU>
 __device__ __forceinline__ void dwconv_lds_body(const DwArgs& p, const int tw, const int rows, const int twh_magic,
-                                                const int block, float4* dsm) {
+                                                const int block, float4* dsm, const int tid0 = 0) {
   constexpr int SP = NT / DW_CQ;
-  const int tid = threadIdx.x;
+  const int tid = threadIdx.x - tid0;
   const int chunks = p.C / 32;
   const int bands = (p.H + rows - 1) / rows;
   const int ctiles = (p.W + tw - 1) / tw;
diff --git a/deephar_amd/csrc/gemm1x1_body.h b/deephar_amd/csrc/gemm1x1_body.h
--- a/deephar_amd/csrc/gemm1x1_body.h
+++ b/deephar_amd/csrc/gemm1x1_body.h
@@ -33,9 +33,10 @@
   constexpr int BM = WM * TM * 32;
   constexpr int BN = WN * TN * 32;
   constexpr int APASS = BM * 8 / NT;
-  constexpr int BPASS = 8 * BN / NT;
+  constexpr int BPASS = (8 * BN + NT - 1) / NT;
+  constexpr bool BFULL = (8 * BN) % NT == 0;
   constexpr int STAGE = BM * BK + BK * BN;
-  static_assert(BM * 8 % NT == 0 && (8 * BN) % NT == 0, "tile/thread mismatch");
+  static_assert(BM * 8 % NT == 0 && (8 * BN) % 64 == 0, "tile/thread mismatch");
 
   const int tid = threadIdx.x;
   const int lane = tid & 63;
@@ -108,7 +109,8 @@
       }
     }
 #pragma unroll
-    for (int q = 0; q < BPASS; ++q) dma16(rs_w, sB + (q * NT + wave_u * 64) * 4, b_off[q], kt * b_step);
+    for (int q = 0; q < BPASS; ++q)
+      if (BFULL || q * NT + wave_u * 64 < 8 * BN) dma16(rs_w, sB + (q * NT + wave_u * 64) * 4, b_off[q], kt * b_step);
   };
 
   f32x16 acc[TM][TN];
diff --git a/deephar_amd/csrc/gemm1x1_dw.h b/deephar_amd/csrc/gemm1x1_dw.h
--- /dev/null
+++ b/deephar_amd/csrc/gemm1x1_dw.h
@@ -0,0 +1,85 @@
+#pragma once
+#include "dw_lds.h"
+#include "gemm1x1_body.h"
+
+namespace dh {
+
+template <int WM, int WN, int TM, int TN, bool RELU, int KS, int DNT, int MAXT, int MAXN, bool DRELU>
+__global__ __launch_bounds__(WM* WN * 64) void gemm1x1_dw_chain_kernel(const ConvArgs pc, const int epi_vec, const DwArgs pd,
+                                                                       const int tw, const int rows, const int twh_magic,
+                                                                       const int dw_lds_f4) {
+  extern __shared__ __attribute__((aligned(16))) float smem[];
+  constexpr int NT = WM * WN * 64, BM = WM * TM * 32, BN = WN * TN * 32;
+  constexpr int G = NT / DNT;
+  constexpr int CPT = BN / 32;
+  static_assert(NT % DNT == 0 && DNT % 64 == 0, "wave groups are whole waves");
+  gemm1x1_body<WM, WN, TM, TN, false, RELU>(pc, epi_vec, (int)blockIdx.x, (int)gridDim.x, smem);
+
+  const int tiles_n = (pc.Cout + BN - 1) / BN;
+  const int tile = xcd_tile((int)blockIdx.x, (int)gridDim.x);
+  const int m0 = (tile / tiles_n) * BM, n0 = (tile % tiles_n) * BN;
+
+  asm volatile("s_waitcnt vmcnt(0) lgkmcnt(0)" ::: "memory");
+  __threadfence_block();
+  __syncthreads();
+
+  const int hw = pd.H * pd.W;
+  const int fpt = BM / hw, jobs = fpt * CPT;
+  const int chunks = pd.C / 32;
+  const int group = __builtin_amdgcn_readfirstlane((int)threadIdx.x / DNT);
+  const int nbar = 2 * ((pd.H + rows - 1) / rows);
+  float4* const dsm = reinterpret_cast<float4*>(smem) + (size_t)group * dw_lds_f4;
+  for (int j0 = 0; j0 < jobs; j0 += G) {
+    const int j = j0 + group;
+    const int frame = m0 / hw + j / CPT, chunk = n0 / 32 + j % CPT;
+    if (j < jobs && frame < pd.N && chunk < chunks) {
+      dwl::dwconv_lds_body<KS, DNT, MAXT, MAXN, false, DRELU>(pd, tw, rows, twh_magic, frame * chunks + chunk, dsm, group * DNT);
+    } else {
+      for (int b = 0; b < nbar; ++b) __syncthreads();
+    }
+  }
+}
+
+template <int WM, int WN, int TM, int TN, int DNT>
+inline size_t chain_lds(size_t dw_lds) {
+  const size_t per = (dw_lds + 15) & ~(size_t)15;
+  return std::max(gemm_f32_lds(WM, WN, TM, TN, false, 0).launch, per * (size_t)(WM * WN * 64 / DNT));
+}
+
+template <int WM, int WN, int TM, int TN, bool RELU, int KS, int DNT, int MAXT, int MAXN, bool DRELU>
+int launch_chain_variant(const ConvArgs& a, int epi, const DwArgs& d, const dwl::DwLdsGeom& g, hipStream_t s) {
+  unsigned tiles;
+  if (gemm_tile_count<WM * TM * 32, WN * TN * 32>(a, &tiles) != DH_OK) return DH_EINVAL;
+  const size_t lds = chain_lds<WM, WN, TM, TN, DNT>(g.lds);
+  if (lds > 160 * 1024) return DH_EUNSUPPORTED;
+  auto kern = gemm1x1_dw_chain_kernel<WM, WN, TM, TN, RELU, KS, DNT, MAXT, MAXN, DRELU>;
+  static LdsLimit lim;
+  lim.raise((const void*)kern, 160 * 1024);
+  hipLaunchKernelGGL(kern, dim3(tiles), dim3(WM * WN * 64), lds, s, a, epi, d, g.tw, g.rows, 65536 / (g.tw + KS - 1) + 1,
+                     (int)(((g.lds + 15) & ~(size_t)15) / 16));
+  return check_launch();
+}
+
+template <int WM, int WN, int TM, int TN, int DNT>
+int launch_chain_tile(const ConvArgs& a, int epi, const DwArgs& d, const dwl::DwLdsGeom& g, hipStream_t s) {
+  if (a.y_pool != nullptr && !conv_epilogue_pools_for<WM, TM, false>(a)) return DH_EUNSUPPORTED;
+  constexpr int T5 = DNT == 256 ? 5 : 6, N5 = DNT == 256 ? 10 : 12;
+  const int sel = (a.pre_relu ? 4 : 0) | (d.KW == 5 ? 2 : 0) | (d.pre_relu ? 1 : 0);
+  switch (sel) {
+    case 0: return launch_chain_variant<WM, WN, TM, TN, false, 3, DNT, 3, 10, false>(a, epi, d, g, s);
+    case 1: return launch_chain_variant<WM, WN, TM, TN, false, 3, DNT, 3, 10, true>(a, epi, d, g, s);
+    case 2: return launch_chain_variant<WM, WN, TM, TN, false, 5, DNT, T5, N5, false>(a, epi, d, g, s);
+    case 3: return launch_chain_variant<WM, WN, TM, TN, false, 5, DNT, T5, N5, true>(a, epi, d, g, s);
+    case 4: return launch_chain_variant<WM, WN, TM, TN, true, 3, DNT, 3, 10, false>(a, epi, d, g, s);
+    case 5: return launch_chain_variant<WM, WN, TM, TN, true, 3, DNT, 3, 10, true>(a, epi, d, g, s);
+    case 6: return launch_chain_variant<WM, WN, TM, TN, true, 5, DNT, T5, N5, false>(a, epi, d, g, s);
+    default: return launch_chain_variant<WM, WN, TM, TN, true, 5, DNT, T5, N5, true>(a, epi, d, g, s);
+  }
+}
+
+constexpr int kNumChainCfgs = 3;
+constexpr int kDefaultChainCfg16 = 2, kDefaultChainCfg8 = 2;
+int launch_chain16(const ConvArgs& a, int epi, const DwArgs& d, const dwl::DwLdsGeom& g, int cfg, hipStream_t s);
+int launch_chain8(const ConvArgs& a, int epi, const DwArgs& d, const dwl::DwLdsGeom& g, int cfg, hipStream_t s);
+
+}
diff --git a/deephar_amd/csrc/gemm1x1_dw.hip b/deephar_amd/csrc/gemm1x1_dw.hip
--- /dev/null
+++ b/deephar_amd/csrc/gemm1x1_dw.hip
@@ -0,0 +1,92 @@
+#include "gemm1x1_dw.h"
+
+namespace dh {
+
+bool gemm1x1_eligible(const ConvArgs& a);
+
+namespace {
+
+struct View {
+  const void* p;
+  long long rows;
+  int ld, C;
+};
+bool views_overlap(const View& a, const View& b) {
+  if (a.p == nullptr || b.p == nullptr) return false;
+  const uintptr_t a0 = reinterpret_cast<uintptr_t>(a.p), b0 = reinterpret_cast<uintptr_t>(b.p);
+  const uintptr_t a1 = a0 + (uintptr_t)((a.rows - 1) * a.ld + a.C) * 4, b1 = b0 + (uintptr_t)((b.rows - 1) * b.ld + b.C) * 4;
+  if (a1 <= b0 || b1 <= a0) return false;
+  if (a.ld == b.ld && a.ld > 0 && (a0 & 3) == (b0 & 3)) {
+    const uintptr_t lo = a0 < b0 ? a0 : b0, hi = a0 < b0 ? b0 : a0;
+    const long long d = (long long)(((hi - lo) / 4) % (uintptr_t)a.ld);
+    const int c_lo = a0 < b0 ? a.C : b.C, c_hi = a0 < b0 ? b.C : a.C;
+    if (d >= c_lo && d + c_hi <= a.ld) return false;
+  }
+  return true;
+}
+
+}
+
+static bool chain_rule(const ConvArgs& a, const DwArgs& d, dwl::DwLdsGeom* geom) {
+  if (a.x == nullptr || a.w == nullptr || a.y == nullptr || d.x == nullptr || d.w == nullptr || d.y == nullptr) return false;
+  if ((a.pre_scale == nullptr) != (a.pre_shift == nullptr) || (a.post_scale == nullptr) != (a.post_shift == nullptr)) return false;
+  if (a.N <= 0 || a.Cin <= 0 || a.Cout <= 0 || a.OH <= 0 || a.OW <= 0 || a.ldx < a.Cin || a.ldy < a.Cout) return false;
+  if (a.Kp % BK != 0 || a.Np % 32 != 0 || a.Kp < a.K || a.Np < a.Cout || a.K != a.Cin) return false;
+  if (!conv_is_pointwise(a) || a.up2 || a.x_u8 || a.x_resample || a.w_split != 0 || a.pre_scale != nullptr) return false;
+  if (!gemm1x1_eligible(a) || conv_is_skinny(a) || conv_stem_eligible(a)) return false;
+  if (a.res2_down && (a.res2 == nullptr || (a.OH & 1) || (a.OW & 1))) return false;
+  const long long M = (long long)a.N * a.OH * a.OW;
+  if (M > 0x7fffffffLL) return false;
+  if (a.y_pool != nullptr) {
+    const int epi = (a.Cout % 4 == 0) && (a.ldy % 4 == 0) && al16(a.y) && (a.res1 == nullptr || (a.ldr1 % 4 == 0 && al16(a.res1))) &&
+                    (a.res2 == nullptr || (a.ldr2 % 4 == 0 && al16(a.res2))) &&
+                    (a.post_scale == nullptr || (al16(a.post_scale) && al16(a.post_shift)));
+    if (!epi || (a.OH & 1) || a.ldyp % 4 != 0 || a.ldyp < a.Cout || !al16(a.y_pool)) return false;
+  }
+  if (d.x != a.y || d.ldx != a.ldy || d.N != a.N || d.H != a.OH || d.W != a.OW || d.C != a.Cout || a.Cout % 32 != 0) return false;
+  if (!((a.OW == 8 && a.OH == 8) || (a.OW == 16 && a.OH == 16))) return false;
+  if (d.up_in || d.pre_scale != nullptr || d.pre_shift != nullptr || d.ldy < d.C) return false;
+  dwl::DwLdsGeom g;
+  if (!dwl::dw_lds_geometry(d, g) || g.tw != d.W || g.rows != d.H || g.nt != (d.W == 8 ? 64 : 256)) return false;
+  const View out{d.y, M, d.ldy, d.C};
+  const View others[] = {{a.x, M, a.ldx, a.Cin},
+                         {a.y, M, a.ldy, a.Cout},
+                         {a.w, 1, 0, a.Kp * a.Np},
+                         {a.res1, M, a.ldr1, a.Cout},
+                         {a.res2, a.res2_down ? M / 4 : M, a.ldr2, a.Cout},
+                         {a.y_pool, M / 4, a.ldyp, a.Cout},
+                         {a.post_scale, 1, 0, a.Cout},
+                         {a.post_shift, 1, 0, a.Cout},
+                         {d.w, 1, 0, d.KH * d.KW * d.C}};
+  for (const View& v : others)
+    if (views_overlap(out, v)) return false;
+  if (geom != nullptr) *geom = g;
+  return true;
+}
+
+bool conv_dw_chain_eligible(const ConvArgs& a, const DwArgs& d) { return chain_rule(a, d, nullptr); }
+
+int launch_chain16(const ConvArgs& a, int epi, const DwArgs& d, const dwl::DwLdsGeom& g, int cfg, hipStream_t s) {
+  switch (cfg) {
+    case 0: return launch_chain_tile<8, 1, 1, 1, 256>(a, epi, d, g, s);
+    case 1: return launch_chain_tile<8, 1, 1, 2, 256>(a, epi, d, g, s);
+    case 2: return launch_chain_tile<8, 1, 1, 3, 256>(a, epi, d, g, s);
+  }
+  return DH_EINVAL;
+}
+
+int conv_dw_chain_num_cfgs() { return kNumChainCfgs; }
+
+int launch_conv_dw_chain(const ConvArgs& a, const DwArgs& d, int cfg, hipStream_t s) {
+  dwl::DwLdsGeom g;
+  if (!chain_rule(a, d, &g)) return DH_EUNSUPPORTED;
+  if (cfg >= kNumChainCfgs) return DH_EINVAL;
+  const int epi0 = (a.Cout % 4 == 0) && (a.ldy % 4 == 0) && al16(a.y) && (a.res1 == nullptr || (a.ldr1 % 4 == 0 && al16(a.res1))) &&
+                   (a.res2 == nullptr || (a.ldr2 % 4 == 0 && al16(a.res2))) &&
+                   (a.post_scale == nullptr || (al16(a.post_scale) && al16(a.post_shift)));
+  const int epi = epi_with_direct(a, epi0);
+  if (a.OW == 16) return launch_chain16(a, epi, d, g, cfg < 0 ? kDefaultChainCfg16 : cfg, s);
+  return launch_chain8(a, epi, d, g, cfg < 0 ? kDefaultChainCfg8 : cfg, s);
+}
+
+}
diff --git a/deephar_amd/csrc/gemm1x1_dw8.hip b/deephar_amd/csrc/gemm1x1_dw8.hip
--- /dev/null
+++ b/deephar_amd/csrc/gemm1x1_dw8.hip
@@ -0,0 +1,14 @@
+#include "gemm1x1_dw.h"
+
+namespace dh {
+
+int launch_chain8(const ConvArgs& a, int epi, const DwArgs& d, const dwl::DwLdsGeom& g, int cfg, hipStream_t s) {
+  switch (cfg) {
+    case 0: return launch_chain_tile<2, 1, 1, 1, 64>(a, epi, d, g, s);
+    case 1: return launch_chain_tile<2, 1, 1, 3, 64>(a, epi, d, g, s);
+    case 2: return launch_chain_tile<4, 1, 1, 2, 64>(a, epi, d, g, s);
+  }
+  return DH_EINVAL;
+}
+
+}
diff --git a/deephar_amd/csrc/plan.hip b/deephar_amd/csrc/plan.hip
--- a/deephar_amd/csrc/plan.hip
+++ b/deephar_amd/csrc/plan.hip
@@ -7,6 +7,8 @@
 using dh::check_launch;
 
 enum Fn { F_CONV, F_DW, F_POOL, F_UPADD, F_ELT, F_SAM, F_CTX, F_DMEANS, F_SAM1D, F_KRON, F_GMM, F_COPY, F_ZPAD, F_DFM, F_SAMCTX, F_NORM, F_GROUP, F_PAIR, F_SEG, F_DWS, F_CONVT, F_CONVTS, F_COUNT };
+
+constexpr int F_CHAIN = F_COUNT, F_COUNT_V5 = F_COUNT + 1;
 
 struct Step { int fn; std::vector<unsigned char> payload; };
 struct In { uint64_t tag; size_t items; int u8; char* dst; };
@@ -140,6 +142,9 @@
     }
     case F_GROUP:
       return dh_conv2d_dw_group_f32(reinterpret_cast<const dh_conv_args*>(p),
+                                    reinterpret_cast<const dh_dw_args*>(p + sizeof(dh_conv_args)), stream);
+    case F_CHAIN:
+      return dh_conv2d_dw_chain_f32(reinterpret_cast<const dh_conv_args*>(p),
                                     reinterpret_cast<const dh_dw_args*>(p + sizeof(dh_conv_args)), stream);
     case F_PAIR:
       return dh_conv2d_pair_f32(reinterpret_cast<const dh_conv_args*>(p), reinterpret_cast<const dh_conv_args*>(p + sizeof(dh_conv_args)),
@@ -175,7 +180,7 @@
   if (std::memcmp(r.p, "DHPL", 4) != 0) return DH_EINVAL;
   r.p += 4;
   const uint32_t version = r.get<uint32_t>();
-  if (version < 1 || version > 4) return DH_EINVAL;
+  if (version < 1 || version > 5) return DH_EINVAL;
   dh_plan* pl = new dh_plan();
   pl->n = r.get<int32_t>();
   pl->arena_bytes = r.get<uint64_t>();
@@ -207,7 +212,7 @@
     Step st;
     st.fn = (int)r.get<uint32_t>();
     const uint32_t nb = r.get<uint32_t>();
-    if (!r.ok || st.fn < 0 || st.fn >= (version >= 4 ? (int)F_COUNT : (version == 3 ? (int)F_CONVTS : (int)F_DWS)) || r.p + nb > r.end) return fail(DH_EINVAL);
+    if (!r.ok || st.fn < 0 || st.fn >= (version >= 5 ? F_COUNT_V5 : version == 4 ? (int)F_COUNT : (version == 3 ? (int)F_CONVTS : (int)F_DWS)) || r.p + nb > r.end) return fail(DH_EINVAL);
     st.payload.assign(r.p, r.p + nb);
     r.p += nb;
     pl->steps.push_back(std::move(st));
@@ -242,14 +247,14 @@
       return fail(DH_EINVAL);
   for (Step& st : pl->steps) {
     const int np = struct_pointers(st.fn);
-    if (st.fn == F_GROUP || st.fn == F_PAIR || st.fn == F_SEG) {
-      const size_t second = st.fn == F_GROUP ? sizeof(dh_dw_args) : (st.fn == F_PAIR ? sizeof(dh_conv_args) : sizeof(dh_conv_seg));
+    if (st.fn == F_GROUP || st.fn == F_CHAIN || st.fn == F_PAIR || st.fn == F_SEG) {
+      const size_t second = (st.fn == F_GROUP || st.fn == F_CHAIN) ? sizeof(dh_dw_args) : (st.fn == F_PAIR ? sizeof(dh_conv_args) : sizeof(dh_conv_seg));
       if (st.payload.size() != sizeof(dh_conv_args) + second) return fail(DH_EINVAL);
       size_t at_off[10 + 1 + 10 + 1];
       int k = 0;
       for (int i = 0; i < 10; ++i) at_off[k++] = (size_t)8 * i;
       at_off[k++] = offsetof(dh_conv_args, y_pool);
-      for (int i = 0; i < (st.fn == F_GROUP ? 5 : (st.fn == F_PAIR ? 10 : 1)); ++i) at_off[k++] = sizeof(dh_conv_args) + (size_t)8 * i;
+      for (int i = 0; i < ((st.fn == F_GROUP || st.fn == F_CHAIN) ? 5 : (st.fn == F_PAIR ? 10 : 1)); ++i) at_off[k++] = sizeof(dh_conv_args) + (size_t)8 * i;
       if (st.fn == F_PAIR) at_off[k++] = sizeof(dh_conv_args) + offsetof(dh_conv_args, y_pool);
       for (int i = 0; i < k; ++i) {
         unsigned char* at = st.payload.data() + at_off[i];
diff --git a/deephar_amd/engine/executor.py b/deephar_amd/engine/executor.py
--- a/deephar_amd/engine/executor.py
+++ b/deephar_amd/engine/executor.py
@@ -196,6 +196,8 @@
         self.noop_calls = set()
         self.paired = []
         self.absorbed = {}
+        self.chained = []
+        self.chain_times = {}
 
     def weight_layout(self, args):
         mode = getattr(self.plan, 'gemm_precision', 'f32')
@@ -560,6 +562,65 @@
             self._drop_graph()
         return self.grouped
 
+    CHAIN_MARGIN = 0.97
+
+    def chain_dw(self, stream_ptr, table=None, reps=20):
+        if not self.plan.rules.group_launches or self.chained:
+            return len(self.chained)
+        lib = self.lib
+        table = {} if table is None else table
+        ev = None
+        for i in range(self.npre, len(self.calls) - 1):
+            fc, ac, sc = self.calls[i]
+            if fc is not lib.dh_conv2d_f32 or sc.kind != 'conv' or i in self.noop_calls:
+                continue
+            j = next((k for k in range(i + 1, len(self.calls)) if self.calls[k][2].stream == sc.stream), None)
+            if j is None:
+                continue
+            fd, ad, sd = self.calls[j]
+            if fd is not lib.dh_dwconv2d_f32 or sd.kind != 'dwconv' or sd.wait or j in self.noop_calls:
+                continue
+            if not lib.dh_conv2d_dw_chain_eligible(ac[0], ad[0]):
+                continue
+            key = ('chain_dw', self.n) + self._conv_signature(sc) + (sd.attrs['kh'], sd.attrs['pre_relu'], sd.outs['y'].ld)
+            if key not in table:
+                if ev is None:
+                    ev = (C.c_void_p(), C.c_void_p())
+                    _lib.check(lib.dh_event_create(C.byref(ev[0])))
+                    _lib.check(lib.dh_event_create(C.byref(ev[1])))
+
+                def timed(launch):
+                    best = float('inf')
+                    for _trial in range(4):
+                        _lib.check(lib.dh_event_record(ev[0], stream_ptr))
+                        for _ in range(reps):
+                            launch()
+                        _lib.check(lib.dh_event_record(ev[1], stream_ptr))
+                        _lib.check(lib.dh_event_synchronize(ev[1]))
+                        ms = C.c_float()
+                        _lib.check(lib.dh_event_elapsed_ms(ev[0], ev[1], C.byref(ms)))
+                        best = min(best, ms.value / reps)
+                    return best
+
+                def two():
+                    _lib.check(fc(*ac, stream_ptr), 'conv')
+                    _lib.check(fd(*ad, stream_ptr), 'dwconv')
+
+                def one():
+                    _lib.check(lib.dh_conv2d_dw_chain_f32(ac[0], ad[0], stream_ptr), 'chained conv + dwconv')
+                t_two, t_one = timed(two), timed(one)
+                table[key] = int(t_one <= self.CHAIN_MARGIN * t_two)
+                self.chain_times[key] = (t_two, t_one)
+            if table[key]:
+                self._absorb(i, j, lib.dh_conv2d_dw_chain_f32)
+                self.chained.append((i, j))
+        if ev is not None:
+            lib.dh_event_destroy(ev[0])
+            lib.dh_event_destroy(ev[1])
+        if self.chained:
+            self._drop_graph()
+        return len(self.chained)
+
     def _absorb(self, i, k, fn):
         (_, ai, si), (_, ak, sk) = self.calls[i], self.calls[k]
         self.calls[i] = (fn, (ai[0], ak[0]), si)
@@ -853,6 +914,7 @@
                 if self.autotune:
                     bp.autotune(self.stream_ptr, self.tune_table)
                 bp.group_launches(self.stream_ptr)
+                bp.chain_dw(self.stream_ptr, self.tune_table)
             self.bound[key] = bp
             while len(self.bound) > self.max_bound:
                 old = next(iter(self.bound))
diff --git a/deephar_amd/engine/planner.py b/deephar_amd/engine/planner.py
--- a/deephar_amd/engine/planner.py
+++ b/deephar_amd/engine/planner.py
@@ -406,10 +406,43 @@
         self._merge_siblings_into_joint_buffers()
         self._merge_sibling_pools()
         self._pool_into_segmented_conv()
+        self._hoist_chained_depthwise()
         self._collect_params()
         from . import schedule
         schedule.finalize(self.plan, self.nstreams, self.stream_policy)
         return self.plan
+
+    @staticmethod
+    def chain_candidate(conv, dw):
+        if conv.kind != 'conv' or dw.kind != 'dwconv':
+            return False
+        a, d, y, x = conv.attrs, dw.attrs, conv.outs['y'], dw.ins['x']
+        if (a['kh'], a['kw'], a['sh'], a['sw'], a['pt'], a['pl']) != (1, 1, 1, 1, 0, 0) or a['up2'] or 'pre_bn' in conv.params or \
+                a.get('seg') is not None or a.get('x_resample', 0):
+            return False
+        if 'pre_bn' in dw.params or d.get('up_in') or 'sh' in d or d['kh'] != d['kw'] or d['kh'] not in (3, 5):
+            return False
+        if x.buf is not y.buf or (x.coff, x.ld, x.shape) != (y.coff, y.ld, y.shape):
+            return False
+        return len(y.shape) >= 3 and y.shape[-3:-1] in ((8, 8), (16, 16)) and y.C % 32 == 0 and y.C == a['Cout']
+
+    def _hoist_chained_depthwise(self):
+        if not self.rules.group_launches:
+            return
+        steps = self.plan.steps
+        i = 0
+        while i < len(steps):
+            p = steps[i]
+            j = next((k for k in range(i + 2, len(steps)) if self.chain_candidate(p, steps[k])), None) if p.kind == 'conv' else None
+            if j is not None and not (i + 1 < len(steps) and self.chain_candidate(p, steps[i + 1])):
+                d = steps[j]
+                xb, yb = d.ins['x'].buf, d.outs['y'].buf
+                between = steps[i + 1:j]
+                clean = all(yb is not v.buf for s in between for v in list(s.ins.values()) + list(s.outs.values()) if v is not None) and \
+                    all(xb is not v.buf for s in between for v in s.outs.values() if v is not None)
+                if clean:
+                    steps.insert(i + 1, steps.pop(j))
+            i += 1
 
     def _merge_sibling_pointwise(self):
         if not self.rules.merge_heads:
diff --git a/deephar_amd/engine/schedule.py b/deephar_amd/engine/schedule.py
--- a/deephar_amd/engine/schedule.py
+++ b/deephar_amd/engine/schedule.py
@@ -200,6 +200,12 @@
         for v in list(s.ins.values()) + list(s.outs.values()):
             if v is not None and j not in acc[id(v.buf)]:
                 acc[id(v.buf)].append(j)
+    if plan.rules.group_launches:
+        from .planner import Planner
+        for j in range(1, n):
+            p, d = plan.steps[j - 1], plan.steps[j]
+            if p.stream == d.stream and Planner.chain_candidate(p, d):
+                acc[id(d.outs['y'].buf)].insert(0, j - 1)
     full = (1 << n) - 1
     info = {}
     for b in plan.bufs:
diff --git a/deephar_amd/engine/serialize.py b/deephar_amd/engine/serialize.py
--- a/deephar_amd/engine/serialize.py
+++ b/deephar_amd/engine/serialize.py
@@ -14,6 +14,8 @@
 V3_FUNCTIONS = FUNCTIONS.index('dh_dwconv2d_strided_f32')
 V4_FUNCTIONS = ['dh_conv2d_transpose2x2_split_f32']
 ALL_FUNCTIONS = FUNCTIONS + V4_FUNCTIONS
+V5_FUNCTIONS = ['dh_conv2d_dw_chain_f32']
+KNOWN_FUNCTIONS = ALL_FUNCTIONS + V5_FUNCTIONS
 ARENA, WEIGHTS, BYTES = 1, 2, 3
 
 
@@ -75,6 +77,8 @@
 
 def blob_version(function_ids):
     top = max(function_ids, default=0)
+    if top >= len(ALL_FUNCTIONS):
+        return 5
     return 4 if top >= len(FUNCTIONS) else (3 if top >= V3_FUNCTIONS else VERSION)
 
 
@@ -87,8 +91,8 @@
         bp = ex.bind(batch, u8_norm=u8_norm)
     ex.stream.synchronize()
     lib = _lib.load()
-    names = {n: i for i, n in enumerate(ALL_FUNCTIONS)}
-    by_addr = {C.cast(getattr(lib, n), C.c_void_p).value: n for n in ALL_FUNCTIONS}
+    names = {n: i for i, n in enumerate(KNOWN_FUNCTIONS)}
+    by_addr = {C.cast(getattr(lib, n), C.c_void_p).value: n for n in KNOWN_FUNCTIONS}
     reg = _Regions(bp)
     steps = []
     for idx, (fn, args, step) in enumerate(bp.calls):
diff --git a/include/deephar_hip.h b/include/deephar_hip.h
--- a/include/deephar_hip.h
+++ b/include/deephar_hip.h
@@ -111,6 +111,11 @@
 
 int dh_conv2d_dw_group_f32(const dh_conv_args* conv, const dh_dw_args* dw, void* stream);
 
+int dh_conv2d_dw_chain_eligible(const dh_conv_args* conv, const dh_dw_args* dw);
+int dh_conv2d_dw_chain_num_tile_cfgs(void);
+int dh_conv2d_dw_chain_cfg_f32(const dh_conv_args* conv, const dh_dw_args* dw, int chain_cfg, void* stream);
+int dh_conv2d_dw_chain_f32(const dh_conv_args* conv, const dh_dw_args* dw, void* stream);
+
 typedef struct dh_conv_seg {
   const float* x2;
   int32_t ldx2;
```

After: 5147 frames/s, median of 6. Within noise of the previous version (+0.3%).
